# Ugness/MeBT

Hardware: AMD Instinct MI355X
Metric: masked video tokens/sec/GPU (train step, 24L d=1024, 1024+256 tok) (higher is better)
Workload: dtype bf16; 1 GPU; Sky-Timelapse 16f MeBT train step: 24L/1024d/16h, 1024 VQ tokens + 256 latents, batch 6/GPU, t=0.5 (NC=NT=512), fwd + masked CE + bwd + AdamW; global_batch=6, parallelism=dp1, optimizer=in-backward (fused into the weight-gradient launches)

## Files before the change

include/mebt_hip.h:

```cpp
#ifndef MEBT_HIP_H
#define MEBT_HIP_H

#include <stdint.h>

#ifdef __cplusplus
extern "C" {
#endif

#define MEBT_ABI_VERSION 2
#define MEBT_MAX_LAYERS 128

typedef void* mebt_stream_t;
typedef struct mebt_model mebt_model;

enum mebt_status { MEBT_STATUS_OK = 0, MEBT_STATUS_EINVAL = 1, MEBT_STATUS_ESHAPE = 2, MEBT_STATUS_EHIP = 3,
                   MEBT_STATUS_EWORKSPACE = 4, MEBT_STATUS_EDTYPE = 5 };
enum mebt_dtype { MEBT_DTYPE_F32 = 0, MEBT_DTYPE_BF16 = 1, MEBT_DTYPE_F16 = 2  };
enum mebt_mode { MEBT_MODE_LATENT_ENC = 0, MEBT_MODE_LATENT_SELF = 1, MEBT_MODE_LATENT_DEC = 2, MEBT_MODE_LT2L = 3,
                 MEBT_MODE_MASKGIT = 4  };

typedef struct mebt_model_desc {
    int32_t n_layer, n_head, n_embd, vocab, n_latent , block_size;
    int32_t dtype;
    int32_t modes[MEBT_MAX_LAYERS];
    float label_smoothing;
    float embd_pdrop, resid_pdrop, attn_pdrop;
} mebt_model_desc;

const char* mebt_last_error(void);
int mebt_abi_version(void);

int mebt_model_create(const mebt_model_desc* desc, mebt_model** out);
void mebt_model_destroy(mebt_model* m);
int mebt_model_param_counts(const mebt_model* m, int64_t* n_w, int64_t* n_p);
int mebt_model_bind(mebt_model* m, float* W, void* W_lp, float* gW, float* P, float* gP);
int mebt_model_sync_lowp(mebt_model* m, mebt_stream_t stream);
int64_t mebt_workspace_bytes(const mebt_model* m, int32_t B, int32_t NC, int32_t NT, int32_t training);

int mebt_forward(mebt_model* m, void* ws, int64_t ws_bytes, int32_t B, int32_t N, int32_t NC, int32_t NT,
                 const int64_t* x_ids, const int64_t* ci, const int64_t* ti, float* logits,
                 int32_t training, uint64_t dropout_seed, mebt_stream_t stream);
int64_t mebt_kvcache_bytes(const mebt_model* m, int32_t B, int32_t N);
int mebt_forward_kvcache(mebt_model* m, void* ws, int64_t ws_bytes, int32_t B, int32_t N, int32_t NC, int32_t NT,
                         const int64_t* x_ids, const int64_t* ci, const int64_t* ti, void* logits, int32_t flags,
                         void* kv_cache, const int64_t* dirty, int32_t ND, mebt_stream_t stream);
int mebt_gpt_forward(mebt_model* m, void* ws, int64_t ws_bytes, int32_t B, int32_t NC, int32_t NT, const float* sos,
                     const float* contexts, const float* targets, float* logits, mebt_stream_t stream);
int mebt_gpt_forward_train(mebt_model* m, void* ws, int64_t ws_bytes, int32_t B, int32_t NC, int32_t NT, const float* sos,
                           const float* contexts, const float* targets, float* logits, int32_t dropout, uint64_t dropout_seed,
                           mebt_stream_t stream);
int mebt_gpt_backward(mebt_model* m, void* ws, const float* dlogits, float* d_sos, float* d_contexts, float* d_targets,
                      mebt_stream_t stream);
int mebt_loss(mebt_model* m, void* ws, const float* logits, double* out4, mebt_stream_t stream);
int mebt_loss_with_grad(mebt_model* m, void* ws, const float* logits, double* out4, float loss_scale, mebt_stream_t stream);
int mebt_backward_head(mebt_model* m, void* ws, const float* logits, const float* upstream, float loss_scale, mebt_stream_t stream);
int mebt_backward_head_dlogits(mebt_model* m, void* ws, const float* dlogits, mebt_stream_t stream);
int mebt_backward_layers(mebt_model* m, void* ws, int32_t layer_hi, int32_t layer_lo, mebt_stream_t stream);
int mebt_backward_embed(mebt_model* m, void* ws, mebt_stream_t stream);
int mebt_adamw_step(mebt_model* m, float* mW, float* vW, float* mP, float* vP, float lr, float beta1, float beta2,
                    float eps, float weight_decay, int32_t step, float grad_scale, mebt_stream_t stream);

int mebt_adamw_range(mebt_model* m, float* mW, float* vW, float* mP, float* vP, float lr, float beta1, float beta2,
                     float eps, float weight_decay, int32_t step, float grad_scale, int32_t kind, int32_t layer_hi,
                     int32_t layer_lo, mebt_stream_t stream);

int mebt_adamw_slice(mebt_model* m, int32_t which, int64_t off, int64_t n, const void* grad, int32_t grad_bf16, float* mW,
                     float* vW, float* mP, float* vP, float lr, float beta1, float beta2, float eps, float weight_decay,
                     int32_t step, float grad_scale, mebt_stream_t stream);

int mebt_adamw_slice_pieces(mebt_model* m, int32_t which, int64_t off, int64_t n, const void* grad_pieces, int32_t pieces, float* mW,
                            float* vW, float* mP, float* vP, float lr, float beta1, float beta2, float eps, float weight_decay,
                            int32_t step, float grad_scale, mebt_stream_t stream);

int mebt_model_set_fused_adamw(mebt_model* m, float* mW, float* vW, float lr, float beta1, float beta2, float eps,
                               float weight_decay, int32_t step, float grad_scale);

int mebt_model_bind_wire_grads(mebt_model* m, void* gWb);

int mebt_model_set_forward_waits(mebt_model* m, int32_t n, const int32_t* layer, void* const* events);
int mebt_model_set_grad_accumulate(mebt_model* m, int32_t on);

int mebt_op_gemm(int32_t dtype, const void* A, const void* B, void* C, void* C2, const float* bias, const void* aux,
                 int32_t M, int32_t N, int32_t K, int32_t lda, int32_t ldb, int32_t ldc, int32_t ld_aux,
                 int32_t a_kc, int32_t b_kc, int32_t epilogue, int32_t c_f32, int32_t beta, int32_t split_k,
                 mebt_stream_t stream);
int mebt_op_layernorm_fwd(int32_t dtype, const void* x, void* y, const float* gamma, const float* beta, float* mean,
                          float* rstd, int32_t rows, int32_t d, mebt_stream_t stream);
int mebt_op_layernorm_bwd(int32_t dtype, const void* x, const void* dy, const float* gamma, const float* mean,
                          const float* rstd, void* dx, float* dgamma, float* dbeta, int32_t rows, int32_t d,
                          mebt_stream_t stream);
int mebt_op_attention_fwd(int32_t dtype, const void* q, const void* k, const void* v, void* o, float* lse, int32_t B,
                          int32_t H, int32_t NQ, int32_t NK, int32_t HD, int32_t ldq, int32_t ldk, int32_t ldv,
                          int32_t ldo, int32_t force_generic, mebt_stream_t stream);
int mebt_op_attention_bwd(int32_t dtype, const void* q, const void* k, const void* v, const void* o, const float* lse,
                          const void* d_o, void* dq, void* dk, void* dv, float* delta, int32_t B, int32_t H,
                          int32_t NQ, int32_t NK, int32_t HD, int32_t ldq, int32_t ldk, int32_t ldv, int32_t ldo,
                          int32_t force_generic, mebt_stream_t stream);
int mebt_op_embed_fwd(int32_t dtype, const int64_t* x_ids, const int64_t* ci, const int64_t* ti, const float* tok_emb,
                      const float* pos_emb, const float* mask_emb, const float* sos_emb, void* sos, void* ctx, void* tgt,
                      int32_t B, int32_t N, int32_t NC, int32_t NT, int32_t NS, int32_t d, int32_t vocab,
                      int32_t block_size, mebt_stream_t stream);
int mebt_op_sample(const float* logits, const float* noise, float temperature, int32_t top_k, float top_p, int64_t* ids,
                   float* score, float* probs, int32_t rows, int32_t V, mebt_stream_t stream);
int mebt_op_sample_seeded(const float* logits, uint64_t seed, float temperature, int32_t top_k, float top_p, int64_t* ids,
                          float* score, float* probs, int32_t rows, int32_t V, mebt_stream_t stream);
int mebt_op_wgrad_grouped(int32_t n, const void* const* dY, const void* const* X, const int32_t* n_out, const int32_t* k_in,
                          const int32_t* tokens, const int64_t* w_off, float* const* bias, float* W, float* gW, float* mW, float* vW,
                          void* Wlp, int32_t fused, float lr, float beta1, float beta2, float eps, float weight_decay, int32_t step,
                          float grad_scale, mebt_stream_t stream);
int mebt_op_gemm_pair(const void* const* A, const void* const* B, void* const* C, const float* const* bias, const void* const* aux,
                      const int32_t* M, const int32_t* N, const int32_t* K, const int32_t* lda, const int32_t* ldb, const int32_t* ldc,
                      const int32_t* ld_aux, const int32_t* epilogue, const int32_t* c_f32, int32_t b_kc, mebt_stream_t stream);
int mebt_op_topk_threshold(const float* logits, int32_t top_k, float* kth, int64_t* ids_scratch, int32_t rows, int32_t V,
                           mebt_stream_t stream);
int mebt_op_sample_scatter(const float* logits, const float* noise, uint64_t seed, float temperature, int32_t top_k, int64_t* ids,
                           float* score, float* probs_map, const int64_t* ti, int32_t B, int32_t N, int32_t NT, int32_t V,
                           mebt_stream_t stream);
int mebt_op_sample_lp(const void* logits, int32_t logits_bf16, const float* noise, uint64_t seed, float temperature, int32_t top_k,
                      int64_t* ids, float* score, float* probs_map, const int64_t* ti, int32_t B, int32_t N, int32_t NT, int32_t V,
                      int32_t draw, mebt_stream_t stream);
int mebt_op_scatter_ids(int64_t* x, const int64_t* ti, const int64_t* ids, int32_t B, int32_t N, int32_t NT,
                        mebt_stream_t stream);
int mebt_op_next_mask(const int64_t* ci, const int64_t* ti, const float* score, const float* noise, float ctemp,
                      int32_t n_new, int32_t B, int32_t NC, int32_t NT, int64_t* new_ci, int64_t* new_ti,
                      mebt_stream_t stream);
int mebt_op_cast_bf16(const float* src, void* dst, int64_t n, mebt_stream_t stream);

void mebt_gemm_autotune(int32_t mode);
int32_t mebt_gemm_autotune_enabled(void);
int64_t mebt_gemm_tune_export(char* buf, int64_t cap);
int32_t mebt_gemm_tune_import(const char* text, int32_t overwrite);
int64_t mebt_gemm_tune_alternatives(char* buf, int64_t cap);

#define MEBT_CONV_MAX_TAPS 64
typedef struct mebt_conv3d_desc {
    const void* in; void* out; const void* w; const float* bias; const void* resid;
    int32_t B, Ti, Hi, Wi, Cin, To, Ho, Wo, Cout;
    int32_t cT, cH, cW;
    int32_t os[3], pi[3], sm[3];
    int32_t ntaps;
    int8_t tap[MEBT_CONV_MAX_TAPS][4];
    int32_t in_mode;
    int32_t out_mode;
} mebt_conv3d_desc;
int mebt_op_conv3d(int32_t dtype, const mebt_conv3d_desc* d, int32_t allow_mfma, mebt_stream_t stream);
int mebt_op_groupnorm_silu(int32_t dtype, const void* x, void* y, const float* gamma, const float* beta, float* stats, int32_t B,
                           int64_t vox_per_sample, int32_t C, mebt_stream_t stream);
int mebt_op_codebook_argmin(const float* z, const float* embeddings, float* score, float* esq, int64_t* ids, int32_t M,
                            int32_t n_codes, int32_t d, mebt_stream_t stream);
int mebt_op_codebook_argmin_filtered(const float* z, const float* embeddings, void* score, float* esq, void* lowp, int64_t* ids,
                                     int32_t M, int32_t n_codes, int32_t d, mebt_stream_t stream);
int mebt_op_embedding_rows(int32_t dtype, const int64_t* ids, const float* embeddings, void* out, int64_t rows, int32_t d,
                           int32_t n_codes, mebt_stream_t stream);
int mebt_op_cast_f16(const float* src, void* dst, int64_t n, mebt_stream_t stream);

int mebt_op_frames_to_video(const uint8_t* frames, float* out, int32_t N, int32_t T, int32_t Hs, int32_t Ws, int32_t y0, int32_t x0,
                            int32_t S, int32_t R, const int32_t* tab, int32_t K, int32_t rows, int32_t span, const float* lut,
                            const int32_t* slots, int32_t Bout, mebt_stream_t stream);
int mebt_op_frames_to_clip_u8(const uint8_t* frames, uint8_t* out, int32_t N, int32_t T, int32_t Hs, int32_t Ws, int32_t y0, int32_t x0,
                              int32_t S, int32_t R, const int32_t* tab, int32_t K, int32_t rows, int32_t span, const uint8_t* lut,
                              const int32_t* slots, int32_t Bout, mebt_stream_t stream);
int mebt_op_pack_to_video(const uint8_t* pack, int64_t F, const int64_t* ids, float* out, int32_t B, int32_t T, int32_t R,
                          const float* lut, mebt_stream_t stream);
int mebt_op_pack_to_clip_u8(const uint8_t* pack, int64_t F, const int64_t* ids, uint8_t* out, int32_t B, int32_t T, int32_t R,
                            const uint8_t* lut, mebt_stream_t stream);
int mebt_op_video_to_clip_u8(const float* in, uint8_t* out, int32_t B, int32_t Td, int32_t T, int32_t H, int32_t W,
                             mebt_stream_t stream);
int mebt_op_i3d_preprocess(int32_t dtype, const uint8_t* in, void* out, int32_t N, int32_t H, int32_t W, int32_t Ho, int32_t Wo,
                           mebt_stream_t stream);
#define MEBT_I3D_MAX_SEGS 3
typedef struct mebt_i3d_seg {
    void* out;
    int32_t n0, n1, cstride, coff;
} mebt_i3d_seg;
typedef struct mebt_i3d_conv_desc {
    const void* in; const void* w; const float* bias;
    int32_t B, Ti, Hi, Wi, Cin, To, Ho, Wo, Cout;
    int32_t k[3], s[3], pad_front[3], pad_back[3];
    int32_t relu;
    int32_t nseg;
    mebt_i3d_seg seg[MEBT_I3D_MAX_SEGS];
} mebt_i3d_conv_desc;
int mebt_op_i3d_conv(int32_t dtype, const mebt_i3d_conv_desc* d, mebt_stream_t stream);
int mebt_op_i3d_maxpool(int32_t dtype, const void* in, void* out, int32_t B, int32_t Ti, int32_t Hi, int32_t Wi, int32_t C, int32_t kt,
                        int32_t kh, int32_t kw, int32_t st, int32_t sh, int32_t sw, mebt_stream_t stream);
int mebt_op_i3d_head(int32_t dtype, const void* x, const float* w, const float* bias, float* pooled, float* logits, int32_t B, int32_t T,
                     int32_t H, int32_t W, int32_t C, int32_t ncls, mebt_stream_t stream);

int mebt_profile_enable(int32_t on);
int mebt_profile_read(int32_t family, double* launches, double* total_ms, double* total_flops);
int64_t mebt_profile_dump(char* buf, int64_t cap);
int32_t mebt_profile_read_waits(int32_t cap, int32_t* layer, double* ms);
int mebt_debug_dropout_mask(uint64_t seed, uint32_t site, float p, int64_t n, float* out, mebt_stream_t stream);
int mebt_debug_clock_probe(unsigned long long* out4, uint64_t ref_ticks_100mhz, mebt_stream_t stream);
void mebt_debug_side_stream(mebt_model* m, int32_t on);
void mebt_debug_set_side_stream(mebt_model* m, mebt_stream_t stream);
void mebt_debug_gemm_tile(int32_t bm, int32_t bn);
void mebt_debug_gemm_variant(int32_t dma);
void mebt_debug_gemm_scratch(void* buf, int64_t bytes);
void mebt_debug_gemm_stamps(unsigned long long* buf);
void mebt_debug_attn_dropout(uint64_t seed, float p, void* dmask);
void mebt_debug_attn_legacy(int32_t bits);
int mebt_debug_attn_block_order(int32_t T, int32_t X, int32_t H, int32_t xcd, int32_t* pos_to_id, mebt_stream_t stream);
void mebt_debug_grouped_config(int32_t tbm, int32_t tbn, int32_t ring);
void mebt_debug_pair_config(int32_t tbm, int32_t tbn, int32_t ring);
int32_t mebt_debug_gemm_last_launch(int32_t out[8]);
void mebt_debug_grouped_stages(int32_t n);

#ifdef __cplusplus
}
#endif
#endif
```

mebt_amd/_lib.py:

```python
import ctypes as C
import os

_HERE = os.path.dirname(os.path.abspath(__file__))
LIB_PATH = os.environ.get("MEBT_HIP_LIB") or os.path.join(_HERE, "lib", "libmebt_hip.so")

SHIPPED_TUNE = os.path.join(_HERE, "tune", "gfx950.txt")

MEBT_MAX_LAYERS = 128
F32, BF16, F16 = 0, 1, 2
EPI_NONE, EPI_GELU, EPI_RESID, EPI_GELU_BWD = 0, 1, 2, 3
MODE_IDS = {"latent_enc": 0, "latent_self": 1, "latent_dec": 2, "lt2l": 3, "maskgit": 4}

c_i32, c_i64, c_f32, c_vp = C.c_int32, C.c_int64, C.c_float, C.c_void_p


class ModelDesc(C.Structure):
    _fields_ = [("n_layer", c_i32), ("n_head", c_i32), ("n_embd", c_i32), ("vocab", c_i32),
                ("n_latent", c_i32), ("block_size", c_i32), ("dtype", c_i32),
                ("modes", c_i32 * MEBT_MAX_LAYERS), ("label_smoothing", c_f32),
                ("embd_pdrop", c_f32), ("resid_pdrop", c_f32), ("attn_pdrop", c_f32)]


PROTOTYPES = {
    "mebt_last_error": (C.c_char_p, []),
    "mebt_abi_version": (c_i32, []),
    "mebt_model_create": (c_i32, [C.POINTER(ModelDesc), C.POINTER(c_vp)]),
    "mebt_model_destroy": (None, [c_vp]),
    "mebt_model_param_counts": (c_i32, [c_vp, C.POINTER(c_i64), C.POINTER(c_i64)]),
    "mebt_model_bind": (c_i32, [c_vp, c_vp, c_vp, c_vp, c_vp, c_vp]),
    "mebt_model_sync_lowp": (c_i32, [c_vp, c_vp]),
    "mebt_workspace_bytes": (c_i64, [c_vp, c_i32, c_i32, c_i32, c_i32]),
    "mebt_forward": (c_i32, [c_vp, c_vp, c_i64, c_i32, c_i32, c_i32, c_i32, c_vp, c_vp, c_vp, c_vp, c_i32, C.c_uint64, c_vp]),
    "mebt_kvcache_bytes": (c_i64, [c_vp, c_i32, c_i32]),
    "mebt_forward_kvcache": (c_i32, [c_vp, c_vp, c_i64, c_i32, c_i32, c_i32, c_i32, c_vp, c_vp, c_vp, c_vp, c_i32, c_vp, c_vp, c_i32, c_vp]),
    "mebt_gpt_forward": (c_i32, [c_vp, c_vp, c_i64, c_i32, c_i32, c_i32, c_vp, c_vp, c_vp, c_vp, c_vp]),
    "mebt_gpt_forward_train": (c_i32, [c_vp, c_vp, c_i64, c_i32, c_i32, c_i32, c_vp, c_vp, c_vp, c_vp, c_i32, C.c_uint64, c_vp]),
    "mebt_gpt_backward": (c_i32, [c_vp, c_vp, c_vp, c_vp, c_vp, c_vp, c_vp]),
    "mebt_loss": (c_i32, [c_vp, c_vp, c_vp, c_vp, c_vp]),
    "mebt_loss_with_grad": (c_i32, [c_vp, c_vp, c_vp, c_vp, C.c_float, c_vp]),
    "mebt_backward_head": (c_i32, [c_vp, c_vp, c_vp, c_vp, c_f32, c_vp]),
    "mebt_backward_head_dlogits": (c_i32, [c_vp, c_vp, c_vp, c_vp]),
    "mebt_backward_layers": (c_i32, [c_vp, c_vp, c_i32, c_i32, c_vp]),
    "mebt_backward_embed": (c_i32, [c_vp, c_vp, c_vp]),
    "mebt_adamw_step": (c_i32, [c_vp, c_vp, c_vp, c_vp, c_vp, c_f32, c_f32, c_f32, c_f32, c_f32, c_i32, c_f32, c_vp]),
    "mebt_adamw_range": (c_i32, [c_vp, c_vp, c_vp, c_vp, c_vp, c_f32, c_f32, c_f32, c_f32, c_f32, c_i32, c_f32, c_i32, c_i32, c_i32, c_vp]),
    "mebt_adamw_slice": (c_i32, [c_vp, c_i32, c_i64, c_i64, c_vp, c_i32, c_vp, c_vp, c_vp, c_vp, c_f32, c_f32, c_f32, c_f32, c_f32, c_i32, c_f32, c_vp]),
    "mebt_adamw_slice_pieces": (c_i32, [c_vp, c_i32, c_i64, c_i64, c_vp, c_i32, c_vp, c_vp, c_vp, c_vp, c_f32, c_f32, c_f32, c_f32, c_f32, c_i32, c_f32, c_vp]),
    "mebt_model_set_fused_adamw": (c_i32, [c_vp, c_vp, c_vp, c_f32, c_f32, c_f32, c_f32, c_f32, c_i32, c_f32]),
    "mebt_model_set_grad_accumulate": (c_i32, [c_vp, c_i32]),
    "mebt_model_bind_wire_grads": (c_i32, [c_vp, c_vp]),
    "mebt_model_set_forward_waits": (c_i32, [c_vp, c_i32, C.POINTER(C.c_int32), C.POINTER(C.c_void_p)]),
    "mebt_op_gemm": (c_i32, [c_i32, c_vp, c_vp, c_vp, c_vp, c_vp, c_vp] + [c_i32] * 13 + [c_vp]),
    "mebt_op_layernorm_fwd": (c_i32, [c_i32, c_vp, c_vp, c_vp, c_vp, c_vp, c_vp, c_i32, c_i32, c_vp]),
    "mebt_op_layernorm_bwd": (c_i32, [c_i32, c_vp, c_vp, c_vp, c_vp, c_vp, c_vp, c_vp, c_vp, c_i32, c_i32, c_vp]),
    "mebt_op_attention_fwd": (c_i32, [c_i32, c_vp, c_vp, c_vp, c_vp, c_vp] + [c_i32] * 10 + [c_vp]),
    "mebt_op_attention_bwd": (c_i32, [c_i32] + [c_vp] * 10 + [c_i32] * 10 + [c_vp]),
    "mebt_op_embed_fwd": (c_i32, [c_i32] + [c_vp] * 10 + [c_i32] * 8 + [c_vp]),
    "mebt_op_sample": (c_i32, [c_vp, c_vp, c_f32, c_i32, c_f32, c_vp, c_vp, c_vp, c_i32, c_i32, c_vp]),
    "mebt_op_sample_seeded": (c_i32, [c_vp, C.c_uint64, c_f32, c_i32, c_f32, c_vp, c_vp, c_vp, c_i32, c_i32, c_vp]),
    "mebt_op_sample_scatter": (c_i32, [c_vp, c_vp, C.c_uint64, c_f32, c_i32, c_vp, c_vp, c_vp, c_vp, c_i32, c_i32, c_i32, c_i32, c_vp]),
    "mebt_op_sample_lp": (c_i32, [c_vp, c_i32, c_vp, C.c_uint64, c_f32, c_i32, c_vp, c_vp, c_vp, c_vp, c_i32, c_i32, c_i32, c_i32, c_i32, c_vp]),
    "mebt_op_wgrad_grouped": (c_i32, [c_i32, c_vp, c_vp, c_vp, c_vp, c_vp, c_vp, c_vp, c_vp, c_vp, c_vp, c_vp, c_vp, c_i32, c_f32, c_f32, c_f32,
                                      c_f32, c_f32, c_i32, c_f32, c_vp]),
    "mebt_op_gemm_pair": (c_i32, [c_vp] * 14 + [c_i32, c_vp]),
    "mebt_op_topk_threshold": (c_i32, [c_vp, c_i32, c_vp, c_vp, c_i32, c_i32, c_vp]),
    "mebt_op_scatter_ids": (c_i32, [c_vp, c_vp, c_vp, c_i32, c_i32, c_i32, c_vp]),
    "mebt_op_next_mask": (c_i32, [c_vp, c_vp, c_vp, c_vp, c_f32, c_i32, c_i32, c_i32, c_i32, c_vp, c_vp, c_vp]),
    "mebt_op_cast_bf16": (c_i32, [c_vp, c_vp, c_i64, c_vp]),
    "mebt_op_conv3d": (c_i32, [c_i32, c_vp, c_i32, c_vp]),
    "mebt_op_groupnorm_silu": (c_i32, [c_i32, c_vp, c_vp, c_vp, c_vp, c_vp, c_i32, c_i64, c_i32, c_vp]),
    "mebt_op_codebook_argmin": (c_i32, [c_vp, c_vp, c_vp, c_vp, c_vp, c_i32, c_i32, c_i32, c_vp]),
    "mebt_op_codebook_argmin_filtered": (c_i32, [c_vp, c_vp, c_vp, c_vp, c_vp, c_vp, c_i32, c_i32, c_i32, c_vp]),
    "mebt_op_embedding_rows": (c_i32, [c_i32, c_vp, c_vp, c_vp, c_i64, c_i32, c_i32, c_vp]),
    "mebt_op_cast_f16": (c_i32, [c_vp, c_vp, c_i64, c_vp]),
    "mebt_op_i3d_preprocess": (c_i32, [c_i32, c_vp, c_vp, c_i32, c_i32, c_i32, c_i32, c_i32, c_vp]),
    "mebt_op_i3d_conv": (c_i32, [c_i32, c_vp, c_vp]),
    "mebt_op_i3d_maxpool": (c_i32, [c_i32, c_vp, c_vp] + [c_i32] * 11 + [c_vp]),
    "mebt_op_i3d_head": (c_i32, [c_i32, c_vp, c_vp, c_vp, c_vp, c_vp] + [c_i32] * 6 + [c_vp]),
    "mebt_op_frames_to_video": (c_i32, [c_vp, c_vp] + [c_i32] * 8 + [c_vp, c_i32, c_i32, c_i32, c_vp, c_vp, c_i32, c_vp]),
    "mebt_op_frames_to_clip_u8": (c_i32, [c_vp, c_vp] + [c_i32] * 8 + [c_vp, c_i32, c_i32, c_i32, c_vp, c_vp, c_i32, c_vp]),
    "mebt_op_pack_to_video": (c_i32, [c_vp, c_i64, c_vp, c_vp, c_i32, c_i32, c_i32, c_vp, c_vp]),
    "mebt_op_pack_to_clip_u8": (c_i32, [c_vp, c_i64, c_vp, c_vp, c_i32, c_i32, c_i32, c_vp, c_vp]),
    "mebt_op_video_to_clip_u8": (c_i32, [c_vp, c_vp, c_i32, c_i32, c_i32, c_i32, c_i32, c_vp]),
    "mebt_debug_dropout_mask": (c_i32, [C.c_uint64, C.c_uint32, c_f32, c_i64, c_vp, c_vp]),
    "mebt_debug_clock_probe": (c_i32, [c_vp, C.c_uint64, c_vp]),
    "mebt_debug_side_stream": (None, [c_vp, c_i32]),
    "mebt_debug_set_side_stream": (None, [c_vp, c_vp]),
    "mebt_debug_gemm_tile": (None, [c_i32, c_i32]),
    "mebt_debug_gemm_variant": (None, [c_i32]),
    "mebt_debug_grouped_stages": (None, [c_i32]),
    "mebt_debug_gemm_scratch": (None, [c_vp, c_i64]),
    "mebt_debug_gemm_stamps": (None, [c_vp]),
    "mebt_debug_grouped_config": (None, [c_i32, c_i32, c_i32]),
    "mebt_debug_pair_config": (None, [c_i32, c_i32, c_i32]),
    "mebt_debug_gemm_last_launch": (c_i32, [C.POINTER(c_i32)]),
    "mebt_debug_attn_dropout": (None, [C.c_uint64, c_f32, c_vp]),
    "mebt_debug_attn_legacy": (None, [c_i32]),
    "mebt_debug_attn_block_order": (c_i32, [c_i32, c_i32, c_i32, c_i32, c_vp, c_vp]),
    "mebt_gemm_autotune": (None, [c_i32]),
    "mebt_gemm_autotune_enabled": (c_i32, []),
    "mebt_gemm_tune_export": (c_i64, [C.c_char_p, c_i64]),
    "mebt_gemm_tune_import": (c_i32, [C.c_char_p, c_i32]),
    "mebt_gemm_tune_alternatives": (c_i64, [C.c_char_p, c_i64]),
    "mebt_profile_enable": (c_i32, [c_i32]),
    "mebt_profile_read": (c_i32, [c_i32, C.POINTER(C.c_double), C.POINTER(C.c_double), C.POINTER(C.c_double)]),
    "mebt_profile_dump": (c_i64, [C.c_char_p, c_i64]),
    "mebt_profile_read_waits": (c_i32, [c_i32, C.POINTER(C.c_int32), C.POINTER(C.c_double)]),
}

_lib = None


def load():
    global _lib
    if _lib is not None:
        return _lib
    if not os.path.exists(LIB_PATH):
        raise RuntimeError(
            f"{LIB_PATH} not found: build it with `python -c 'import __graft_entry__ as g; g.build()'` "
            "(or `make -C mebt_amd/csrc`). mebt_amd has no fallback path without its HIP library.")
    try:
        import torch
    except ImportError:
        pass
    lib = C.CDLL(LIB_PATH)
    for name, (res, args) in PROTOTYPES.items():
        fn = getattr(lib, name)
        fn.restype = res
        fn.argtypes = args
    _lib = lib
    if os.environ.get("MEBT_GEMM_TUNE_SHIPPED", "1") != "0" and os.path.exists(SHIPPED_TUNE):
        with open(SHIPPED_TUNE, "rb") as f:
            lib.mebt_gemm_tune_import(f.read(), 0)
    return lib


def tune_table_text():
    lib = load()
    n = lib.mebt_gemm_tune_export(None, 0)
    buf = C.create_string_buffer(int(n))
    lib.mebt_gemm_tune_export(buf, n)
    return buf.value.decode()


def tune_table_merge(text, overwrite=True, replace=False):
    return int(load().mebt_gemm_tune_import(text.encode() if isinstance(text, str) else text, 2 if replace else (1 if overwrite else 0)))


class MebtError(RuntimeError):
    pass


def check(status):
    if status != 0:
        msg = load().mebt_last_error()
        raise MebtError(f"libmebt_hip status {status}: {msg.decode() if msg else '?'}")


def ptr(t):
    return None if t is None else t.data_ptr()


def cur_stream():
    import torch
    return torch.cuda.current_stream().cuda_stream
```

mebt_amd/csrc/capi.cpp:

```cpp
#include "common.h"
#include "kernels.h"
#include <cmath>
#include "../../include/mebt_hip.h"
#include <string.h>

static hipStream_t S(mebt_stream_t s) { return reinterpret_cast<hipStream_t>(s); }
static int check_dtype(int dtype) {
    if (dtype == MEBT_F32 || dtype == MEBT_BF16) return MEBT_OK;
    mebt_set_error("unsupported dtype (0 = f32, 1 = bf16)");
    return MEBT_EDTYPE;
}

extern "C" int mebt_op_gemm(int32_t dtype, const void* A, const void* B, void* C, void* C2, const float* bias, const void* aux,
                            int32_t M, int32_t N, int32_t K, int32_t lda, int32_t ldb, int32_t ldc, int32_t ld_aux,
                            int32_t a_kc, int32_t b_kc, int32_t epilogue, int32_t c_f32, int32_t beta, int32_t split_k,
                            mebt_stream_t stream) {
    if (int rc = check_dtype(dtype)) return rc;
    if (!A || !B || (!C && epilogue != EPI_GELU)) { mebt_set_error("gemm: null operand"); return MEBT_EINVAL; }
    if (epilogue < EPI_NONE || epilogue > EPI_GELU_BWD) { mebt_set_error("gemm: bad epilogue"); return MEBT_EINVAL; }
    if ((epilogue == EPI_RESID || epilogue == EPI_GELU_BWD) && !aux) { mebt_set_error("gemm: epilogue needs aux"); return MEBT_EINVAL; }
    if (epilogue == EPI_GELU && !C2) { mebt_set_error("gemm: GELU epilogue needs C2"); return MEBT_EINVAL; }
    if (M < 0 || N < 0 || K <= 0) { mebt_set_error("gemm: bad extents"); return MEBT_ESHAPE; }
    static bool inited = false;
    if (!inited) { if (int rc = gemm_init_attributes()) return rc; inited = true; }
// ... 52 lines not shown
}

extern "C" int mebt_op_layernorm_fwd(int32_t dtype, const void* x, void* y, const float* gamma, const float* beta, float* mean,
                                     float* rstd, int32_t rows, int32_t d, mebt_stream_t stream) {
    if (int rc = check_dtype(dtype)) return rc;
    if (!x || !y || !gamma || !beta) { mebt_set_error("layernorm: null pointer"); return MEBT_EINVAL; }
    LnFwdParams p;
    p.x = x; p.y = y; p.gamma = gamma; p.beta = beta; p.mean = mean; p.rstd = rstd; p.rows = rows; p.d = d;
    p.seg = 0; p.seg_stride = 0; p.seg_off = 0;
    return launch_ln_fwd(p, dtype, S(stream));
}

extern "C" int mebt_op_layernorm_bwd(int32_t dtype, const void* x, const void* dy, const float* gamma, const float* mean,
                                     const float* rstd, void* dx, float* dgamma, float* dbeta, int32_t rows, int32_t d,
                                     mebt_stream_t stream) {
    if (int rc = check_dtype(dtype)) return rc;
    if (!x || !dy || !gamma || !mean || !rstd || !dx || !dgamma || !dbeta) { mebt_set_error("layernorm_bwd: null pointer"); return MEBT_EINVAL; }
    LnBwdParams p;
    p.x = x; p.dy = dy; p.dy2 = nullptr; p.dx_add = nullptr; p.gamma = gamma; p.mean = mean; p.rstd = rstd; p.dx = dx; p.dx_f32 = dtype == MEBT_F32;
    p.dx_accumulate = 0; p.dgamma = dgamma; p.dbeta = dbeta; p.rows = rows; p.d = d; p.seg = 0; p.seg_stride = 0; p.seg_off = 0;
    return launch_ln_bwd(p, dtype, S(stream));
}

static DropCfg g_op_attn_drop = make_drop(0, 0, 0.f);
static uint16_t* g_op_attn_dmask = nullptr;
extern "C" void mebt_debug_attn_dropout(uint64_t seed, float p, void* dmask) {
    g_op_attn_drop = make_drop(seed, SITE_ATTN, p);
    g_op_attn_dmask = p > 0.f ? (uint16_t*)dmask : nullptr;
}
extern "C" void mebt_debug_attn_legacy(int32_t bits) { mebt_attn_set_legacy(bits); }
extern "C" int mebt_debug_attn_block_order(int32_t T, int32_t X, int32_t H, int32_t xcd, int32_t* pos_to_id, mebt_stream_t stream) {
    if (!pos_to_id) { mebt_set_error("attention block order: null pointer"); return MEBT_EINVAL; }
    return launch_attn_block_order_probe(T, X, H, xcd, pos_to_id, S(stream));
}

extern "C" int mebt_op_attention_fwd(int32_t dtype, const void* q, const void* k, const void* v, void* o, float* lse, int32_t B,
                                     int32_t H, int32_t NQ, int32_t NK, int32_t HD, int32_t ldq, int32_t ldk, int32_t ldv,
                                     int32_t ldo, int32_t force_generic, mebt_stream_t stream) {
    if (int rc = check_dtype(dtype)) return rc;
    if (!q || !o || (NK > 0 && (!k || !v))) { mebt_set_error("attention: null pointer"); return MEBT_EINVAL; }
    AttnParams p;
    memset(&p, 0, sizeof(p));
    p.q = q; p.k = k; p.v = v; p.o = o; p.lse = lse; p.B = B; p.H = H; p.NQ = NQ; p.NK = NK; p.HD = HD;
    p.ldq = ldq; p.ldk = ldk; p.ldv = ldv; p.ldo = ldo;
    p.drop = g_op_attn_drop; p.dmask = g_op_attn_dmask;
    mebt_attn_force_generic(force_generic);
    const int rc = launch_attn_fwd(p, dtype, S(stream));
    mebt_attn_force_generic(0);
    return rc;
}

extern "C" int mebt_op_attention_bwd(int32_t dtype, const void* q, const void* k, const void* v, const void* o, const float* lse,
                                     const void* d_o, void* dq, void* dk, void* dv, float* delta, int32_t B, int32_t H,
                                     int32_t NQ, int32_t NK, int32_t HD, int32_t ldq, int32_t ldk, int32_t ldv, int32_t ldo,
                                     int32_t force_generic, mebt_stream_t stream) {
    if (int rc = check_dtype(dtype)) return rc;
    if (!q || !o || !lse || !d_o || !dq || !delta || (NK > 0 && (!k || !v || !dk || !dv))) { mebt_set_error("attention_bwd: null pointer"); return MEBT_EINVAL; }
    AttnParams p;
    memset(&p, 0, sizeof(p));
    p.q = q; p.k = k; p.v = v; p.o = const_cast<void*>(o); p.lse = const_cast<float*>(lse); p.B = B; p.H = H; p.NQ = NQ; p.NK = NK; p.HD = HD;
    p.ldq = ldq; p.ldk = ldk; p.ldv = ldv; p.ldo = ldo;
    p.d_o = d_o; p.dq = dq; p.dk = dk; p.dv = dv; p.delta = delta; p.lddo = ldo; p.lddq = ldq; p.lddk = ldk; p.lddv = ldv;
    p.drop = g_op_attn_drop; p.dmask = g_op_attn_dmask;
    mebt_attn_force_generic(force_generic);
    const int rc = launch_attn_bwd(p, dtype, S(stream));
    mebt_attn_force_generic(0);
    return rc;
}

extern "C" int mebt_op_embed_fwd(int32_t dtype, const int64_t* x_ids, const int64_t* ci, const int64_t* ti, const float* tok_emb,
                                 const float* pos_emb, const float* mask_emb, const float* sos_emb, void* sos, void* ctx, void* tgt,
                                 int32_t B, int32_t N, int32_t NC, int32_t NT, int32_t NS, int32_t d, int32_t vocab,
                                 int32_t block_size, mebt_stream_t stream) {
    if (int rc = check_dtype(dtype)) return rc;
    if (!x_ids || !tok_emb || !pos_emb || !mask_emb) { mebt_set_error("embed: null pointer"); return MEBT_EINVAL; }
    if (N > block_size) { mebt_set_error("embed: N exceeds block_size"); return MEBT_ESHAPE; }
    EmbedParams p;
    p.x_ids = x_ids; p.ci = ci; p.ti = ti; p.tok_emb = tok_emb; p.pos_emb = pos_emb; p.mask_emb = mask_emb; p.sos_emb = sos_emb;
    p.sos = sos; p.ctx = ctx; p.tgt = tgt; p.B = B; p.N = N; p.NC = NC; p.NT = NT; p.NS = NS; p.d = d; p.vocab = vocab; p.block_size = block_size;
    p.drop = make_drop(0, 0, 0.f);
    return launch_embed_fwd(p, dtype, S(stream));
}

extern "C" int mebt_op_sample(const float* logits, const float* noise, float temperature, int32_t top_k, float top_p, int64_t* ids,
                              float* score, float* probs, int32_t rows, int32_t V, mebt_stream_t stream) {
    if (!logits || !noise || !ids) { mebt_set_error("sample: null pointer"); return MEBT_EINVAL; }
    SampleParams p;
    p.logits = logits; p.noise = noise; p.temperature = temperature; p.top_k = top_k; p.top_p = top_p; p.ids = ids; p.score = score;
    p.probs = probs; p.rows = rows; p.V = V;
    return launch_sample(p, S(stream));
}

extern "C" int mebt_op_sample_seeded(const float* logits, uint64_t seed, float temperature, int32_t top_k, float top_p, int64_t* ids,
                                     float* score, float* probs, int32_t rows, int32_t V, mebt_stream_t stream) {
    if (!logits || !ids) { mebt_set_error("sample: null pointer"); return MEBT_EINVAL; }
    SampleParams p;
    p.logits = logits; p.noise = nullptr; p.noise_seed = seed; p.temperature = temperature; p.top_k = top_k; p.top_p = top_p; p.ids = ids;
    p.score = score; p.probs = probs; p.rows = rows; p.V = V;
    return launch_sample(p, S(stream));
}

extern "C" int mebt_op_sample_scatter(const float* logits, const float* noise, uint64_t seed, float temperature, int32_t top_k, int64_t* ids,
                                      float* score, float* probs_map, const int64_t* ti, int32_t B, int32_t N, int32_t NT, int32_t V,
                                      mebt_stream_t stream) {
    if (!logits || !ids || !probs_map || !ti) { mebt_set_error("sample_scatter: null pointer"); return MEBT_EINVAL; }
    if (B <= 0 || NT <= 0 || N < NT) { mebt_set_error("sample_scatter: need B > 0 and 0 < NT <= N"); return MEBT_ESHAPE; }
    SampleParams p;
    p.logits = logits; p.noise = noise; p.noise_seed = seed; p.temperature = temperature; p.top_k = top_k; p.top_p = 0.f; p.ids = ids;
    p.score = score; p.probs = probs_map; p.rows = B * NT; p.V = V; p.probs_ti = ti; p.probs_N = N; p.probs_NT = NT;
    return launch_sample(p, S(stream));
}

extern "C" int mebt_op_sample_lp(const void* logits, int32_t logits_bf16, const float* noise, uint64_t seed, float temperature, int32_t top_k,
                                 int64_t* ids, float* score, float* probs_map, const int64_t* ti, int32_t B, int32_t N, int32_t NT, int32_t V,
                                 int32_t draw, mebt_stream_t stream) {
    if (!logits || !ids) { mebt_set_error("sample_lp: null pointer"); return MEBT_EINVAL; }
    if ((probs_map != nullptr) != (ti != nullptr)) { mebt_set_error("sample_lp: probs_map and ti go together"); return MEBT_EINVAL; }
    if (B <= 0 || NT <= 0 || (probs_map && N < NT)) { mebt_set_error("sample_lp: need B > 0 and 0 < NT <= N"); return MEBT_ESHAPE; }
    SampleParams p;
    p.logits = reinterpret_cast<const float*>(logits); p.logits_bf16 = logits_bf16 ? 1 : 0; p.noise = noise; p.noise_seed = seed;
    p.temperature = temperature; p.top_k = top_k; p.top_p = 0.f; p.ids = ids; p.score = score; p.probs = probs_map; p.rows = B * NT; p.V = V;
    p.probs_ti = ti; p.probs_N = probs_map ? N : 0; p.probs_NT = probs_map ? NT : 0;
    if (draw != 0 && draw != 1) { mebt_set_error("sample_lp: draw must be 0 (arg-max p / q) or 1 (inverse CDF)"); return MEBT_EINVAL; }
    if (draw == 1 && noise) { mebt_set_error("sample_lp: the inverse-CDF draw takes no noise tensor"); return MEBT_EINVAL; }
    p.icdf = draw;
    return launch_sample(p, S(stream));
}

extern "C" int mebt_op_topk_threshold(const float* logits, int32_t top_k, float* kth, int64_t* ids_scratch, int32_t rows, int32_t V, mebt_stream_t stream) {
    if (!logits || !kth || !ids_scratch) { mebt_set_error("topk_threshold: null pointer"); return MEBT_EINVAL; }
    if (top_k <= 0 || top_k >= V) { mebt_set_error("topk_threshold: k must be in [1, V)"); return MEBT_ESHAPE; }
    SampleParams p;
    p.logits = logits; p.noise = nullptr; p.noise_seed = 0; p.temperature = 1.0f; p.top_k = top_k; p.top_p = 0.f; p.ids = ids_scratch;
    p.score = nullptr; p.probs = nullptr; p.rows = rows; p.V = V; p.kth = kth;
    return launch_sample(p, S(stream));
}

extern "C" int mebt_op_scatter_ids(int64_t* x, const int64_t* ti, const int64_t* ids, int32_t B, int32_t N, int32_t NT, mebt_stream_t stream) {
    if (!x || !ti || !ids) { mebt_set_error("scatter_ids: null pointer"); return MEBT_EINVAL; }
    return launch_scatter_ids(x, ti, ids, B, N, NT, S(stream));
}

extern "C" int mebt_op_next_mask(const int64_t* ci, const int64_t* ti, const float* score, const float* noise, float ctemp,
                                 int32_t n_new, int32_t B, int32_t NC, int32_t NT, int64_t* new_ci, int64_t* new_ti, mebt_stream_t stream) {
    if (!ti || !score || !noise || !new_ci || (NT - n_new > 0 && !new_ti) || (NC > 0 && !ci)) { mebt_set_error("next_mask: null pointer"); return MEBT_EINVAL; }
    NextMaskParams p;
    p.ci = ci; p.ti = ti; p.score = score; p.noise = noise; p.ctemp = ctemp; p.n_new = n_new; p.B = B; p.NC = NC; p.NT = NT;
    p.new_ci = new_ci; p.new_ti = new_ti;
    return launch_next_mask(p, S(stream));
}

extern "C" int mebt_op_cast_bf16(const float* src, void* dst, int64_t n, mebt_stream_t stream) {
    if (!src || !dst) { mebt_set_error("cast: null pointer"); return MEBT_EINVAL; }
    return launch_cast_f32_to_bf16(src, dst, (size_t)n, S(stream));
}
```

mebt_amd/csrc/common.h:

```cpp
#pragma once
#include <hip/hip_runtime.h>
#include <stdint.h>

typedef __bf16 bf16_t;
typedef __bf16 bf16x4 __attribute__((ext_vector_type(4)));
typedef __bf16 bf16x8 __attribute__((ext_vector_type(8)));
typedef short s16x4 __attribute__((ext_vector_type(4)));
typedef float f32x4 __attribute__((ext_vector_type(4)));
typedef float f32x16 __attribute__((ext_vector_type(16)));
typedef uint32_t u32x4 __attribute__((ext_vector_type(4)));
typedef uint32_t u32x2 __attribute__((ext_vector_type(2)));

#define MEBT_WAVE 64

enum { MEBT_OK = 0, MEBT_EINVAL = 1, MEBT_ESHAPE = 2, MEBT_EHIP = 3, MEBT_EWORKSPACE = 4, MEBT_EDTYPE = 5 };

#define MEBT_HIP_CHECK(expr)                                   \
    do {                                                       \
        hipError_t _e = (expr);                                \
        if (_e != hipSuccess) { mebt_set_hip_error(_e, #expr); (void)hipGetLastError(); return MEBT_EHIP; } \
    } while (0)
void mebt_set_hip_error(hipError_t e, const char* what);
void mebt_set_error(const char* msg);

// ... 9 lines not shown

typedef __attribute__((address_space(3))) void* lds_void_ptr;
typedef __attribute__((address_space(3))) char* lds_char_ptr;
__device__ __forceinline__ void dma16(__amdgpu_buffer_rsrc_t rsrc, unsigned lds_addr, unsigned voff) {
    unsigned keep;
    asm volatile("s_mov_b32 %0, m0\n\ts_mov_b32 m0, %2\n\ts_nop 0\n\tbuffer_load_dwordx4 %1, %3, 0 offen lds\n\ts_mov_b32 m0, %0"
                 : "=&s"(keep)
                 : "v"(voff), "s"(lds_addr), "s"(rsrc)
                 : "memory");
}

__device__ __forceinline__ unsigned lds_addr_of(const void* p) { return (unsigned)(size_t)(lds_char_ptr)(char*)p; }

template <typename T> __device__ __forceinline__ float to_f32(T v);
template <> __device__ __forceinline__ float to_f32<float>(float v) { return v; }
template <> __device__ __forceinline__ float to_f32<bf16_t>(bf16_t v) { return (float)v; }
template <typename T> __device__ __forceinline__ T from_f32(float v);
template <> __device__ __forceinline__ float from_f32<float>(float v) { return v; }
template <> __device__ __forceinline__ bf16_t from_f32<bf16_t>(float v) { return (bf16_t)v; }

template <typename T> __device__ __forceinline__ f32x4 load4(const T* p);
template <> __device__ __forceinline__ f32x4 load4<float>(const float* p) { return *reinterpret_cast<const f32x4*>(p); }
template <> __device__ __forceinline__ f32x4 load4<bf16_t>(const bf16_t* p) {
    bf16x4 v = *reinterpret_cast<const bf16x4*>(p);
    return f32x4{(float)v[0], (float)v[1], (float)v[2], (float)v[3]};
}
template <typename T> __device__ __forceinline__ void store4(T* p, f32x4 v);
template <> __device__ __forceinline__ void store4<float>(float* p, f32x4 v) { *reinterpret_cast<f32x4*>(p) = v; }
template <> __device__ __forceinline__ void store4<bf16_t>(bf16_t* p, f32x4 v) {
    bf16x4 o = {(bf16_t)v[0], (bf16_t)v[1], (bf16_t)v[2], (bf16_t)v[3]};
    *reinterpret_cast<bf16x4*>(p) = o;
}

__device__ __forceinline__ float wave_sum(float v) {
#pragma unroll
    for (int o = 32; o > 0; o >>= 1) v += __shfl_xor(v, o, 64);
    return v;
}
__device__ __forceinline__ float wave_max(float v) {
#pragma unroll
    for (int o = 32; o > 0; o >>= 1) v = fmaxf(v, __shfl_xor(v, o, 64));
    return v;
}
__device__ __forceinline__ int wave_sum_i(int v) {
#pragma unroll
    for (int o = 32; o > 0; o >>= 1) v += __shfl_xor(v, o, 64);
    return v;
}

__device__ __forceinline__ float gelu_f(float x) { return 0.5f * x * (1.0f + erff(x * 0.70710678118654752f)); }
__device__ __forceinline__ float gelu_grad_f(float x) {
    const float cdf = 0.5f * (1.0f + erff(x * 0.70710678118654752f));
    const float pdf = 0.3989422804014327f * __expf(-0.5f * x * x);
    return cdf + x * pdf;
}

__device__ __forceinline__ float erf_fast(float x) {
    const float ax = fabsf(x);
    float d = 1.0f + ax * (0.278393f + ax * (0.230389f + ax * (0.000972f + ax * 0.078108f)));
    d *= d; d *= d;
    return copysignf(1.0f - __frcp_rn(d), x);
}
__device__ __forceinline__ float gelu_fast(float x) { return 0.5f * x * (1.0f + erf_fast(x * 0.70710678118654752f)); }
__device__ __forceinline__ float gelu_grad_fast(float x) {
    const float cdf = 0.5f * (1.0f + erf_fast(x * 0.70710678118654752f));
    return cdf + x * 0.3989422804014327f * __builtin_amdgcn_exp2f(-0.7213475204444817f * x * x);
}

struct AdamWHyper { float lr, beta1, beta2, eps, weight_decay, bc1, bc2, grad_scale; };
__device__ __forceinline__ void adamw_update4(f32x4& p, const f32x4& g, f32x4& m, f32x4& v, const AdamWHyper& a) {
    const float step_size = a.lr / a.bc1;
    const float inv_sqrt_bc2 = rsqrtf(a.bc2);
#pragma unroll
    for (int j = 0; j < 4; ++j) {
        const float gj = g[j] * a.grad_scale;
        p[j] *= 1.0f - a.lr * a.weight_decay;
        m[j] = a.beta1 * m[j] + (1.0f - a.beta1) * gj;
        v[j] = a.beta2 * v[j] + (1.0f - a.beta2) * gj * gj;
        const float denom = sqrtf(v[j]) * inv_sqrt_bc2 + a.eps;
        p[j] -= step_size * (m[j] / denom);
    }
}

__device__ __forceinline__ uint32_t pair_hash(uint64_t seed, uint32_t site, uint64_t pair) {
    uint32_t h = ((uint32_t)pair ^ (uint32_t)seed) + ((uint32_t)(pair >> 32) + site) * 0x632BE5ABu + (uint32_t)(seed >> 32);
    h *= 0x9E3779B1u;
    h ^= h >> 15;
    h *= 0x85EBCA77u;
    h ^= h >> 13;
    return h;
}
__device__ __forceinline__ uint32_t mix_hash(uint64_t seed, uint32_t site, uint64_t idx) {
    const uint32_t h = pair_hash(seed, site, idx >> 1);
    return (idx & 1) ? (h >> 16) : (h & 0xFFFFu);
}
struct DropCfg {
    uint64_t seed;
    uint32_t site;
    uint32_t thresh;
    float inv_keep;
    uint32_t small;
    uint32_t base32;
};
__device__ __forceinline__ uint32_t pair_hash_cfg(const DropCfg& d, uint64_t pair) {
    if (!d.small) return pair_hash(d.seed, d.site, pair);
    uint32_t h = ((uint32_t)pair ^ (uint32_t)d.seed) + d.base32;
    h *= 0x9E3779B1u;
    h ^= h >> 15;
    h *= 0x85EBCA77u;
    h ^= h >> 13;
    return h;
}
__device__ __forceinline__ float drop_keep(const DropCfg& d, uint64_t idx) {
    const uint32_t h = pair_hash_cfg(d, idx >> 1);
    return ((idx & 1) ? (h >> 16) : (h & 0xFFFFu)) >= d.thresh ? d.inv_keep : 0.0f;
}
__device__ __forceinline__ f32x4 drop_keep4(const DropCfg& d, uint64_t idx0) {
    f32x4 k;
    if ((idx0 & 1) == 0) {
        const uint32_t h0 = pair_hash_cfg(d, idx0 >> 1), h1 = pair_hash_cfg(d, (idx0 >> 1) + 1);
        k[0] = (h0 & 0xFFFFu) >= d.thresh ? d.inv_keep : 0.0f;
        k[1] = (h0 >> 16) >= d.thresh ? d.inv_keep : 0.0f;
        k[2] = (h1 & 0xFFFFu) >= d.thresh ? d.inv_keep : 0.0f;
        k[3] = (h1 >> 16) >= d.thresh ? d.inv_keep : 0.0f;
    } else {
#pragma unroll
        for (int j = 0; j < 4; ++j) k[j] = drop_keep(d, idx0 + j);
    }
    return k;
}
```

mebt_amd/csrc/elementwise.hip:

```cpp
#include "common.h"
#include <cstdlib>
#include "kernels.h"

namespace {

template <typename T>
__global__ __launch_bounds__(256) void embed_fwd_kernel(const EmbedParams p) {
    const int lane = threadIdx.x & 63;
    const long row = (long)blockIdx.x * 4 + (threadIdx.x >> 6);
    const long per_b = (long)p.NS + p.NC + p.NT;
    if (row >= per_b * p.B) return;
    const int b = (int)(row / per_b);
    const int r = (int)(row % per_b);
    const float* src0;
    const float* src1 = nullptr;
    T* dst;
    DropCfg dc = p.drop;
    uint64_t ebase;
    if (r < p.NS) {
        src0 = p.sos_emb + (size_t)r * p.d;
        dst = reinterpret_cast<T*>(p.sos) + ((size_t)b * p.NS + r) * p.d;
        dc.site = SITE_EMB_SOS; ebase = ((uint64_t)b * p.NS + r) * p.d;
    } else if (r < p.NS + p.NC) {
        const int i = r - p.NS;
        long pos = p.ci[(size_t)b * p.NC + i];
        pos = pos < 0 ? 0 : (pos >= p.N ? p.N - 1 : pos);
        long tok = p.x_ids[(size_t)b * p.N + pos];
        tok = tok < 0 ? 0 : (tok >= p.vocab ? p.vocab - 1 : tok);
        src0 = p.tok_emb + (size_t)tok * p.d;
        src1 = p.pos_emb + (size_t)pos * p.d;
        dst = reinterpret_cast<T*>(p.ctx) + ((size_t)b * p.NC + i) * p.d;
        dc.site = SITE_EMB_CTX; ebase = ((uint64_t)b * p.NC + i) * p.d;
    } else {
        const int j = r - p.NS - p.NC;
        long pos = p.ti[(size_t)b * p.NT + j];
        pos = pos < 0 ? 0 : (pos >= p.N ? p.N - 1 : pos);
        src0 = p.mask_emb;
        src1 = p.pos_emb + (size_t)pos * p.d;
        dst = reinterpret_cast<T*>(p.tgt) + ((size_t)b * p.NT + j) * p.d;
        dc.site = SITE_EMB_TGT; ebase = ((uint64_t)b * p.NT + j) * p.d;
    }
    for (int e = lane * 4; e < p.d; e += 256) {
        f32x4 v = *reinterpret_cast<const f32x4*>(src0 + e);
        if (src1) v += *reinterpret_cast<const f32x4*>(src1 + e);
        if (dc.thresh) {
            v *= drop_keep4(dc, ebase + e);
        }
        store4<T>(dst + e, v);
    }
}

template <typename T>
__global__ __launch_bounds__(256) void embed_bwd_kernel(const EmbedBwdParams p) {
    const int lane = threadIdx.x & 63;
    const long row = (long)blockIdx.x * 4 + (threadIdx.x >> 6);
    const long per_b = (long)p.NC + p.NT;
    if (row >= per_b * p.B) return;
    const int b = (int)(row / per_b);
    const int r = (int)(row % per_b);
    if (r < p.NC) {
        const long pos = p.ci[(size_t)b * p.NC + r];
        const long tok = p.x_ids[(size_t)b * p.N + pos];
        const float* g = p.g_ctx + ((size_t)b * p.NC + r) * p.d;
        float* gt = p.g_tok_emb + (size_t)tok * p.d;
        float* gp = p.g_pos_emb + (size_t)pos * p.d;
        for (int e = lane; e < p.d; e += 64) {
            const float v = g[e];
            atomicAdd(gt + e, v);
            atomicAdd(gp + e, v);
        }
    } else {
        const int j0 = r - p.NC;
        const long pos = p.ti[(size_t)b * p.NT + j0];
        const T* g = reinterpret_cast<const T*>(p.g_tgt) + ((size_t)b * p.NT + j0) * p.d;
        float* gp = p.g_pos_emb + (size_t)pos * p.d;
        for (int e = lane; e < p.d; e += 64) atomicAdd(gp + e, to_f32<T>(g[e]));
    }
}

constexpr int LN_MAXC = 8;

__device__ __forceinline__ long map_row(long r, int seg, int seg_stride, int seg_off) {
    return seg > 0 ? (r / seg) * (long)seg_stride + seg_off + (r % seg) : r;
}

struct LnFwdMulti { LnFwdParams j[MEBT_LN_MAXJ]; int blk_start[MEBT_LN_MAXJ + 1]; int n; };
struct LnBwdMulti { LnBwdParams j[MEBT_LN_MAXJ]; int blk_start[MEBT_LN_MAXJ + 1]; int rpw[MEBT_LN_MAXJ]; int n; };

template <typename T>
__global__ __launch_bounds__(256) void ln_fwd_kernel(const LnFwdMulti mj) {
    int job = 0;
#pragma unroll
    for (int i = 1; i < MEBT_LN_MAXJ; ++i)
        if (i < mj.n && (int)blockIdx.x >= mj.blk_start[i]) job = i;
    const LnFwdParams& p = mj.j[job];
    const int lane = threadIdx.x & 63;
    const long row = (long)(blockIdx.x - mj.blk_start[job]) * 4 + (threadIdx.x >> 6);
    if (row >= p.rows) return;
    const T* x = reinterpret_cast<const T*>(p.x) + (size_t)row * p.d;
    f32x4 v[LN_MAXC];
    float s = 0.f;
#pragma unroll
    for (int c = 0; c < LN_MAXC; ++c) {
        const int e = lane * 4 + 256 * c;
        if (e < p.d) {
            v[c] = load4<T>(x + e);
            s += v[c][0] + v[c][1] + v[c][2] + v[c][3];
        }
    }
    const float mean = wave_sum(s) / p.d;
    float q = 0.f;
#pragma unroll
    for (int c = 0; c < LN_MAXC; ++c) {
        const int e = lane * 4 + 256 * c;
        if (e < p.d) {
#pragma unroll
            for (int j = 0; j < 4; ++j) { const float t = v[c][j] - mean; q += t * t; }
        }
    }
    const float rstd = rsqrtf(wave_sum(q) / p.d + 1e-5f);
    const long orow = map_row(row, p.seg, p.seg_stride, p.seg_off);
    T* y = reinterpret_cast<T*>(p.y) + (size_t)orow * p.d;
#pragma unroll
    for (int c = 0; c < LN_MAXC; ++c) {
        const int e = lane * 4 + 256 * c;
        if (e < p.d) {
            const f32x4 g = *reinterpret_cast<const f32x4*>(p.gamma + e);
            const f32x4 b = *reinterpret_cast<const f32x4*>(p.beta + e);
            f32x4 o;
#pragma unroll
            for (int j = 0; j < 4; ++j) o[j] = (v[c][j] - mean) * rstd * g[j] + b[j];
            store4<T>(y + e, o);
        }
    }
    if (p.mean && lane == 0) { p.mean[orow] = mean; p.rstd[orow] = rstd; }
}

template <typename T>
__device__ __forceinline__ void ln_bwd_dx_body(const LnBwdMulti& mj, int bid) {
    int job = 0;
#pragma unroll
    for (int i = 1; i < MEBT_LN_MAXJ; ++i)
        if (i < mj.n && bid >= mj.blk_start[i]) job = i;
    const LnBwdParams& p = mj.j[job];
    const int lane = threadIdx.x & 63;
    const int d = p.d;
    const long row = (long)(bid - mj.blk_start[job]) * 4 + (threadIdx.x >> 6);
    if (row >= p.rows) return;
    const long mrow = map_row(row, p.seg, p.seg_stride, p.seg_off);
    const T* x = reinterpret_cast<const T*>(p.x) + (size_t)row * d;
    const T* dy = reinterpret_cast<const T*>(p.dy) + (size_t)mrow * d;
    const T* dy2 = p.dy2 ? reinterpret_cast<const T*>(p.dy2) + (size_t)row * d : nullptr;
    const float mean = p.mean[mrow], rstd = p.rstd[mrow];
    f32x4 xh[LN_MAXC], gy[LN_MAXC];
    float s1 = 0.f, s2 = 0.f;
#pragma unroll
    for (int c = 0; c < LN_MAXC; ++c) {
        const int e = lane * 4 + 256 * c;
        if (e < d) {
// ... 338 lines not shown
    const float lt = l[tgt];
    float mx = -INFINITY, sum = 0.f;
    int rank = 0;
    for (int e = threadIdx.x * 4; e < p.V; e += 1024) {
        const f32x4 v = *reinterpret_cast<const f32x4*>(l + e);
#pragma unroll
        for (int q = 0; q < 4; ++q) {
            mx = fmaxf(mx, v[q]);
            sum += v[q];
            rank += (v[q] > lt) || (v[q] == lt && (e + q) < tgt);
        }
    }
    mx = block_max(mx, sh);
    float se = 0.f;
    for (int e = threadIdx.x * 4; e < p.V; e += 1024) {
        const f32x4 v = *reinterpret_cast<const f32x4*>(l + e);
#pragma unroll
        for (int q = 0; q < 4; ++q) se += __expf(v[q] - mx);
    }
    se = block_sum(se, sh);
    sum = block_sum(sum, sh);
    const float rk = block_sum((float)rank, sh);
    if (threadIdx.x == 0) {
        const float lse = mx + logf(se);
        const float eps = p.label_smoothing;
        p.row_lse[row] = lse;
        p.row_loss[row] = (1.f - eps) * (lse - lt) + eps * (lse - sum / p.V);
        p.row_rank[row] = (int)(rk + 0.5f);
    }
}

template <typename T, int NCH>
__global__ __launch_bounds__(256) void ce_fused_kernel(const CeParams p) {
    __shared__ float sh[4];
    const int row = blockIdx.x;
    const int b = row / p.NT, j = row % p.NT;
    const long pos = p.ti[(size_t)b * p.NT + j];
    const long tgt = p.x_ids[(size_t)b * p.N + pos];
    const float* l = p.logits + (size_t)row * p.V;
    f32x4 v[NCH];
#pragma unroll
    for (int c = 0; c < NCH; ++c) v[c] = *reinterpret_cast<const f32x4*>(l + threadIdx.x * 4 + 1024 * c);
    const float lt = l[tgt];
    float mx = -INFINITY, sum = 0.f;
    int rank = 0;
#pragma unroll
    for (int c = 0; c < NCH; ++c) {
        const int e = threadIdx.x * 4 + 1024 * c;
#pragma unroll
        for (int q = 0; q < 4; ++q) {
            mx = fmaxf(mx, v[c][q]);
            sum += v[c][q];
            rank += (v[c][q] > lt) || (v[c][q] == lt && (e + q) < tgt);
        }
    }
    mx = block_max(mx, sh);
    float se = 0.f;
#pragma unroll
    for (int c = 0; c < NCH; ++c)
#pragma unroll
        for (int q = 0; q < 4; ++q) se += __expf(v[c][q] - mx);
    se = block_sum(se, sh);
    sum = block_sum(sum, sh);
    const float rk = block_sum((float)rank, sh);
    const float lse = mx + logf(se);
    const float eps = p.label_smoothing;
    if (threadIdx.x == 0) {
        p.row_lse[row] = lse;
        p.row_loss[row] = (1.f - eps) * (lse - lt) + eps * (lse - sum / p.V);
        p.row_rank[row] = (int)(rk + 0.5f);
    }
    T* d = reinterpret_cast<T*>(p.dlogits) + (size_t)row * p.V;
    const float sc = p.grad_scale, u = eps / p.V;
#pragma unroll
    for (int c = 0; c < NCH; ++c) {
        const int e = threadIdx.x * 4 + 1024 * c;
        f32x4 o;
#pragma unroll
        for (int q = 0; q < 4; ++q) o[q] = (__expf(v[c][q] - lse) - ((e + q) == tgt ? 1.f - eps : 0.f) - u) * sc;
        store4<T>(d + e, o);
    }
}

__global__ __launch_bounds__(256) void ce_reduce_kernel(const float* row_loss, const int* row_rank, int rows, double* out) {
    __shared__ double sd[3][256];
    double s = 0, t1 = 0, t5 = 0;
    for (int r = threadIdx.x; r < rows; r += 256) {
        s += row_loss[r];
        t1 += row_rank[r] < 1;
        t5 += row_rank[r] < 5;
    }
    sd[0][threadIdx.x] = s; sd[1][threadIdx.x] = t1; sd[2][threadIdx.x] = t5;
    __syncthreads();
    for (int o = 128; o > 0; o >>= 1) {
        if (threadIdx.x < o) {
            sd[0][threadIdx.x] += sd[0][threadIdx.x + o];
            sd[1][threadIdx.x] += sd[1][threadIdx.x + o];
            sd[2][threadIdx.x] += sd[2][threadIdx.x + o];
        }
        __syncthreads();
    }
    if (threadIdx.x == 0) { out[0] = sd[0][0]; out[1] = sd[1][0]; out[2] = sd[2][0]; out[3] = rows; }
}

template <typename T>
__global__ __launch_bounds__(256) void ce_bwd_kernel(const CeBwdParams p) {
    const int row = blockIdx.x;
    const int b = row / p.NT, j = row % p.NT;
    const long pos = p.ti[(size_t)b * p.NT + j];
    const long tgt = p.x_ids[(size_t)b * p.N + pos];
    const float* l = p.logits + (size_t)row * p.V;
    T* d = reinterpret_cast<T*>(p.dlogits) + (size_t)row * p.V;
    const float lse = p.row_lse[row];
    const float sc = p.scale * (p.upstream ? *p.upstream : 1.0f);
    const float eps = p.label_smoothing, u = eps / p.V;
    for (int e = threadIdx.x * 4; e < p.V; e += 1024) {
        const f32x4 v = *reinterpret_cast<const f32x4*>(l + e);
        f32x4 o;
#pragma unroll
        for (int q = 0; q < 4; ++q) o[q] = (__expf(v[q] - lse) - ((e + q) == tgt ? 1.f - eps : 0.f) - u) * sc;
        store4<T>(d + e, o);
    }
}

template <typename TG>
__global__ __launch_bounds__(256) void adamw_kernel(const AdamWParams a) {
    const AdamWHyper h = {a.lr, a.beta1, a.beta2, a.eps, a.weight_decay, a.bc1, a.bc2, a.grad_scale};
    for (size_t i = ((size_t)blockIdx.x * 256 + threadIdx.x) * 4; i < a.n; i += (size_t)gridDim.x * 1024) {
        f32x4 p = *reinterpret_cast<const f32x4*>(a.p + i);
        f32x4 g = load4<TG>(reinterpret_cast<const TG*>(a.g) + i);
        if constexpr (sizeof(TG) == 2)
            for (int j = 1; j < a.g_pieces; ++j) g += load4<TG>(reinterpret_cast<const TG*>(a.g) + (size_t)j * a.g_stride + i);
        f32x4 m = *reinterpret_cast<const f32x4*>(a.m + i);
        f32x4 v = *reinterpret_cast<const f32x4*>(a.v + i);
        adamw_update4(p, g, m, v, h);
        *reinterpret_cast<f32x4*>(a.p + i) = p;
        *reinterpret_cast<f32x4*>(a.m + i) = m;
        *reinterpret_cast<f32x4*>(a.v + i) = v;
        if (a.p_bf16) store4<bf16_t>(reinterpret_cast<bf16_t*>(a.p_bf16) + i, p);
    }
}

template <typename TS, typename TD>
__global__ __launch_bounds__(256) void apply_dropout_kernel(const TS* src, TD* dst, size_t n, DropCfg d) {
    for (size_t i = ((size_t)blockIdx.x * 256 + threadIdx.x) * 4; i < n; i += (size_t)gridDim.x * 1024) {
        f32x4 v = load4<TS>(src + i);
        v *= drop_keep4(d, i);
        store4<TD>(dst + i, v);
    }
}

template <typename TS, typename TD>
__global__ __launch_bounds__(256) void copy_rows_kernel(const TS* src, TD* dst, long rows, int d, int s_seg, int s_stride, int s_off,
                                                        int d_seg, int d_stride, int d_off) {
    const int d4 = d / 4;
    const long total = rows * d4;
    for (long i = (long)blockIdx.x * 256 + threadIdx.x; i < total; i += (long)gridDim.x * 256) {
        const long r = i / d4;
        const int e = (int)(i % d4) * 4;
        store4<TD>(dst + (size_t)map_row(r, d_seg, d_stride, d_off) * d + e, load4<TS>(src + (size_t)map_row(r, s_seg, s_stride, s_off) * d + e));
    }
}

__global__ __launch_bounds__(256) void cast_bf16_kernel(const float* src, bf16_t* dst, size_t n) {
    for (size_t i = ((size_t)blockIdx.x * 256 + threadIdx.x) * 4; i < n; i += (size_t)gridDim.x * 1024)
        store4<bf16_t>(dst + i, *reinterpret_cast<const f32x4*>(src + i));
}

}

#define CHECK_LAUNCH() MEBT_HIP_CHECK(hipGetLastError())

int launch_embed_fwd(const EmbedParams& p, int dtype, hipStream_t stream) {
    if (p.d % 4) { mebt_set_error("embed: d must be a multiple of 4"); return MEBT_ESHAPE; }
    const long rows = (long)p.B * (p.NS + p.NC + p.NT);
    if (rows == 0) return MEBT_OK;
    const dim3 grid((unsigned)((rows + 3) / 4));
    if (dtype == MEBT_BF16) hipLaunchKernelGGL(embed_fwd_kernel<bf16_t>, grid, dim3(256), 0, stream, p);
    else hipLaunchKernelGGL(embed_fwd_kernel<float>, grid, dim3(256), 0, stream, p);
    CHECK_LAUNCH();
    return MEBT_OK;
}

int launch_embed_bwd(const EmbedBwdParams& p, int dtype, hipStream_t stream) {
    const long rows = (long)p.B * (p.NC + p.NT);
    if (rows > 0) {
        const dim3 grid((unsigned)((rows + 3) / 4));
        if (dtype == MEBT_BF16) hipLaunchKernelGGL(embed_bwd_kernel<bf16_t>, grid, dim3(256), 0, stream, p);
        else hipLaunchKernelGGL(embed_bwd_kernel<float>, grid, dim3(256), 0, stream, p);
        CHECK_LAUNCH();
    }
    int rc = launch_colsum(p.g_tgt, p.B * p.NT, p.d, p.d, p.g_mask_emb, dtype, stream);
    if (rc) return rc;
    if (p.NS > 0) rc = launch_colsum(p.g_sos, p.B, p.NS * p.d, p.NS * p.d, p.g_sos_emb, dtype, stream);
    return rc;
}

int launch_ln_fwd_multi(const LnFwdParams* jobs, int n, int dtype, hipStream_t stream) {
    LnFwdMulti mj;
    int k = 0, blocks = 0;
    for (int i = 0; i < n; ++i) {
        const LnFwdParams& p = jobs[i];
        if (p.rows <= 0) continue;
        if (p.d % 4 || p.d > 256 * LN_MAXC) { mebt_set_error("layernorm: d must be a multiple of 4 and <= 2048"); return MEBT_ESHAPE; }
        if (k == MEBT_LN_MAXJ) { mebt_set_error("layernorm: too many jobs in one launch"); return MEBT_EINVAL; }
        mj.j[k] = p;
        mj.blk_start[k] = blocks;
        blocks += (p.rows + 3) / 4;
        ++k;
    }
    if (!k) return MEBT_OK;
    mj.n = k;
    for (int i = k; i <= MEBT_LN_MAXJ; ++i) mj.blk_start[i] = blocks;
    bool same_d = true;
    for (int i = 1; i < k; ++i) same_d = same_d && mj.j[i].d == mj.j[0].d;
    const int d0 = mj.j[0].d;
    if (dtype == MEBT_BF16) {
        if (same_d && d0 == 1024) hipLaunchKernelGGL((ln_fwd_fast_kernel<bf16_t, 2>), dim3(blocks), dim3(256), 0, stream, mj);
        else if (same_d && d0 == 512) hipLaunchKernelGGL((ln_fwd_fast_kernel<bf16_t, 1>), dim3(blocks), dim3(256), 0, stream, mj);
        else if (same_d && d0 == 2048) hipLaunchKernelGGL((ln_fwd_fast_kernel<bf16_t, 4>), dim3(blocks), dim3(256), 0, stream, mj);
        else hipLaunchKernelGGL(ln_fwd_kernel<bf16_t>, dim3(blocks), dim3(256), 0, stream, mj);
    } else {
        if (same_d && d0 == 1024) hipLaunchKernelGGL((ln_fwd_fast_kernel<float, 4>), dim3(blocks), dim3(256), 0, stream, mj);
        else if (same_d && d0 == 256) hipLaunchKernelGGL((ln_fwd_fast_kernel<float, 1>), dim3(blocks), dim3(256), 0, stream, mj);
        else hipLaunchKernelGGL(ln_fwd_kernel<float>, dim3(blocks), dim3(256), 0, stream, mj);
    }
    CHECK_LAUNCH();
    return MEBT_OK;
}

int launch_ln_fwd(const LnFwdParams& p, int dtype, hipStream_t stream) { return launch_ln_fwd_multi(&p, 1, dtype, stream); }

static int prepare_colsum(const GroupedColsum& c, GroupedColsum& k, int& blocks_out);
int launch_ln_bwd_multi(const LnBwdParams* jobs, int n, int dtype, hipStream_t stream, hipStream_t param_stream, const GroupedColsum* colsums) {
    LnBwdMulti mj, mp;
    int k = 0, blocks = 0, pblocks = 0;
    for (int i = 0; i < n; ++i) {
        const LnBwdParams& p = jobs[i];
        if (p.rows <= 0) continue;
        if (p.d % 4 || p.d > 256 * LN_MAXC) { mebt_set_error("layernorm: d must be a multiple of 4 and <= 2048"); return MEBT_ESHAPE; }
        if (k == MEBT_LN_MAXJ) { mebt_set_error("layernorm: too many jobs in one launch"); return MEBT_EINVAL; }
        mj.j[k] = p; mp.j[k] = p;
        mj.rpw[k] = 1;
        mj.blk_start[k] = blocks;
        blocks += (p.rows + 3) / 4;
        const int gx = (p.d + 63) / 64;
        int rpb = 256;
        while ((p.rows + rpb - 1) / rpb > 32) rpb *= 2;
        while (rpb > 64 && (long)gx * ((p.rows + rpb - 1) / rpb) < 256) rpb /= 2;
        mp.rpw[k] = rpb;
        mp.blk_start[k] = pblocks;
        pblocks += gx * ((p.rows + rpb - 1) / rpb);
        ++k;
    }
    if (!k) return MEBT_OK;
    mj.n = mp.n = k;
    for (int i = k; i <= MEBT_LN_MAXJ; ++i) { mj.blk_start[i] = blocks; mp.blk_start[i] = pblocks; }
    (void)param_stream;
    bool same_d = true;
    for (int i = 1; i < k; ++i) same_d = same_d && mj.j[i].d == mj.j[0].d;
    const int d0 = mj.j[0].d;
    GroupedColsum cs;
    int cblocks = 0;
    if (colsums) { if (int rc = prepare_colsum(*colsums, cs, cblocks)) return rc; }
    if (cblocks) {
        const dim3 grid(blocks + pblocks + cblocks);
        const int cs_start = blocks + pblocks;
        if (dtype == MEBT_BF16) {
            if (same_d && d0 == 1024) hipLaunchKernelGGL((ln_bwd_colsum_kernel<bf16_t, 2>), grid, dim3(256), 0, stream, mj, mp, cs, blocks, cs_start);
            else if (same_d && d0 == 512) hipLaunchKernelGGL((ln_bwd_colsum_kernel<bf16_t, 1>), grid, dim3(256), 0, stream, mj, mp, cs, blocks, cs_start);
            else if (same_d && d0 == 2048) hipLaunchKernelGGL((ln_bwd_colsum_kernel<bf16_t, 4>), grid, dim3(256), 0, stream, mj, mp, cs, blocks, cs_start);
            else hipLaunchKernelGGL((ln_bwd_colsum_kernel<bf16_t, 0>), grid, dim3(256), 0, stream, mj, mp, cs, blocks, cs_start);
        } else {
            if (same_d && d0 == 1024) hipLaunchKernelGGL((ln_bwd_colsum_kernel<float, 4>), grid, dim3(256), 0, stream, mj, mp, cs, blocks, cs_start);
            else if (same_d && d0 == 256) hipLaunchKernelGGL((ln_bwd_colsum_kernel<float, 1>), grid, dim3(256), 0, stream, mj, mp, cs, blocks, cs_start);
            else hipLaunchKernelGGL((ln_bwd_colsum_kernel<float, 0>), grid, dim3(256), 0, stream, mj, mp, cs, blocks, cs_start);
        }
        CHECK_LAUNCH();
        return MEBT_OK;
    }
    const dim3 grid(blocks + pblocks);
    if (dtype == MEBT_BF16) {
        if (same_d && d0 == 1024) hipLaunchKernelGGL((ln_bwd_kernel<bf16_t, 2>), grid, dim3(256), 0, stream, mj, mp, blocks);
        else if (same_d && d0 == 512) hipLaunchKernelGGL((ln_bwd_kernel<bf16_t, 1>), grid, dim3(256), 0, stream, mj, mp, blocks);
        else if (same_d && d0 == 2048) hipLaunchKernelGGL((ln_bwd_kernel<bf16_t, 4>), grid, dim3(256), 0, stream, mj, mp, blocks);
        else hipLaunchKernelGGL((ln_bwd_kernel<bf16_t, 0>), grid, dim3(256), 0, stream, mj, mp, blocks);
    } else {
        if (same_d && d0 == 1024) hipLaunchKernelGGL((ln_bwd_kernel<float, 4>), grid, dim3(256), 0, stream, mj, mp, blocks);
        else if (same_d && d0 == 256) hipLaunchKernelGGL((ln_bwd_kernel<float, 1>), grid, dim3(256), 0, stream, mj, mp, blocks);
        else hipLaunchKernelGGL((ln_bwd_kernel<float, 0>), grid, dim3(256), 0, stream, mj, mp, blocks);
    }
    CHECK_LAUNCH();
    return MEBT_OK;
}

int launch_ln_bwd(const LnBwdParams& p, int dtype, hipStream_t stream, hipStream_t param_stream) { return launch_ln_bwd_multi(&p, 1, dtype, stream, param_stream, nullptr); }

int launch_colsum(const void* X, int M, int N, int ldx, float* out, int dtype, hipStream_t stream) {
    if (M <= 0 || N <= 0) return MEBT_OK;
    if (N % 4) { mebt_set_error("colsum: N must be a multiple of 4"); return MEBT_ESHAPE; }
    const int gx = (N + 63) / 64;
    int rpb = 256;
    while ((M + rpb - 1) / rpb > 32) rpb *= 2;
    while (rpb > 64 && (long)gx * ((M + rpb - 1) / rpb) < 256) rpb /= 2;
    const dim3 grid(gx, (M + rpb - 1) / rpb);
    if (dtype == MEBT_BF16) hipLaunchKernelGGL(colsum_kernel<bf16_t>, grid, dim3(256), 0, stream, reinterpret_cast<const bf16_t*>(X), M, N, ldx, out, rpb);
    else hipLaunchKernelGGL(colsum_kernel<float>, grid, dim3(256), 0, stream, reinterpret_cast<const float*>(X), M, N, ldx, out, rpb);
    CHECK_LAUNCH();
    return MEBT_OK;
}

static int prepare_colsum(const GroupedColsum& c, GroupedColsum& k, int& blocks_out) {
    int n = 0, blocks = 0;
    for (int i = 0; i < c.n; ++i) {
        if (c.g[i].M <= 0 || c.g[i].N <= 0) continue;
        if (c.g[i].N % 4) { mebt_set_error("colsum: N must be a multiple of 4"); return MEBT_ESHAPE; }
        k.g[n] = c.g[i];
        k.g[n].gx = (c.g[i].N + 63) / 64;
        int rpb = 256;
        while ((c.g[i].M + rpb - 1) / rpb > 32) rpb *= 2;
        while (rpb > 64 && (long)k.g[n].gx * ((c.g[i].M + rpb - 1) / rpb) < 128) rpb /= 2;
        k.g[n].rpb = rpb;
        k.blk_start[n] = blocks;
        blocks += k.g[n].gx * ((c.g[i].M + rpb - 1) / rpb);
        ++n;
    }
    k.n = n;
    for (int i = n; i <= MEBT_MAX_GROUP; ++i) k.blk_start[i] = blocks;
    blocks_out = blocks;
    return MEBT_OK;
}

int launch_colsum_grouped(GroupedColsum& c, int dtype, hipStream_t stream) {
    GroupedColsum k;
    int blocks = 0;
    if (int rc = prepare_colsum(c, k, blocks)) return rc;
    if (!blocks) return MEBT_OK;
    if (dtype == MEBT_BF16) hipLaunchKernelGGL(colsum_grouped_kernel<bf16_t>, dim3(blocks), dim3(256), 0, stream, k);
    else hipLaunchKernelGGL(colsum_grouped_kernel<float>, dim3(blocks), dim3(256), 0, stream, k);
    CHECK_LAUNCH();
    return MEBT_OK;
}

int launch_ce_fwd(const CeParams& p, hipStream_t stream) {
    if (p.V % 4) { mebt_set_error("cross-entropy: V must be a multiple of 4"); return MEBT_ESHAPE; }
    if (p.rows > 0) {
        if (p.dlogits && ce_fwd_can_fuse_grad(p.V)) {
            if (p.dl_bf16) hipLaunchKernelGGL((ce_fused_kernel<bf16_t, 16>), dim3(p.rows), dim3(256), 0, stream, p);
            else hipLaunchKernelGGL((ce_fused_kernel<float, 16>), dim3(p.rows), dim3(256), 0, stream, p);
        } else {
            hipLaunchKernelGGL(ce_fwd_kernel, dim3(p.rows), dim3(256), 0, stream, p);
        }
        CHECK_LAUNCH();
    }
    hipLaunchKernelGGL(ce_reduce_kernel, dim3(1), dim3(256), 0, stream, p.row_loss, p.row_rank, p.rows, p.out);
    CHECK_LAUNCH();
    return MEBT_OK;
}

int launch_ce_bwd(const CeBwdParams& p, int dtype, hipStream_t stream) {
    if (p.rows <= 0) return MEBT_OK;
    if (dtype == MEBT_BF16) hipLaunchKernelGGL(ce_bwd_kernel<bf16_t>, dim3(p.rows), dim3(256), 0, stream, p);
    else hipLaunchKernelGGL(ce_bwd_kernel<float>, dim3(p.rows), dim3(256), 0, stream, p);
    CHECK_LAUNCH();
    return MEBT_OK;
}

int launch_adamw(const AdamWParams& p, hipStream_t stream) {
    if (p.n == 0) return MEBT_OK;
    if (p.n % 4) { mebt_set_error("adamw: flat buffer length must be a multiple of 4"); return MEBT_ESHAPE; }
    const size_t blocks = (p.n / 4 + 255) / 256;
    if (p.g_bf16) hipLaunchKernelGGL(adamw_kernel<bf16_t>, dim3((unsigned)(blocks < 4096 ? blocks : 4096)), dim3(256), 0, stream, p);
    else hipLaunchKernelGGL(adamw_kernel<float>, dim3((unsigned)(blocks < 4096 ? blocks : 4096)), dim3(256), 0, stream, p);
    CHECK_LAUNCH();
    return MEBT_OK;
}

int launch_apply_dropout(const void* src, void* dst, size_t n, int src_f32, int dst_f32, const DropCfg& d, hipStream_t stream) {
    if (n == 0) return MEBT_OK;
    if (n % 4) { mebt_set_error("dropout: length must be a multiple of 4"); return MEBT_ESHAPE; }
    const size_t blocks = (n / 4 + 255) / 256;
    const dim3 grid((unsigned)(blocks < 4096 ? blocks : 4096));
    if (src_f32 && dst_f32) hipLaunchKernelGGL((apply_dropout_kernel<float, float>), grid, dim3(256), 0, stream, (const float*)src, (float*)dst, n, d);
    else if (!src_f32 && !dst_f32) hipLaunchKernelGGL((apply_dropout_kernel<bf16_t, bf16_t>), grid, dim3(256), 0, stream, (const bf16_t*)src, (bf16_t*)dst, n, d);
    else { mebt_set_error("dropout: mixed element types are not supported"); return MEBT_EDTYPE; }
    CHECK_LAUNCH();
    return MEBT_OK;
}

int launch_copy_rows(const void* src, void* dst, long rows, int d, int src_f32, int dst_f32, int s_seg, int s_stride, int s_off,
                     int d_seg, int d_stride, int d_off, hipStream_t stream) {
    if (rows <= 0 || d <= 0) return MEBT_OK;
    if (d % 4) { mebt_set_error("copy_rows: d must be a multiple of 4"); return MEBT_ESHAPE; }
    const long blocks = (rows * (d / 4) + 255) / 256;
    const dim3 grid((unsigned)(blocks < 8192 ? blocks : 8192));
#define COPY_ROWS(TS, TD) hipLaunchKernelGGL((copy_rows_kernel<TS, TD>), grid, dim3(256), 0, stream, (const TS*)src, (TD*)dst, rows, d, s_seg, s_stride, s_off, d_seg, d_stride, d_off)
    if (src_f32 && dst_f32) COPY_ROWS(float, float);
    else if (src_f32) COPY_ROWS(float, bf16_t);
    else if (dst_f32) COPY_ROWS(bf16_t, float);
    else COPY_ROWS(bf16_t, bf16_t);
#undef COPY_ROWS
    CHECK_LAUNCH();
    return MEBT_OK;
}

namespace {
__global__ __launch_bounds__(256) void index_rows_kernel(const char* src, char* dst, const int64_t* idx, long rows, int n, int npos, int row_bytes, int scatter) {
    const int lane = threadIdx.x & 63;
    const long r = (long)blockIdx.x * 4 + (threadIdx.x >> 6);
    if (r >= rows) return;
    const long b = r / n;
    const long pos = idx[r];
    if (pos < 0 || pos >= npos) return;
    const char* s = src + (size_t)(scatter ? r : b * npos + pos) * row_bytes;
    char* d = dst + (size_t)(scatter ? b * npos + pos : r) * row_bytes;
    for (int o = lane * 16; o < row_bytes; o += 1024) *reinterpret_cast<u32x4*>(d + o) = *reinterpret_cast<const u32x4*>(s + o);
}
}
namespace {
__global__ __launch_bounds__(256) void cast_i64_i32_kernel(const int64_t* src, int32_t* dst, size_t n) {
    const size_t i = (size_t)blockIdx.x * 256 + threadIdx.x;
    if (i < n) dst[i] = (int32_t)src[i];
}
}
int launch_cast_i64_i32(const int64_t* src, int32_t* dst, size_t n, hipStream_t stream) {
    if (!n) return MEBT_OK;
    hipLaunchKernelGGL(cast_i64_i32_kernel, dim3((unsigned)((n + 255) / 256)), dim3(256), 0, stream, src, dst, n);
    CHECK_LAUNCH();
    return MEBT_OK;
}
int launch_index_rows(const void* src, void* dst, const int64_t* idx, int B, int n, int npos, int row_bytes, int scatter, hipStream_t stream) {
    const long rows = (long)B * n;
    if (rows <= 0) return MEBT_OK;
    if (row_bytes % 16) { mebt_set_error("index_rows: rows must be a multiple of 16 bytes"); return MEBT_ESHAPE; }
    hipLaunchKernelGGL(index_rows_kernel, dim3((unsigned)((rows + 3) / 4)), dim3(256), 0, stream, (const char*)src, (char*)dst, idx, rows, n, npos, row_bytes, scatter);
    CHECK_LAUNCH();
    return MEBT_OK;
}

int launch_cast_f32_to_bf16(const float* src, void* dst, size_t n, hipStream_t stream) {
    if (n == 0) return MEBT_OK;
    if (n % 4) { mebt_set_error("cast: length must be a multiple of 4"); return MEBT_ESHAPE; }
    const size_t blocks = (n / 4 + 255) / 256;
    hipLaunchKernelGGL(cast_bf16_kernel, dim3((unsigned)(blocks < 4096 ? blocks : 4096)), dim3(256), 0, stream, src, reinterpret_cast<bf16_t*>(dst), n);
    CHECK_LAUNCH();
    return MEBT_OK;
}

namespace {
__global__ __launch_bounds__(64) void clock_probe_kernel(unsigned long long* out, unsigned long long ref_ticks) {
    if (threadIdx.x != 0) return;
    const unsigned long long t0 = __builtin_amdgcn_s_memtime(), r0 = __builtin_amdgcn_s_memrealtime();
    while (__builtin_amdgcn_s_memrealtime() - r0 < ref_ticks) __builtin_amdgcn_s_sleep(127);
    out[0] = t0; out[1] = r0; out[2] = __builtin_amdgcn_s_memtime(); out[3] = __builtin_amdgcn_s_memrealtime();
}
}
// ... 7 lines not shown
```

mebt_amd/csrc/engine.cpp:

```cpp
#include "common.h"
#include "kernels.h"
#include "../../include/mebt_hip.h"
#include <string.h>
#include <math.h>
#include <vector>
#include <string>
#include <cstdlib>

namespace {

struct LayerOffsets {
    int64_t wq, wk, wv, wp, w1, w2;
    int64_t ln1w, ln1b, ln2w, ln2b, bq, bk, bv, bp, b1, b2;
};

struct Carve {
    char* base;
    int64_t off;
    void* take(int64_t bytes) {
        const int64_t o = off;
        off += (bytes + 255) & ~(int64_t)255;
        return base ? base + o : nullptr;
    }
};

struct LayerAct {
    void *qn, *kn, *q, *k, *v, *att, *x, *hn, *pre, *u, *out;
    float *mean1q, *rstd1q, *mean1k, *rstd1k, *mean2, *rstd2, *lse;
    uint16_t* dmask = nullptr;
    const void* q_in;
    const void* k_in;
    void *c_out, *t_out;
    int NQ, NK, ldqkv_q, ldqkv_k;
};

struct FwdCtx {
    bool valid = false;
    void* ws = nullptr;
    int B = 0, N = 0, NC = 0, NT = 0;
    const int64_t *x_ids = nullptr, *ci = nullptr, *ti = nullptr;
    int32_t* ci32 = nullptr;
    void *sos0 = nullptr, *ctx = nullptr, *tgt0 = nullptr;
    std::vector<LayerAct> L;
    const void *S_final = nullptr, *T_final = nullptr;
    void* hf = nullptr; float *meanf = nullptr, *rstdf = nullptr;
    float* logits_ws = nullptr;
    float *row_lse = nullptr, *row_loss = nullptr; int* row_rank = nullptr; double* loss_out = nullptr;
    bool loss_done = false;
    bool dlogits_ready = false;
    float dlogits_scale = 0.f;
    void *g_S = nullptr, *g_T = nullptr; float* g_C = nullptr;
    void* g_cat = nullptr;
    void *dlogits = nullptr, *dhf = nullptr, *datt = nullptr;
    struct Scratch { void *d4, *dh, *dx, *dqkv_q, *dqkv_k, *dqn, *dkn, *dout_m, *dx_m; } sc[2];
    float* delta = nullptr;
    bool gS_defined = false, gT_defined = false, gC_defined = false;
    int doutm_ready = -1;
    int last_bwd_lo = -1;
    bool drop_on = false; uint64_t drop_seed = 0;
    GemmScratch tune = {nullptr, 0, nullptr, 0};
};

}

struct mebt_model {
    mebt_model_desc d;
    std::vector<LayerOffsets> lo;
    int64_t n_w = 0, n_p = 0;
    int64_t head_w = 0, lnf_w = 0, lnf_b = 0, mask_emb = 0, sos_emb = 0, pos_emb = 0, tok_emb = 0;
    float *W = nullptr, *gW = nullptr, *P = nullptr, *gP = nullptr;
    void* Wlp = nullptr;
    bool attn_bits = true;
    bool tune_flush = true;
    void* gWb = nullptr;

    std::vector<char> live;
    bool tok_live = false;
    bool has_maskgit = false;
    FwdCtx ctx;
    hipStream_t side = nullptr;
    hipEvent_t ev_fork = nullptr, ev_e1 = nullptr, ev_layer[2] = {nullptr, nullptr}, ev_join = nullptr;
    bool use_side = true;
    hipStream_t side_own = nullptr;
    bool fused_on = false;
    bool grad_acc = false;
    GroupedWgrad pend_w;
    bool pend = false;
    float *fused_mW = nullptr, *fused_vW = nullptr;
    AdamWHyper fused_h = {0, 0, 0, 0, 0, 1, 1, 1};
    bool wire() const { return gWb && d.dtype == MEBT_BF16 && !grad_acc && !fused_on; }
    std::vector<std::pair<int, hipEvent_t>> fw_waits;
    int esz() const { return d.dtype == MEBT_BF16 ? 2 : 4; }
    const void* Wop(int64_t off) const {
        return d.dtype == MEBT_BF16 ? (const void*)((const char*)Wlp + off * 2) : (const void*)(W + off);
    }
};

static hipStream_t S(mebt_stream_t s) { return reinterpret_cast<hipStream_t>(s); }
static int fork_side(mebt_model* m, hipStream_t st);
static int join_side(mebt_model* m, hipStream_t st);

namespace {
struct ProfRec {
    hipEvent_t a, b; double flops, bytes; int kind = 0;
    int tag = 0;
    int dims[8] = {0, 0, 0, 0, 0, 0, 0, 0};
};
bool g_prof_on = false;
std::vector<ProfRec> g_prof;
std::vector<hipEvent_t> g_ev_pool;
hipEvent_t get_event() {
    if (!g_ev_pool.empty()) { hipEvent_t e = g_ev_pool.back(); g_ev_pool.pop_back(); return e; }
    hipEvent_t e;
    (void)hipEventCreate(&e);
    return e;
}
}

static int gemm(const mebt_model* m, GemmParams p, hipStream_t st) {
    if (p.K <= 0) {
        if (p.c_f32 && !p.beta && p.M > 0 && p.N > 0 && p.epilogue == EPI_NONE && !p.bias)
            MEBT_HIP_CHECK(hipMemset2DAsync(p.C, (size_t)p.ldc * 4, 0, (size_t)p.N * 4, p.M, st));
        else if (p.M > 0 && p.N > 0) { mebt_set_error("gemm: K = 0 with a fused epilogue is not supported"); return MEBT_ESHAPE; }
        return MEBT_OK;
    }
    p.scratch = m->ctx.tune.flush ? &m->ctx.tune : nullptr;
    ProfRec r;
    const bool prof = g_prof_on && p.M > 0 && p.N > 0;
    if (prof) {
        r.a = get_event(); r.b = get_event(); r.flops = 2.0 * p.M * p.N * p.K;
        r.tag = 'g'; r.dims[0] = p.M; r.dims[1] = p.N; r.dims[2] = p.K; r.dims[3] = p.a_kc; r.dims[4] = p.b_kc; r.dims[5] = p.epilogue; r.dims[6] = p.c_f32;
        const double esz = m->d.dtype == MEBT_BF16 ? 2.0 : 4.0, csz = (p.c_f32 || m->d.dtype == MEBT_F32) ? 4.0 : 2.0;
        r.bytes = ((double)p.M * p.K + (double)p.N * p.K) * esz + (double)p.M * p.N * (csz * (p.C ? 1 : 0) + (p.C2 ? esz : 0) + (p.aux ? esz : 0));
        (void)hipEventRecord(r.a, st);
    }
    const int rc = launch_gemm(p, m->d.dtype, st);
    if (prof) { (void)hipEventRecord(r.b, st); g_prof.push_back(r); }
    return rc;
}

static int gemm_pair(const mebt_model* m, const GemmParams& p0_in, const GemmParams& p1_in, hipStream_t st) {
    GemmParams p0 = p0_in, p1 = p1_in;
    if (m->d.dtype != MEBT_BF16 || p0.K <= 0 || p1.K <= 0 || p0.M <= 0 || p1.M <= 0) {
        if (int rc = gemm(m, p0, st)) return rc;
        return gemm(m, p1, st);
    }
    p0.scratch = p1.scratch = m->ctx.tune.flush ? &m->ctx.tune : nullptr;
    ProfRec r;
    if (g_prof_on) {
        r.a = get_event(); r.b = get_event(); r.flops = 2.0 * p0.M * p0.N * p0.K + 2.0 * p1.M * p1.N * p1.K;
        r.tag = 'p'; r.dims[0] = p0.M; r.dims[1] = p0.N; r.dims[2] = p0.K; r.dims[3] = p1.M; r.dims[4] = p1.N; r.dims[5] = p1.K; r.dims[6] = p0.b_kc;
        r.bytes = 0;
        for (const GemmParams* q : {&p0, &p1})
            r.bytes += ((double)q->M * q->K + (double)q->N * q->K) * 2.0 + (double)q->M * q->N * (2.0 * (q->C ? 1 : 0) + (q->aux ? 2.0 : 0));
        (void)hipEventRecord(r.a, st);
    }
    const int rc = launch_gemm_pair(p0, p1, m->d.dtype, st);
    if (g_prof_on) { (void)hipEventRecord(r.b, st); g_prof.push_back(r); }
    return rc;
}

extern "C" int mebt_profile_enable(int32_t on) {
    g_prof_on = on != 0;
    for (auto& r : g_prof) { g_ev_pool.push_back(r.a); g_ev_pool.push_back(r.b); }
    g_prof.clear();
    return MEBT_OK;
}
extern "C" int mebt_profile_read(int32_t family, double* launches, double* total_ms, double* total_flops) {
    double ms = 0, fl = 0, n = 0;
    const int kind = family >= 2 ? family : 0;
    for (auto& r : g_prof) {
        if (r.kind != kind) continue;
        MEBT_HIP_CHECK(hipEventSynchronize(r.b));
        float t = 0;
        MEBT_HIP_CHECK(hipEventElapsedTime(&t, r.a, r.b));
        ms += t; fl += family >= 1 ? r.bytes : r.flops;
        n += 1;
    }
    *launches = n; *total_ms = ms; *total_flops = fl;
// ... 144 lines not shown
}

static void mode_shape(const mebt_model* m, int mode, int NC, int NT, int& NQ, int& NK) {
    const int NS = m->d.n_latent;
    switch (mode) {
        case MEBT_MODE_LATENT_ENC: NQ = NS; NK = NC; break;
        case MEBT_MODE_LATENT_SELF: NQ = NS; NK = NS; break;
        case MEBT_MODE_LATENT_DEC: NQ = NT; NK = NS; break;
        case MEBT_MODE_MASKGIT: NQ = NC + NT; NK = NC + NT; break;
        default: NQ = NS; NK = NS + NT; break;
    }
}

static void carve(const mebt_model* m, Carve& c, FwdCtx& x, int B, int NC, int NT, int training) {
    const int64_t d = m->d.n_embd, e = m->esz(), NS = m->d.n_latent, H = m->d.n_head, V = m->d.vocab;
    if (m->d.dtype == MEBT_BF16) {
        const int64_t fb = m->tune_flush ? (int64_t)MEBT_TUNE_FLUSH_BYTES : 16;
        x.tune.flush = c.take(fb); x.tune.flush_bytes = (size_t)fb;
        x.tune.splitk = (float*)c.take((int64_t)MEBT_TUNE_SPLITK_BYTES); x.tune.splitk_bytes = MEBT_TUNE_SPLITK_BYTES;
    } else {
        x.tune = {nullptr, 0, nullptr, 0};
    }
    x.sos0 = c.take(B * NS * d * e);
    x.ctx = c.take((int64_t)B * NC * d * e);
    x.tgt0 = c.take((int64_t)B * NT * d * e);
    x.ci32 = training ? nullptr : (int32_t*)c.take((int64_t)B * NC * 4);
    x.L.assign(m->d.n_layer, LayerAct());
    const int64_t layer_base = c.off;
    int64_t layer_max = c.off;
    void* pingS[2] = {nullptr, nullptr};
    void* pingT[2] = {nullptr, nullptr};
    if (!training) {
        pingS[0] = c.take(B * NS * d * e); pingS[1] = c.take(B * NS * d * e);
        pingT[0] = c.take((int64_t)B * NT * d * e); pingT[1] = c.take((int64_t)B * NT * d * e);
    }
    for (int i = 0; i < m->d.n_layer; ++i)
        if (m->d.modes[i] == MEBT_MODE_MASKGIT) {
            x.L[i].c_out = c.take((int64_t)B * NC * d * e);
            x.L[i].t_out = c.take((int64_t)B * NT * d * e);
        }
    const int64_t after_ping = c.off;
    int nS = 0, nT = 0;
    for (int i = 0; i < m->d.n_layer; ++i) {
        LayerAct& a = x.L[i];
        const int mode = m->d.modes[i];
        mode_shape(m, mode, NC, NT, a.NQ, a.NK);
        const int64_t Mq = (int64_t)B * a.NQ, Mk = (int64_t)B * a.NK;
        if (!training) c.off = after_ping;
        a.qn = c.take(Mq * d * e);
        a.mean1q = (float*)c.take(Mq * 4); a.rstd1q = (float*)c.take(Mq * 4);
        if (mode == MEBT_MODE_LATENT_SELF || mode == MEBT_MODE_MASKGIT) {
            a.kn = a.qn; a.mean1k = a.mean1q; a.rstd1k = a.rstd1q;
            a.q = c.take(Mq * 3 * d * e);
            a.k = (char*)a.q + d * e; a.v = (char*)a.q + 2 * d * e;
            a.ldqkv_q = 3 * d; a.ldqkv_k = 3 * d;
        } else {
            a.kn = c.take(Mk * d * e);
            a.mean1k = (float*)c.take(Mk * 4); a.rstd1k = (float*)c.take(Mk * 4);
            a.q = c.take(Mq * d * e);
            a.k = c.take(Mk * 2 * d * e); a.v = (char*)a.k + d * e;
            a.ldqkv_q = d; a.ldqkv_k = 2 * d;
        }
        a.att = c.take(Mq * d * e);
        a.lse = (float*)c.take((int64_t)B * H * a.NQ * 4);
        a.dmask = (training && m->d.attn_pdrop > 0.f && m->d.dtype == MEBT_BF16 && d / H == 64 && m->attn_bits)
                      ? (uint16_t*)c.take((int64_t)mebt_attn_dmask_bytes(B, (int)H, a.NQ, a.NK)) : nullptr;
        a.x = c.take(Mq * d * e);
        a.mean2 = (float*)c.take(Mq * 4); a.rstd2 = (float*)c.take(Mq * 4);
        a.hn = c.take(Mq * d * e);
        a.pre = training ? c.take(Mq * 4 * d * e) : nullptr;
        a.u = c.take(Mq * 4 * d * e);
        if (training || mode == MEBT_MODE_MASKGIT) a.out = c.take(Mq * d * e);
        else a.out = (mode == MEBT_MODE_LATENT_DEC) ? pingT[(nT++) & 1] : pingS[(nS++) & 1];
        if (c.off > layer_max) layer_max = c.off;
    }
    (void)layer_base;
    c.off = layer_max;
    const int64_t R = (int64_t)B * NT;
    x.hf = c.take(R * d * e);
    x.meanf = (float*)c.take(R * 4); x.rstdf = (float*)c.take(R * 4);
    x.logits_ws = nullptr;
    if (training) {
        x.row_lse = (float*)c.take(R * 4); x.row_loss = (float*)c.take(R * 4); x.row_rank = (int*)c.take(R * 4);
        x.loss_out = (double*)c.take(32);
        int64_t Mmax = (int64_t)B * (NS + NT);
        if ((int64_t)B * NC > Mmax) Mmax = (int64_t)B * NC;
        if (m->has_maskgit && (int64_t)B * (NC + NT) > Mmax) Mmax = (int64_t)B * (NC + NT);
        x.g_cat = m->has_maskgit ? c.take((int64_t)B * (NC + NT) * d * e) : nullptr;
        x.g_S = c.take(B * NS * d * e);
        x.g_T = c.take(R * d * e);
        x.g_C = (float*)c.take((int64_t)B * NC * d * 4);
        x.dlogits = c.take(R * V * e);
        x.dhf = c.take(R * d * e);
        x.datt = c.take(Mmax * d * e);
        for (int k = 0; k < 2; ++k) {
            FwdCtx::Scratch& s = x.sc[k];
            s.d4 = c.take(Mmax * 4 * d * e);
            s.dh = c.take(Mmax * d * e);
            s.dx = c.take(Mmax * d * e);
            s.dqkv_q = c.take(Mmax * 3 * d * e);
            s.dqkv_k = c.take(Mmax * 2 * d * e);
            s.dqn = c.take(Mmax * d * e);
            s.dkn = c.take(Mmax * d * e);
            s.dout_m = c.take(Mmax * d * e);
            s.dx_m = m->d.resid_pdrop > 0.f ? c.take(Mmax * d * e) : nullptr;
        }
        x.delta = (float*)c.take((int64_t)B * H * (m->has_maskgit && NC > NS ? NC + NT : NS + NT) * 4);
    }
}

extern "C" int64_t mebt_workspace_bytes(const mebt_model* m, int32_t B, int32_t NC, int32_t NT, int32_t training) {
    if (!m || B < 0 || NC < 0 || NT < 0) return -1;
    Carve c{reinterpret_cast<char*>((uintptr_t)1 << 30), 0};
    FwdCtx x;
    carve(m, c, x, B, NC, NT, training);
    return c.off + 256;
}

static GemmParams gp(const void* A, const void* Bm, void* C, int M, int N, int K, int lda, int ldb, int ldc, int a_kc, int b_kc) {
    GemmParams p;
    memset(&p, 0, sizeof(p));
    p.A = A; p.B = Bm; p.C = C; p.M = M; p.N = N; p.K = K; p.lda = lda; p.ldb = ldb; p.ldc = ldc; p.a_kc = a_kc; p.b_kc = b_kc;
    p.split_k = 1;
    return p;
}

static int ln_fwd(const mebt_model* m, const void* x, void* y, int64_t gw, int64_t gb, float* mean, float* rstd, int rows,
                  int seg, int seg_stride, int seg_off, hipStream_t st) {
    LnFwdParams p;
    p.x = x; p.y = y; p.gamma = m->P + gw; p.beta = m->P + gb; p.mean = mean; p.rstd = rstd;
    p.rows = rows; p.d = m->d.n_embd; p.seg = seg; p.seg_stride = seg_stride; p.seg_off = seg_off;
    return launch_ln_fwd(p, m->d.dtype, st);
}

#define RC(expr) do { int _rc = (expr); if (_rc) return _rc; } while (0)

static int pf_level() {
    static const int lv = [] { const char* e = getenv("MEBT_GEMM_PREFETCH"); return e ? atoi(e) : 1; }();
    return lv;
}
static void set_pf(const mebt_model* m, GemmParams& p, int64_t w_off, int64_t n_elems) {
    if (pf_level() < 1 || m->d.dtype != MEBT_BF16 || w_off < 0 || n_elems <= 0) return;
    p.pf = m->Wop(w_off);
    p.pf_bytes = (unsigned)(n_elems * 2 > 0x7FFFFFFF ? 0x7FFFFFFF : n_elems * 2);
}
static void set_pf2(const mebt_model* m, GemmParams& p, const void* lo, const void* hi) {
    if (pf_level() < 2 || m->d.dtype != MEBT_BF16 || !lo || !hi || hi <= lo) return;
    const size_t n = (const char*)hi - (const char*)lo;
    p.pf2 = lo;
    p.pf2_bytes = (unsigned)(n > 0x7FFFFFFFull ? 0x7FFFFFFFull : n);
}
static void pf2_tail(const mebt_model* m, GemmParams& p, const LayerAct& a) { set_pf2(m, p, a.x, (const char*)a.out); }
static void pf2_head(const mebt_model* m, GemmParams& p, const LayerAct& a) { set_pf2(m, p, a.qn, (const char*)a.x); }

static int fw_wait(const mebt_model* m, int layer, hipStream_t st) {
    for (const auto& w : m->fw_waits)
        if (w.first == layer) {
            ProfRec r;
            if (g_prof_on) { r.a = get_event(); r.b = get_event(); r.flops = layer; r.bytes = 0; r.kind = 4; (void)hipEventRecord(r.a, st); }
            MEBT_HIP_CHECK(hipStreamWaitEvent(st, w.second, 0));
            if (g_prof_on) { (void)hipEventRecord(r.b, st); g_prof.push_back(r); }
        }
    return MEBT_OK;
}
static bool fw_pending(const mebt_model* m, int layer) {
    for (const auto& w : m->fw_waits)
        if (w.first == layer) return true;
// ... 149 lines not shown
        ap.drop = make_drop(dropout_seed, 16 * i + SITE_ATTN, p_att);
        ap.dmask = (p_att > 0.f && training) ? a.dmask : nullptr;
        RC(launch_attn_fwd(ap, dt, st));
        {
            GemmParams p = gp(a.att, m->Wop(o.wp), a.x, Mq, d, d, d, d, d, 1, 1);
            p.bias = m->P + o.bp; p.epilogue = EPI_RESID; p.aux = a.qn; p.ld_aux = d;
            p.drop = make_drop(dropout_seed, 16 * i + SITE_PROJ, p_res);
            set_pf(m, p, o.w1, (int64_t)4 * d * d);
            RC(gemm(m, p, st));
        }
        RC(ln_fwd(m, a.x, a.hn, o.ln2w, o.ln2b, a.mean2, a.rstd2, Mq, 0, 0, 0, st));
        {
            GemmParams p = gp(a.hn, m->Wop(o.w1), a.pre, Mq, 4 * d, d, d, d, 4 * d, 1, 1);
            p.bias = m->P + o.b1; p.epilogue = EPI_GELU; p.C2 = a.u;
            set_pf(m, p, o.w2, (int64_t)4 * d * d);
            RC(gemm(m, p, st));
        }
        {
            GemmParams p = gp(a.u, m->Wop(o.w2), a.out, Mq, d, 4 * d, 4 * d, 4 * d, d, 1, 1);
            p.bias = m->P + o.b2; p.epilogue = EPI_RESID; p.aux = a.x; p.ld_aux = d;
            p.drop = make_drop(dropout_seed, 16 * i + SITE_MLP, p_res);
            if (fw_pending(m, i + 1)) {}
            else if (i + 1 < m->d.n_layer) set_pf(m, p, m->lo[i + 1].wq, (int64_t)3 * d * d);
            else set_pf(m, p, m->head_w, (int64_t)V * d);
            RC(gemm(m, p, st));
        }
        if (mode == MEBT_MODE_LATENT_DEC) Tv = a.out;
        else if (mode == MEBT_MODE_MASKGIT) {
            const int f32 = dt == MEBT_F32;
            RC(launch_copy_rows(a.out, a.c_out, (long)B * NC, d, f32, f32, NC, NC + NT, 0, 0, 0, 0, st));
            RC(launch_copy_rows(a.out, a.t_out, (long)B * NT, d, f32, f32, NT, NC + NT, NC, 0, 0, 0, st));
            Cv = a.c_out; Tv = a.t_out;
        } else Sv = a.out;
    }
    x.S_final = Sv; x.T_final = Tv;
    RC(ln_fwd(m, Tv, x.hf, m->lnf_w, m->lnf_b, x.meanf, x.rstdf, B * NT, 0, 0, 0, st));
    RC(fw_wait(m, m->d.n_layer, st));
    {
        GemmParams p = gp(x.hf, m->Wop(m->head_w), logits, B * NT, V, d, d, d, V, 1, 1);
        p.c_f32 = logits_lp ? 0 : 1;
        RC(gemm(m, p, st));
    }
    m->fw_waits.clear();
    x.valid = training != 0;
    x.loss_done = false;
    x.dlogits_ready = false;
    return MEBT_OK;
}

extern "C" int mebt_forward(mebt_model* m, void* ws, int64_t ws_bytes, int32_t B, int32_t N, int32_t NC, int32_t NT,
                            const int64_t* x_ids, const int64_t* ci, const int64_t* ti, float* logits,
                            int32_t training, uint64_t dropout_seed, mebt_stream_t stream) {
    return forward_impl(m, ws, ws_bytes, B, N, NC, NT, x_ids, ci, ti, nullptr, logits, training, dropout_seed, stream);
}

extern "C" int64_t mebt_kvcache_bytes(const mebt_model* m, int32_t B, int32_t N) {
    if (!m || B <= 0 || N <= 0) return -1;
    int n_enc = 0;
    for (int i = 0; i < m->d.n_layer; ++i) n_enc += m->d.modes[i] == MEBT_MODE_LATENT_ENC;
    return (int64_t)n_enc * B * N * 2 * m->d.n_embd * 2;
}
extern "C" int mebt_forward_kvcache(mebt_model* m, void* ws, int64_t ws_bytes, int32_t B, int32_t N, int32_t NC, int32_t NT,
                                    const int64_t* x_ids, const int64_t* ci, const int64_t* ti, void* logits, int32_t flags,
                                    void* kv_cache, const int64_t* dirty, int32_t ND, mebt_stream_t stream) {
    if (!kv_cache) { mebt_set_error("forward_kvcache: null cache"); return MEBT_EINVAL; }
    if (flags & ~4) { mebt_set_error("forward_kvcache: inference only (flags: 0 or 4)"); return MEBT_EINVAL; }
    const KvCacheArgs kv{kv_cache, dirty, ND};
    return forward_impl(m, ws, ws_bytes, B, N, NC, NT, x_ids, ci, ti, nullptr, reinterpret_cast<float*>(logits), flags, 0, stream, &kv);
}

extern "C" int mebt_gpt_forward(mebt_model* m, void* ws, int64_t ws_bytes, int32_t B, int32_t NC, int32_t NT,
                                const float* sos, const float* contexts, const float* targets, float* logits, mebt_stream_t stream) {
    const float* e[3] = {sos, contexts, targets};
    return forward_impl(m, ws, ws_bytes, B, 1, NC, NT, nullptr, nullptr, nullptr, e, logits, 0, 0, stream);
}

extern "C" int mebt_gpt_forward_train(mebt_model* m, void* ws, int64_t ws_bytes, int32_t B, int32_t NC, int32_t NT, const float* sos,
                                      const float* contexts, const float* targets, float* logits, int32_t dropout, uint64_t dropout_seed,
                                      mebt_stream_t stream) {
    const float* e[3] = {sos, contexts, targets};
    return forward_impl(m, ws, ws_bytes, B, 1, NC, NT, nullptr, nullptr, nullptr, e, logits, 1 | (dropout ? 2 : 0), dropout_seed, stream);
}

static int loss_impl(mebt_model* m, void* ws, const float* logits, double* out4, bool with_grad, float loss_scale, mebt_stream_t stream) {
    if (!m || !m->ctx.valid || m->ctx.ws != ws) { mebt_set_error("loss: no training-mode forward on this workspace"); return MEBT_EINVAL; }
    FwdCtx& x = m->ctx;
    if (!x.x_ids) { mebt_set_error("loss: the last forward ran on caller-embedded inputs (no token ids to score against)"); return MEBT_EINVAL; }
    if (!out4) out4 = x.loss_out;
    x.loss_done = true;
    CeParams p;
    p.logits = logits; p.x_ids = x.x_ids; p.ti = x.ti; p.rows = x.B * x.NT; p.V = m->d.vocab; p.B = x.B; p.N = x.N; p.NT = x.NT;
    p.label_smoothing = m->d.label_smoothing; p.row_lse = x.row_lse; p.row_loss = x.row_loss; p.row_rank = x.row_rank; p.out = out4;
    x.dlogits_ready = false;
    if (with_grad && x.dlogits && ce_fwd_can_fuse_grad(p.V)) {
        p.dlogits = x.dlogits; p.grad_scale = loss_scale; p.dl_bf16 = m->d.dtype == MEBT_BF16;
        x.dlogits_ready = true; x.dlogits_scale = loss_scale;
    }
    return launch_ce_fwd(p, S(stream));
}
extern "C" int mebt_loss(mebt_model* m, void* ws, const float* logits, double* out4, mebt_stream_t stream) {
    return loss_impl(m, ws, logits, out4, false, 0.f, stream);
}
extern "C" int mebt_loss_with_grad(mebt_model* m, void* ws, const float* logits, double* out4, float loss_scale, mebt_stream_t stream) {
    return loss_impl(m, ws, logits, out4, true, loss_scale, stream);
}

static int ln_bwd(const mebt_model* m, const void* x, const void* dy, const void* dy2, int64_t gw, int64_t gb, const float* mean,
                  const float* rstd, void* dx, int dx_f32, int acc, int rows, int seg, int seg_stride, int seg_off, hipStream_t st,
                  const void* dx_add = nullptr) {
    LnBwdParams p;
    p.x = x; p.dy = dy; p.dy2 = dy2; p.dx_add = dx_add; p.gamma = m->P + gw; p.mean = mean; p.rstd = rstd; p.dx = dx; p.dx_f32 = dx_f32;
    p.dx_accumulate = acc; p.dgamma = m->gP + gw; p.dbeta = m->gP + gb; p.rows = rows; p.d = m->d.n_embd;
    p.seg = seg; p.seg_stride = seg_stride; p.seg_off = seg_off;
    return launch_ln_bwd(p, m->d.dtype, st);
}

static int wgrad(const mebt_model* m, const void* dY, int ld_dy, const void* X, int ld_x, int64_t w_off, int n_out, int k_in, int tokens, hipStream_t st) {
    GemmParams p = gp(dY, X, m->gW + w_off, n_out, k_in, tokens, ld_dy, ld_x, k_in, 0, 0);
    p.c_f32 = 1; p.split_k = 0; p.beta = m->grad_acc ? 1 : 0;
    if (m->wire()) { p.C = (char*)m->gWb + (size_t)w_off * 2; p.c_f32 = 0; p.split_k = 1; }
    return gemm(m, p, st);
}
static int dgrad(const mebt_model* m, const void* dY, int ld_dy, int64_t w_off, void* dX, int tokens, int n_out, int k_in, int epilogue, const void* aux, int ld_aux, hipStream_t st,
                 int64_t pf_off = -1, int64_t pf_elems = 0, const LayerAct* pf2_layer = nullptr, int pf2_part = 0) {
    GemmParams p = gp(dY, m->Wop(w_off), dX, tokens, k_in, n_out, ld_dy, k_in, k_in, 1, 0);
    p.epilogue = epilogue; p.aux = aux; p.ld_aux = ld_aux;
    set_pf(m, p, pf_off, pf_elems);
    if (pf2_layer) { if (pf2_part) pf2_tail(m, p, *pf2_layer); else pf2_head(m, p, *pf2_layer); }
    return gemm(m, p, st);
}

static int head_backward_common(mebt_model* m, hipStream_t st) {
    FwdCtx& x = m->ctx;
    const int d = m->d.n_embd, V = m->d.vocab, R = x.B * x.NT;
    hipStream_t sd = st;
    if (m->use_side) {
        RC(fork_side(m, st));
        sd = m->side;
        MEBT_HIP_CHECK(hipEventRecord(m->ev_layer[0], sd));
        MEBT_HIP_CHECK(hipEventRecord(m->ev_layer[1], sd));
    }
    RC(wgrad(m, x.dlogits, V, x.hf, d, m->head_w, V, d, R, sd));
    RC(dgrad(m, x.dlogits, V, m->head_w, x.dhf, R, V, d, EPI_NONE, nullptr, 0, st, m->lo[m->d.n_layer - 1].w2, (int64_t)4 * d * d,
             &x.L[m->d.n_layer - 1], 1));
    RC(ln_bwd(m, x.T_final, x.dhf, nullptr, m->lnf_w, m->lnf_b, x.meanf, x.rstdf, x.g_T, 0, 0, R, 0, 0, 0, st));
    x.gT_defined = true; x.gS_defined = false; x.gC_defined = false; x.doutm_ready = -1; x.last_bwd_lo = m->d.n_layer;
    return join_side(m, st);
}

static int backward_prologue(mebt_model* m, void* ws, hipStream_t st) {
    if (!m || !m->ctx.valid || m->ctx.ws != ws) { mebt_set_error("backward: no training-mode forward on this workspace"); return MEBT_EINVAL; }
    if (!m->gW || !m->gP) { mebt_set_error("backward: gradient buffers not bound"); return MEBT_EINVAL; }
    const int d = m->d.n_embd;
    if (m->grad_acc) {
        if (m->fused_on) { mebt_set_error("backward: gradient accumulation and the optimizer-in-backward exclude each other"); return MEBT_EINVAL; }
        return MEBT_OK;
    }
    MEBT_HIP_CHECK(hipMemsetAsync(m->gP, 0, (size_t)m->n_p * 4, st));
    for (int i = 0; i < m->d.n_layer; ++i)
        if (!m->live[i]) {
            MEBT_HIP_CHECK(hipMemsetAsync(m->gW + m->lo[i].wq, 0, (size_t)12 * d * d * 4, st));
            if (m->wire()) MEBT_HIP_CHECK(hipMemsetAsync((char*)m->gWb + (size_t)m->lo[i].wq * 2, 0, (size_t)12 * d * d * 2, st));
        }
    return MEBT_OK;
}

extern "C" int mebt_backward_head(mebt_model* m, void* ws, const float* logits, const float* upstream, float loss_scale, mebt_stream_t stream) {
    hipStream_t st = S(stream);
    RC(backward_prologue(m, ws, st));
    FwdCtx& x = m->ctx;
    const int V = m->d.vocab, dt = m->d.dtype, R = x.B * x.NT;
    if (x.dlogits_ready && !upstream && x.dlogits_scale == loss_scale) {
        x.dlogits_ready = false;
        return head_backward_common(m, st);
    }
    if (!x.loss_done) RC(mebt_loss(m, ws, logits, nullptr, stream));
    CeBwdParams cp;
    cp.logits = logits; cp.x_ids = x.x_ids; cp.ti = x.ti; cp.row_lse = x.row_lse; cp.dlogits = x.dlogits; cp.upstream = upstream;
    cp.scale = loss_scale; cp.label_smoothing = m->d.label_smoothing; cp.rows = R; cp.V = V; cp.B = x.B; cp.N = x.N; cp.NT = x.NT;
    RC(launch_ce_bwd(cp, dt, st));
    return head_backward_common(m, st);
}

extern "C" int mebt_backward_head_dlogits(mebt_model* m, void* ws, const float* dlogits, mebt_stream_t stream) {
    hipStream_t st = S(stream);
    RC(backward_prologue(m, ws, st));
    FwdCtx& x = m->ctx;
    if (!dlogits) { mebt_set_error("backward: null dlogits"); return MEBT_EINVAL; }
    x.dlogits_ready = false;
    const size_t n = (size_t)x.B * x.NT * m->d.vocab;
    if (m->d.dtype == MEBT_BF16) RC(launch_cast_f32_to_bf16(dlogits, x.dlogits, n, st));
    else MEBT_HIP_CHECK(hipMemcpyAsync(x.dlogits, dlogits, n * 4, hipMemcpyDeviceToDevice, st));
    return head_backward_common(m, st);
}

static int fork_side(mebt_model* m, hipStream_t st) {
    MEBT_HIP_CHECK(hipEventRecord(m->ev_fork, st));
    MEBT_HIP_CHECK(hipStreamWaitEvent(m->side, m->ev_fork, 0));
    return MEBT_OK;
}
static int join_side(mebt_model* m, hipStream_t st) {
    if (!m->use_side) return MEBT_OK;
    MEBT_HIP_CHECK(hipEventRecord(m->ev_join, m->side));
    MEBT_HIP_CHECK(hipStreamWaitEvent(st, m->ev_join, 0));
    return MEBT_OK;
}

struct Leaves {
    GroupedWgrad w;
    GroupedColsum c;
    Leaves() { w.n = 0; c.n = 0; }
    void wgrad(const void* dY, int ld_dy, const void* X, int ld_x, float* C, int n_out, int k_in, int tokens, float* bias = nullptr, bool in_gemm = false) {
        GroupedWgrad::Item& it = w.g[w.n++];
        it.A = dY; it.B = X; it.C = C; it.M = n_out; it.N = k_in; it.K = tokens; it.lda = ld_dy; it.ldb = ld_x; it.ldc = k_in; it.ntx = 0;
        it.bias = in_gemm ? bias : nullptr;
        if (bias && !in_gemm) colsum(dY, tokens, n_out, ld_dy, bias);
    }
    void colsum(const void* X, int M, int N, int ldx, float* out) {
        GroupedColsum::Item& it = c.g[c.n++];
        it.X = X; it.out = out; it.M = M; it.N = N; it.ldx = ldx; it.gx = 0; it.rpb = 0;
    }
};

static int fused_adamw_slice(mebt_model* m, const float* g, int64_t n, hipStream_t st) {
    const int64_t off = g - m->gW;
    AdamWParams a;
    a.p = m->W + off; a.g = g; a.m = m->fused_mW + off; a.v = m->fused_vW + off; a.n = (size_t)n;
    a.p_bf16 = m->Wlp ? (void*)((char*)m->Wlp + off * 2) : nullptr;
    a.lr = m->fused_h.lr; a.beta1 = m->fused_h.beta1; a.beta2 = m->fused_h.beta2; a.eps = m->fused_h.eps;
    a.weight_decay = m->fused_h.weight_decay; a.bc1 = m->fused_h.bc1; a.bc2 = m->fused_h.bc2; a.grad_scale = m->fused_h.grad_scale;
    return launch_adamw(a, st);
}

static int flush_leaves(mebt_model* m, Leaves& lv, hipStream_t sd, bool with_colsum = false) {
    const int dt = m->d.dtype;
    if (with_colsum) RC(launch_colsum_grouped(lv.c, dt, sd));
    for (int i = 0; i < lv.w.n; ++i) {
        const GroupedWgrad::Item& it = lv.w.g[i];
        if (it.K <= 0 && it.M > 0 && it.N > 0 && !m->grad_acc) {
            MEBT_HIP_CHECK(hipMemset2DAsync(it.C, (size_t)it.ldc * 4, 0, (size_t)it.N * 4, it.M, sd));
            if (m->wire()) MEBT_HIP_CHECK(hipMemset2DAsync((char*)m->gWb + (size_t)(it.C - m->gW) * 2, (size_t)it.ldc * 2, 0, (size_t)it.N * 2, it.M, sd));
        }
    }
    if (dt == MEBT_BF16) {
        ProfRec r;
        const bool prof = g_prof_on;
        if (prof) {
            r.a = get_event(); r.b = get_event(); r.flops = 0; r.bytes = 0;
            r.tag = 'w'; r.dims[0] = lv.w.n;
            for (int i = 0; i < lv.w.n; ++i) {
                const GroupedWgrad::Item& it = lv.w.g[i];
                if (it.K <= 0) continue;
                r.dims[1] += it.M * it.N / 1024; if (it.K > r.dims[2]) r.dims[2] = it.K;
                r.flops += 2.0 * it.M * it.N * it.K;
                r.bytes += ((double)it.M * it.K + (double)it.N * it.K) * 2.0 + (double)it.M * it.N * (m->fused_on ? 26.0 : 4.0);
            }
            (void)hipEventRecord(r.a, sd);
        }
        lv.w.scratch = m->ctx.tune.flush ? &m->ctx.tune : nullptr;
        lv.w.beta = m->grad_acc ? 1 : 0;
        lv.w.gW = m->gW;
        lv.w.Cb = m->wire() ? m->gWb : nullptr;
        if (m->fused_on) {
            lv.w.fused = 1; lv.w.W = m->W; lv.w.gW = m->gW; lv.w.mW = m->fused_mW; lv.w.vW = m->fused_vW; lv.w.Wlp = m->Wlp;
            lv.w.opt = m->fused_h;
            for (int i = 0; i < lv.w.n; ++i) {
                const GroupedWgrad::Item& it = lv.w.g[i];
                if (it.K <= 0 && it.M > 0 && it.N > 0) RC(fused_adamw_slice(m, it.C, (int64_t)it.M * it.N, sd));
            }
        }
        const int rc = launch_wgrad_grouped(lv.w, dt, sd);
        if (prof) { (void)hipEventRecord(r.b, sd); g_prof.push_back(r); }
        return rc;
    }
    for (int i = 0; i < lv.w.n; ++i) {
        const GroupedWgrad::Item& it = lv.w.g[i];
        if (it.K > 0) {
            GemmParams p = gp(it.A, it.B, it.C, it.M, it.N, it.K, it.lda, it.ldb, it.ldc, 0, 0);
            p.c_f32 = 1; p.beta = m->grad_acc ? 1 : 0;
            RC(gemm(m, p, sd));
        }
        if (m->fused_on && it.M > 0 && it.N > 0) RC(fused_adamw_slice(m, it.C, (int64_t)it.M * it.N, sd));
    }
    return MEBT_OK;
}

static int flush_or_park(mebt_model* m, Leaves& lv, hipStream_t sd, bool side) {
    static const bool pair_on = [] { const char* e = getenv("MEBT_WGRAD_PAIR"); return !(e && e[0] == '0'); }();
    if (!pair_on || side || m->d.dtype != MEBT_BF16 || lv.w.n > MEBT_MAX_GROUP / 2) return flush_leaves(m, lv, sd);
    if (!m->pend) {
        m->pend_w = lv.w;
        m->pend = true;
        return MEBT_OK;
    }
    for (int k = 0; k < m->pend_w.n && lv.w.n < MEBT_MAX_GROUP; ++k) lv.w.g[lv.w.n++] = m->pend_w.g[k];
    m->pend = false;
    return flush_leaves(m, lv, sd);
}
static int flush_parked(mebt_model* m, hipStream_t sd) {
    if (!m->pend) return MEBT_OK;
    Leaves lv;
    lv.w = m->pend_w;
    m->pend = false;
    return flush_leaves(m, lv, sd);
}

static int backward_layer(mebt_model* m, int i, hipStream_t st) {
    FwdCtx& x = m->ctx;
    LayerAct& a = x.L[i];
    const LayerOffsets& o = m->lo[i];
    const int mode = m->d.modes[i], d = m->d.n_embd, dt = m->d.dtype, B = x.B, NS = m->d.n_latent, NT = x.NT, H = m->d.n_head;
    const int Mq = B * a.NQ, Mk = B * a.NK;
    const bool isdec = mode == MEBT_MODE_LATENT_DEC, ismg = mode == MEBT_MODE_MASKGIT;
    if (ismg ? !(x.gT_defined || x.gC_defined) : isdec ? !x.gT_defined : !x.gS_defined) return MEBT_OK;
    const bool side = m->use_side;
    hipStream_t sd = side ? m->side : st;
    FwdCtx::Scratch& sc = x.sc[i & 1];
    if (side) MEBT_HIP_CHECK(hipStreamWaitEvent(st, m->ev_layer[i & 1], 0));
    const void* dout = isdec ? x.g_T : x.g_S;
    const int f32 = dt == MEBT_F32;
    const size_t esz = m->esz();
    if (ismg) {
        const int NC = x.NC;
        if (x.gC_defined) RC(launch_copy_rows(x.g_C, x.g_cat, (long)B * NC, d, 1, f32, 0, 0, 0, NC, NC + NT, 0, st));
        else if (NC > 0) MEBT_HIP_CHECK(hipMemset2DAsync(x.g_cat, (size_t)(NC + NT) * d * esz, 0, (size_t)NC * d * esz, B, st));
        if (x.gT_defined) RC(launch_copy_rows(x.g_T, x.g_cat, (long)B * NT, d, f32, f32, 0, 0, 0, NT, NC + NT, NC, st));
        else MEBT_HIP_CHECK(hipMemset2DAsync((char*)x.g_cat + (size_t)NC * d * esz, (size_t)(NC + NT) * d * esz, 0, (size_t)NT * d * esz, B, st));
        dout = x.g_cat;
    }
    const float p_res = x.drop_on ? m->d.resid_pdrop : 0.f, p_att = x.drop_on ? m->d.attn_pdrop : 0.f;
    Leaves lv;
    if (x.doutm_ready == i) x.doutm_ready = -1;
    else if (p_res > 0.f) RC(launch_apply_dropout(dout, sc.dout_m, (size_t)Mq * d, f32, f32, make_drop(x.drop_seed, 16 * i + SITE_MLP, p_res), st));
    else MEBT_HIP_CHECK(hipMemcpyAsync(sc.dout_m, dout, (size_t)Mq * d * esz, hipMemcpyDeviceToDevice, st));
    const void* dmlp = sc.dout_m;
    static const bool bias_in_wgrad = [] { const char* e = getenv("MEBT_BIAS_IN_WGRAD"); return !(e && e[0] == '0'); }();
    const bool bg = dt == MEBT_BF16 && bias_in_wgrad;
    const int64_t dd = (int64_t)d * d;
    lv.wgrad(dmlp, d, a.u, 4 * d, m->gW + o.w2, d, 4 * d, Mq, m->gP + o.b2, bg);
    RC(dgrad(m, dmlp, d, o.w2, sc.d4, Mq, d, 4 * d, EPI_GELU_BWD, a.pre, 4 * d, st, o.w1, 4 * dd));
    lv.wgrad(sc.d4, 4 * d, a.hn, d, m->gW + o.w1, 4 * d, d, Mq, m->gP + o.b1, bg);
    RC(dgrad(m, sc.d4, 4 * d, o.w1, sc.dh, Mq, 4 * d, d, EPI_NONE, nullptr, 0, st, o.wp, dd, &a, 0));
    const void* dproj = sc.dx;
    {
        LnBwdParams p;
        p.x = a.x; p.dy = sc.dh; p.dy2 = nullptr; p.dx_add = dout; p.gamma = m->P + o.ln2w; p.mean = a.mean2; p.rstd = a.rstd2;
        p.dx = sc.dx; p.dx_f32 = f32; p.dx_accumulate = 0; p.dgamma = m->gP + o.ln2w; p.dbeta = m->gP + o.ln2b;
        p.rows = Mq; p.d = d; p.seg = 0; p.seg_stride = 0; p.seg_off = 0;
        if (p_res > 0.f) {
            p.dx2 = sc.dx_m; p.drop2 = make_drop(x.drop_seed, 16 * i + SITE_PROJ, p_res);
            dproj = sc.dx_m;
        }
        if (side) RC(fork_side(m, st));
        RC(launch_ln_bwd(p, dt, st, sd));
    }
    lv.wgrad(dproj, d, a.att, d, m->gW + o.wp, d, d, Mq, m->gP + o.bp, bg);
    RC(dgrad(m, dproj, d, o.wp, x.datt, Mq, d, d, EPI_NONE, nullptr, 0, st, o.wq, 3 * dd));
    AttnParams ap;
    memset(&ap, 0, sizeof(ap));
    ap.q = a.q; ap.k = a.k; ap.v = a.v; ap.o = a.att; ap.lse = a.lse; ap.B = B; ap.H = H; ap.NQ = a.NQ; ap.NK = a.NK; ap.HD = d / H;
    ap.ldq = a.ldqkv_q; ap.ldk = a.ldqkv_k; ap.ldv = a.ldqkv_k; ap.ldo = d;
    ap.d_o = x.datt; ap.lddo = d; ap.delta = x.delta;
    ap.drop = make_drop(x.drop_seed, 16 * i + SITE_ATTN, p_att);
    ap.dmask = p_att > 0.f ? a.dmask : nullptr;
    if (mode == MEBT_MODE_LATENT_SELF || ismg) {
        ap.dq = sc.dqkv_q; ap.dk = (char*)sc.dqkv_q + (size_t)d * esz; ap.dv = (char*)sc.dqkv_q + (size_t)2 * d * esz;
        ap.lddq = ap.lddk = ap.lddv = 3 * d;
// ... 43 lines not shown
        RC(flush_or_park(m, lv, sd, side));
        if (mode == MEBT_MODE_LATENT_ENC) {
            ln1(a.q_in, sc.dqn, nullptr, a.mean1q, a.rstd1q, x.g_S, 0, 0, Mq, 0, 0, 0);
            if (Mk > 0) {
                ln1(a.k_in, sc.dkn, nullptr, a.mean1k, a.rstd1k, x.g_C, 1, x.gC_defined ? 1 : 0, Mk, 0, 0, 0);
                x.gC_defined = true;
            }
        } else if (mode == MEBT_MODE_LATENT_DEC) {
            ln1(a.q_in, sc.dqn, nullptr, a.mean1q, a.rstd1q, x.g_T, 0, 0, Mq, 0, 0, 0);
            ln1(a.k_in, sc.dkn, nullptr, a.mean1k, a.rstd1k, x.g_S, 0, x.gS_defined ? 1 : 0, Mk, 0, 0, 0);
            x.gS_defined = true;
        } else {
            ln1(a.q_in, sc.dkn, sc.dqn, a.mean1k, a.rstd1k, x.g_S, 0, 0, B * NS, NS, NS + NT, 0);
            ln1(a.k_in, sc.dkn, nullptr, a.mean1k, a.rstd1k, x.g_T, 0, x.gT_defined ? 1 : 0, B * NT, NT, NS + NT, NS);
            x.gT_defined = true;
        }
    }
    static const int fuse_doutm = [] { const char* e = getenv("MEBT_FUSE_DOUTM"); return e ? atoi(e) : 1; }();
    if (i > 0 && !side && p_res > 0.f && fuse_doutm && m->d.modes[i - 1] != MEBT_MODE_MASKGIT) {
        const bool below_dec = m->d.modes[i - 1] == MEBT_MODE_LATENT_DEC;
        const void* want = below_dec ? x.g_T : x.g_S;
        int k = -1;
        for (int j = 0; j < nj; ++j) if (lj[j].dx == want) k = j;
        if (k >= 0 && !lj[k].dx_f32) {
            lj[k].dx2 = x.sc[(i - 1) & 1].dout_m;
            lj[k].drop2 = make_drop(x.drop_seed, 16 * (i - 1) + SITE_MLP, p_res);
            x.doutm_ready = i - 1;
        }
    }
    RC(launch_ln_bwd_multi(lj, nj, dt, st, sd, &lv.c));
    if (side) MEBT_HIP_CHECK(hipEventRecord(m->ev_layer[i & 1], sd));
    return MEBT_OK;
}

extern "C" int mebt_backward_layers(mebt_model* m, void* ws, int32_t layer_hi, int32_t layer_lo, mebt_stream_t stream) {
    if (!m || !m->ctx.valid || m->ctx.ws != ws) { mebt_set_error("backward: no training-mode forward on this workspace"); return MEBT_EINVAL; }
    if (layer_hi >= m->d.n_layer || layer_lo < 0 || layer_lo > layer_hi) { mebt_set_error("backward_layers: bad layer range"); return MEBT_EINVAL; }
    if (m->ctx.last_bwd_lo != layer_hi + 1) m->ctx.doutm_ready = -1;
    m->pend = false;
    for (int i = layer_hi; i >= layer_lo; --i) RC(backward_layer(m, i, S(stream)));
    RC(flush_parked(m, S(stream)));
    m->ctx.last_bwd_lo = layer_lo;
    return join_side(m, S(stream));
}

static int input_grad_dropout(mebt_model* m, hipStream_t st);

extern "C" int mebt_gpt_backward(mebt_model* m, void* ws, const float* dlogits, float* d_sos, float* d_contexts, float* d_targets,
                                 mebt_stream_t stream) {
    RC(mebt_backward_head_dlogits(m, ws, dlogits, stream));
    RC(mebt_backward_layers(m, ws, m->d.n_layer - 1, 0, stream));
    FwdCtx& x = m->ctx;
    hipStream_t st = S(stream);
    RC(input_grad_dropout(m, st));
    const int d = m->d.n_embd, f32 = m->d.dtype == MEBT_F32;
    struct { float* dst; const void* src; bool defined; long rows; int src_f32; } o[3] = {
        {d_sos, x.g_S, x.gS_defined, (long)x.B * m->d.n_latent, f32}, {d_contexts, x.g_C, x.gC_defined, (long)x.B * x.NC, 1},
        {d_targets, x.g_T, x.gT_defined, (long)x.B * x.NT, f32}};
    for (auto& t : o) {
        if (!t.dst || t.rows <= 0) continue;
        if (t.defined) RC(launch_copy_rows(t.src, t.dst, t.rows, d, t.src_f32, 1, 0, 0, 0, 0, 0, 0, st));
        else MEBT_HIP_CHECK(hipMemsetAsync(t.dst, 0, (size_t)t.rows * d * 4, st));
    }
    return MEBT_OK;
}

static int input_grad_dropout(mebt_model* m, hipStream_t st) {
    FwdCtx& x = m->ctx;
    if (x.drop_on && m->d.embd_pdrop > 0.f) {
        const int f32 = m->d.dtype == MEBT_F32;
        const size_t dd = m->d.n_embd;
        const float pe = m->d.embd_pdrop;
        if (x.gS_defined) RC(launch_apply_dropout(x.g_S, x.g_S, (size_t)x.B * m->d.n_latent * dd, f32, f32, make_drop(x.drop_seed, SITE_EMB_SOS, pe), st));
        if (x.gT_defined) RC(launch_apply_dropout(x.g_T, x.g_T, (size_t)x.B * x.NT * dd, f32, f32, make_drop(x.drop_seed, SITE_EMB_TGT, pe), st));
        if (x.gC_defined) RC(launch_apply_dropout(x.g_C, x.g_C, (size_t)x.B * x.NC * dd, 1, 1, make_drop(x.drop_seed, SITE_EMB_CTX, pe), st));
    }
    return MEBT_OK;
}

extern "C" int mebt_backward_embed(mebt_model* m, void* ws, mebt_stream_t stream) {
    if (!m || !m->ctx.valid || m->ctx.ws != ws) { mebt_set_error("backward: no training-mode forward on this workspace"); return MEBT_EINVAL; }
    FwdCtx& x = m->ctx;
    if (!x.x_ids) { mebt_set_error("backward_embed: the last forward ran on caller-embedded inputs: use mebt_gpt_backward"); return MEBT_EINVAL; }
    RC(input_grad_dropout(m, S(stream)));
    EmbedBwdParams p;
    p.x_ids = x.x_ids; p.ci = x.ci; p.ti = x.ti;
    p.g_ctx = x.g_C; p.g_tgt = x.g_T; p.g_sos = x.g_S;
    p.g_tok_emb = m->gP + m->tok_emb; p.g_pos_emb = m->gP + m->pos_emb; p.g_mask_emb = m->gP + m->mask_emb; p.g_sos_emb = m->gP + m->sos_emb;
    p.B = x.B; p.N = x.N; p.NC = x.gC_defined ? x.NC : 0; p.NT = x.gT_defined ? x.NT : 0; p.NS = x.gS_defined ? m->d.n_latent : 0; p.d = m->d.n_embd;
    if (p.NC != x.NC && x.NC > 0) {
        mebt_set_error("backward_embed: contexts without a live latent_enc block are not supported");
        return MEBT_EINVAL;
    }
    ProfRec r;
    if (g_prof_on) {
        r.a = get_event(); r.b = get_event(); r.kind = 3; r.flops = 0;
        const double dd = p.d;
        r.bytes = (double)p.B * ((double)p.NC * dd * 4 + ((double)p.NT + p.NS) * dd * m->esz() + ((double)2 * p.NC + p.NT) * dd * 4);
        (void)hipEventRecord(r.a, S(stream));
    }
    const int rc = launch_embed_bwd(p, m->d.dtype, S(stream));
    if (g_prof_on) { (void)hipEventRecord(r.b, S(stream)); g_prof.push_back(r); }
    return rc;
}

extern "C" int mebt_adamw_range(mebt_model* m, float* mW, float* vW, float* mP, float* vP, float lr, float beta1, float beta2,
                                float eps, float weight_decay, int32_t step, float grad_scale, int32_t kind, int32_t layer_hi,
                                int32_t layer_lo, mebt_stream_t stream) {
    if (!m || !m->W || !m->gW || !m->gP) { mebt_set_error("adamw: model / gradients not bound"); return MEBT_EINVAL; }
    if (step < 1) { mebt_set_error("adamw: step must be >= 1"); return MEBT_EINVAL; }
    if (kind == 1 && (layer_hi >= m->d.n_layer || layer_lo < 0 || layer_lo > layer_hi)) { mebt_set_error("adamw: bad layer range"); return MEBT_EINVAL; }
    hipStream_t st = S(stream);
    AdamWParams a;
    a.lr = lr; a.beta1 = beta1; a.beta2 = beta2; a.eps = eps; a.grad_scale = grad_scale;
    a.bc1 = (float)(1.0 - pow((double)beta1, step)); a.bc2 = (float)(1.0 - pow((double)beta2, step));
    const int d = m->d.n_embd;
    auto run = [&](float* p, const float* g, float* mm, float* vv, void* lp, int64_t off, int64_t n, float wd) -> int {
        a.p = p + off; a.g = g + off; a.m = mm + off; a.v = vv + off; a.n = (size_t)n; a.weight_decay = wd;
        a.p_bf16 = lp ? (void*)((char*)lp + off * 2) : nullptr;
        return launch_adamw(a, st);
    };
    if (kind == 1 || kind == 3 || kind == 4) {
        const int lo = kind != 1 ? 0 : layer_lo, hi = kind != 1 ? m->d.n_layer - 1 : layer_hi;
        int i = lo;
        while (i <= hi) {
            if (!m->live[i]) { ++i; continue; }
            int j = i;
            while (j + 1 <= hi && m->live[j + 1]) ++j;
            if (kind != 4) RC(run(m->W, m->gW, mW, vW, m->Wlp, m->lo[i].wq, (int64_t)(j - i + 1) * 12 * d * d, weight_decay));
            RC(run(m->P, m->gP, mP, vP, nullptr, m->lo[i].ln1w, (int64_t)(j - i + 1) * 13 * d, 0.f));
            i = j + 1;
        }
    }
    if (kind == 0 || kind == 3 || kind == 4) RC(run(m->W, m->gW, mW, vW, m->Wlp, m->head_w, (int64_t)m->d.vocab * d, weight_decay));
    if (kind == 2 || kind == 3 || kind == 4) {
        const int64_t tail_n = (m->tok_live ? m->n_p : m->tok_emb) - m->lnf_w;
        RC(run(m->P, m->gP, mP, vP, nullptr, m->lnf_w, tail_n, 0.f));
    }
    return MEBT_OK;
}

static int adamw_slice_impl(mebt_model* m, int32_t which, int64_t off, int64_t n, const void* grad, int32_t grad_bf16, int32_t pieces, float* mW,
                            float* vW, float* mP, float* vP, float lr, float beta1, float beta2, float eps, float weight_decay,
                            int32_t step, float grad_scale, mebt_stream_t stream) {
    if (!m || !m->W || !grad) { mebt_set_error("adamw_slice: model not bound / null gradient"); return MEBT_EINVAL; }
    if (pieces < 1 || (pieces > 1 && !grad_bf16)) { mebt_set_error("adamw_slice: pieces >= 1, several pieces only of bf16 gradients"); return MEBT_EINVAL; }
    if (step < 1) { mebt_set_error("adamw: step must be >= 1"); return MEBT_EINVAL; }
    const int64_t total = which == 0 ? m->n_w : m->n_p;
    if (off < 0 || n < 0 || off + n > total || (off % 4) || (n % 4)) { mebt_set_error("adamw_slice: bad range (multiples of 4 inside the buffer)"); return MEBT_EINVAL; }
    hipStream_t st = S(stream);
    AdamWParams a;
    a.lr = lr; a.beta1 = beta1; a.beta2 = beta2; a.eps = eps; a.grad_scale = grad_scale; a.g_bf16 = grad_bf16 ? 1 : 0;
    a.g_pieces = pieces; a.g_stride = (size_t)n;
    a.bc1 = (float)(1.0 - pow((double)beta1, step)); a.bc2 = (float)(1.0 - pow((double)beta2, step));
    a.weight_decay = which == 0 ? weight_decay : 0.f;
    const int d = m->d.n_embd;
    const int64_t gsz = grad_bf16 ? 2 : 4;
    auto run = [&](int64_t lo, int64_t hi) -> int {
        const int64_t a0 = lo > off ? lo : off, a1 = hi < off + n ? hi : off + n;
        if (a1 <= a0) return MEBT_OK;
        float* pb = which == 0 ? m->W : m->P;
        a.p = pb + a0; a.m = (which == 0 ? mW : mP) + a0; a.v = (which == 0 ? vW : vP) + a0; a.n = (size_t)(a1 - a0);
        a.g = reinterpret_cast<const float*>(reinterpret_cast<const char*>(grad) + (a0 - off) * gsz);
        a.p_bf16 = (which == 0 && m->Wlp) ? (void*)((char*)m->Wlp + a0 * 2) : nullptr;
        return launch_adamw(a, st);
    };
    for (int i = 0; i < m->d.n_layer; ++i) {
        if (!m->live[i]) continue;
        if (which == 0) RC(run(m->lo[i].wq, m->lo[i].wq + (int64_t)12 * d * d));
        else RC(run(m->lo[i].ln1w, m->lo[i].ln1w + (int64_t)13 * d));
    }
    if (which == 0) RC(run(m->head_w, m->n_w));
    else RC(run(m->lnf_w, m->tok_live ? m->n_p : m->tok_emb));
    return MEBT_OK;
}
extern "C" int mebt_adamw_slice(mebt_model* m, int32_t which, int64_t off, int64_t n, const void* grad, int32_t grad_bf16, float* mW,
                                float* vW, float* mP, float* vP, float lr, float beta1, float beta2, float eps, float weight_decay,
                                int32_t step, float grad_scale, mebt_stream_t stream) {
    return adamw_slice_impl(m, which, off, n, grad, grad_bf16, 1, mW, vW, mP, vP, lr, beta1, beta2, eps, weight_decay, step, grad_scale, stream);
}
extern "C" int mebt_adamw_slice_pieces(mebt_model* m, int32_t which, int64_t off, int64_t n, const void* grad_pieces, int32_t pieces, float* mW,
                                       float* vW, float* mP, float* vP, float lr, float beta1, float beta2, float eps, float weight_decay,
                                       int32_t step, float grad_scale, mebt_stream_t stream) {
    return adamw_slice_impl(m, which, off, n, grad_pieces, 1, pieces, mW, vW, mP, vP, lr, beta1, beta2, eps, weight_decay, step, grad_scale, stream);
}

extern "C" int mebt_model_bind_wire_grads(mebt_model* m, void* gWb) {
    if (!m) { mebt_set_error("bind_wire_grads: null model"); return MEBT_EINVAL; }
    m->gWb = gWb;
    return MEBT_OK;
}

extern "C" int mebt_model_set_grad_accumulate(mebt_model* m, int32_t on) {
    if (!m) { mebt_set_error("set_grad_accumulate: null model"); return MEBT_EINVAL; }
    m->grad_acc = on != 0;
    return MEBT_OK;
}

extern "C" int mebt_model_set_fused_adamw(mebt_model* m, float* mW, float* vW, float lr, float beta1, float beta2, float eps,
                                          float weight_decay, int32_t step, float grad_scale) {
    if (!m) { mebt_set_error("set_fused_adamw: null model"); return MEBT_EINVAL; }
    if (step <= 0) { m->fused_on = false; return MEBT_OK; }
    if (!mW || !vW || !m->W || !m->gW) { mebt_set_error("set_fused_adamw: optimizer state / model not bound"); return MEBT_EINVAL; }
    m->fused_on = true; m->fused_mW = mW; m->fused_vW = vW;
    m->fused_h = {lr, beta1, beta2, eps, weight_decay, (float)(1.0 - pow((double)beta1, step)), (float)(1.0 - pow((double)beta2, step)), grad_scale};
    return MEBT_OK;
}

extern "C" int mebt_adamw_step(mebt_model* m, float* mW, float* vW, float* mP, float* vP, float lr, float beta1, float beta2,
                               float eps, float weight_decay, int32_t step, float grad_scale, mebt_stream_t stream) {
    return mebt_adamw_range(m, mW, vW, mP, vP, lr, beta1, beta2, eps, weight_decay, step, grad_scale, 3, 0, 0, stream);
}

extern "C" int mebt_debug_dropout_mask(uint64_t seed, uint32_t site, float p, int64_t n, float* out, mebt_stream_t stream) {
    if (!out || n < 0 || (n % 4)) { mebt_set_error("dropout_mask: bad arguments (n must be a multiple of 4)"); return MEBT_EINVAL; }
    return launch_apply_dropout(out, out, (size_t)n, 1, 1, make_drop(seed, site, p), S(stream));
}
```

mebt_amd/csrc/kernels.h:

```cpp
#pragma once
#include <hip/hip_runtime.h>
#include <stdint.h>
#include <cstdlib>
#include "common.h"

enum { MEBT_F32 = 0, MEBT_BF16 = 1 };
enum { SITE_ATTN = 0, SITE_PROJ = 1, SITE_MLP = 2, SITE_EMB_SOS = 0xFFFF0, SITE_EMB_CTX = 0xFFFF1, SITE_EMB_TGT = 0xFFFF2 };
static inline DropCfg make_drop(uint64_t seed, uint32_t site, float p) {
    DropCfg d;
    d.seed = seed; d.site = site;
    d.thresh = p > 0.f ? (uint32_t)((double)p * 65536.0 + 0.5) : 0u;
    d.inv_keep = d.thresh ? (float)(65536.0 / (65536.0 - d.thresh)) : 1.0f;
    d.small = 0;
    d.base32 = site * 0x632BE5ABu + (uint32_t)(seed >> 32);
    return d;
}
static inline void drop_mark_small(DropCfg& d, uint64_t n_elems) {
    static const bool on = [] { const char* e = getenv("MEBT_DROP_SMALL"); return !(e && e[0] == '0'); }();
    d.small = (on && n_elems < (1ull << 33)) ? 1u : 0u;
}
enum { EPI_NONE = 0, EPI_GELU = 1, EPI_RESID = 2, EPI_GELU_BWD = 3, EPI_ADAMW = 4  };

struct GemmScratch { void* flush; size_t flush_bytes; float* splitk; size_t splitk_bytes; };
#define MEBT_TUNE_FLUSH_BYTES (384ull << 20)
#define MEBT_TUNE_SPLITK_BYTES (112ull << 20)

struct GemmParams {
    const void* A;
    const void* B;
    void* C;
    void* C2;
    const float* bias;
    const void* aux;
    int M, N, K;
    int lda, ldb, ldc, ld_aux;
    int a_kc, b_kc;
    int epilogue;
    int c_f32;
    int beta;
    int split_k;
    long slab = 0;
    DropCfg drop;
    float* opt_p = nullptr; float* opt_m = nullptr; float* opt_v = nullptr; void* opt_lp = nullptr;
    AdamWHyper opt = {0, 0, 0, 0, 0, 1, 1, 1};
    const GemmScratch* scratch = nullptr;
    const void* pf = nullptr;
    unsigned pf_bytes = 0;
    const void* pf2 = nullptr;
    unsigned pf2_bytes = 0;
    unsigned* pf_sink = nullptr;
    int coarse_m = 0;
    int narrow_store = 0;
    float* rowsum_a = nullptr;
    unsigned long long* stamps = nullptr;
};
int launch_gemm(const GemmParams& p, int dtype, hipStream_t stream);
int launch_gemm_pair(const GemmParams& p0, const GemmParams& p1, int dtype, hipStream_t stream);
struct GemmPair { GemmParams p[2]; int tiles0; int ntx[2]; };
#define MEBT_MAX_GROUP 12
struct GroupedWgrad {
    int n;
    int tile_start[MEBT_MAX_GROUP + 1];
    struct Item { const void* A; const void* B; float* C; int M, N, K, lda, ldb, ldc, ntx; float* bias = nullptr; } g[MEBT_MAX_GROUP];
    int fused = 0;
    float* W = nullptr; float* gW = nullptr; float* mW = nullptr; float* vW = nullptr; void* Wlp = nullptr;
    AdamWHyper opt = {0, 0, 0, 0, 0, 1, 1, 1};
    int beta = 0;
    void* Cb = nullptr;
    const GemmScratch* scratch = nullptr;
};
int launch_wgrad_grouped(GroupedWgrad& w, int dtype, hipStream_t stream);
struct GroupedColsum {
    int n;
    int blk_start[MEBT_MAX_GROUP + 1];
    struct Item { const void* X; float* out; int M, N, ldx, gx, rpb; } g[MEBT_MAX_GROUP];
};
int launch_colsum_grouped(GroupedColsum& c, int dtype, hipStream_t stream);
int gemm_init_attributes();
extern "C" int32_t mebt_gemm_autotune_enabled(void);
void mebt_gemm_force_split(int s);

struct EmbedParams {
    const int64_t* x_ids;
    const int64_t* ci;
    const int64_t* ti;
    const float* tok_emb;
    const float* pos_emb;
    const float* mask_emb;
    const float* sos_emb;
    void* sos;
    void* ctx;
    void* tgt;
    int B, N, NC, NT, NS, d, vocab, block_size;
    DropCfg drop;
};
int launch_embed_fwd(const EmbedParams& p, int dtype, hipStream_t stream);
struct EmbedBwdParams {
    const int64_t* x_ids; const int64_t* ci; const int64_t* ti;
    const float* g_ctx;
    const void* g_tgt;
    const void* g_sos;
    float* g_tok_emb; float* g_pos_emb; float* g_mask_emb; float* g_sos_emb;
    int B, N, NC, NT, NS, d;
};
int launch_embed_bwd(const EmbedBwdParams& p, int dtype, hipStream_t stream);

struct LnFwdParams {
    const void* x; void* y; const float* gamma; const float* beta;
    float* mean; float* rstd;
    int rows, d; int seg, seg_stride, seg_off;
};
int launch_ln_fwd(const LnFwdParams& p, int dtype, hipStream_t stream);
constexpr int MEBT_LN_MAXJ = 3;
int launch_ln_fwd_multi(const LnFwdParams* jobs, int n, int dtype, hipStream_t stream);
struct LnBwdParams {
    const void* x;
    const void* dy;
    const void* dy2;
    const void* dx_add;
    const float* gamma; const float* mean; const float* rstd;
    void* dx; int dx_f32; int dx_accumulate;
    float* dgamma; float* dbeta;
    int rows, d; int seg, seg_stride, seg_off;
    void* dx2 = nullptr;
    DropCfg drop2 = {0, 0, 0, 1.0f};
};
int launch_ln_bwd(const LnBwdParams& p, int dtype, hipStream_t stream, hipStream_t param_stream = nullptr);
struct GroupedColsum;
int launch_ln_bwd_multi(const LnBwdParams* jobs, int n, int dtype, hipStream_t stream, hipStream_t param_stream = nullptr, const GroupedColsum* colsums = nullptr);

int launch_apply_dropout(const void* src, void* dst, size_t n, int src_f32, int dst_f32, const DropCfg& d, hipStream_t stream);

int launch_copy_rows(const void* src, void* dst, long rows, int d, int src_f32, int dst_f32, int s_seg, int s_stride, int s_off,
                     int d_seg, int d_stride, int d_off, hipStream_t stream);

int launch_cast_i64_i32(const int64_t* src, int32_t* dst, size_t n, hipStream_t stream);
int launch_index_rows(const void* src, void* dst, const int64_t* idx, int B, int n, int npos, int row_bytes, int scatter, hipStream_t stream);

int launch_colsum(const void* X, int M, int N, int ldx, float* out, int dtype, hipStream_t stream);

struct CeParams {
    const float* logits;
    const int64_t* x_ids;
    const int64_t* ti;
    int rows, V, B, N, NT;
    float label_smoothing;
    float* row_lse;
    float* row_loss;
    int* row_rank;
    double* out;
    void* dlogits = nullptr;
    float grad_scale = 0.f;
    int dl_bf16 = 0;
};
int launch_ce_fwd(const CeParams& p, hipStream_t stream);
inline bool ce_fwd_can_fuse_grad(int V) { return V == 16384; }
struct CeBwdParams {
    const float* logits; const int64_t* x_ids; const int64_t* ti; const float* row_lse;
    void* dlogits;
    const float* upstream;
    float scale;
    float label_smoothing;
    int rows, V, B, N, NT;
};
int launch_ce_bwd(const CeBwdParams& p, int dtype, hipStream_t stream);

struct AdamWParams {
    float* p; const float* g; float* m; float* v; void* p_bf16;
    size_t n; float lr, beta1, beta2, eps, weight_decay, bc1, bc2, grad_scale;
    int g_bf16 = 0;
    int g_pieces = 1;
    size_t g_stride = 0;
};
int launch_adamw(const AdamWParams& p, hipStream_t stream);
int launch_cast_f32_to_bf16(const float* src, void* dst, size_t n, hipStream_t stream);

struct AttnParams {
    const void* q; const void* k; const void* v; void* o; float* lse;
    int B, H, NQ, NK, HD; int ldq, ldk, ldv, ldo;
    const void* d_o; void* dq; void* dk; void* dv; float* delta; int lddo, lddq, lddk, lddv;
    DropCfg drop;
    uint16_t* dmask = nullptr;
    const int32_t* kidx = nullptr;
    int kidx_rows = 0;
    int xcd_order = 0;
};
__host__ __device__ static inline int mebt_attn_dmask_tiles(int NK) { return 4 * ((NK + 255) / 256); }
static inline size_t mebt_attn_dmask_bytes(int B, int H, int NQ, int NK) { return (size_t)B * H * NQ * mebt_attn_dmask_tiles(NK) * 8; }
int launch_attn_fwd(const AttnParams& p, int dtype, hipStream_t stream);
int launch_attn_bwd(const AttnParams& p, int dtype, hipStream_t stream);
void mebt_attn_force_generic(int on);
void mebt_attn_set_legacy(int bits);
int mebt_attn_legacy();
int launch_attn_block_order_probe(int T, int X, int H, int xcd, int32_t* pos_to_id, hipStream_t stream);
bool attn_fwd_can_gather(int dtype, int HD);

struct SampleParams {
    const float* logits;
    int logits_bf16 = 0;
    int icdf = 0;
    const float* noise;
    uint64_t noise_seed = 0;
    float temperature; int top_k; float top_p;
    int64_t* ids;
    float* score;
    float* probs;
    int rows, V;
    float* kth = nullptr;
    const int64_t* probs_ti = nullptr;
    int probs_N = 0, probs_NT = 0;
};
int launch_sample(const SampleParams& p, hipStream_t stream);
int launch_scatter_ids(int64_t* x, const int64_t* ti, const int64_t* ids, int B, int N, int NT, hipStream_t stream);
struct NextMaskParams {
    const int64_t* ci; const int64_t* ti; const float* score; const float* noise;
    float ctemp; int n_new; int B, NC, NT;
    int64_t* new_ci;
    int64_t* new_ti;
};
int launch_next_mask(const NextMaskParams& p, hipStream_t stream);
```

mebt_amd/engine.py:

```python
import ctypes as C
import math
import os

import torch

from . import _lib
from ._lib import check, ptr, cur_stream


def layer_param_names(i):
    p = f"transformer.blocks.{i}."
    w = [p + "attn.query.weight", p + "attn.key.weight", p + "attn.value.weight", p + "attn.proj.weight",
         p + "mlp.0.weight", p + "mlp.2.weight"]
    s = [p + "ln1.weight", p + "ln1.bias", p + "ln2.weight", p + "ln2.bias", p + "attn.query.bias",
         p + "attn.key.bias", p + "attn.value.bias", p + "attn.proj.bias", p + "mlp.0.bias", p + "mlp.2.bias"]
    return w, s


def flat_layout(n_layer, has_sos=True):
    W, P = [], []
    for i in range(n_layer):
        w, s = layer_param_names(i)
        W += w
        P += s
# ... 93 lines not shown
            raise _lib.MebtError("bad workspace query")
        if self.ws is None or self.ws.numel() < need or self.ws.device != self.device:
            self.ws = torch.empty(int(need * 1.05) + 4096, dtype=torch.uint8, device=self.device)
        return self.ws

    def forward(self, x_ids, ci, ti, training=False, logits=None, dropout_seed=0, dropout=True, logits_bf16=False):
        assert x_ids.dtype == torch.long and ti.dtype == torch.long
        x_ids, ti = x_ids.contiguous(), ti.contiguous()
        ci = ci.contiguous() if ci is not None else None
        B, N = x_ids.shape
        NC = 0 if ci is None else ci.shape[1]
        NT = ti.shape[1]
        self.sync_lowp()
        ws = self.workspace(B, NC, NT, training)
        logits_bf16 = bool(logits_bf16) and not training and self.dtype == "bf16"
        if logits is None:
            logits = torch.empty(B, NT, self.vocab, device=self.device, dtype=torch.bfloat16 if logits_bf16 else torch.float32)
        check(self.lib.mebt_forward(self.h, ptr(ws), ws.numel(), B, N, NC, NT, ptr(x_ids),
                                    ptr(ci) if NC > 0 else None, ptr(ti), ptr(logits),
                                    (1 | (2 if dropout else 0)) if training else (4 if logits_bf16 else 0),
                                    int(dropout_seed), cur_stream()))
        self._keep = (x_ids, ci, ti, logits)
        if training:
            self.generation += 1
        return logits

    def new_kv_cache(self, B, N):
        nbytes = self.lib.mebt_kvcache_bytes(self.h, int(B), int(N))
        if nbytes <= 0:
            return None
        return torch.empty(int(nbytes), dtype=torch.uint8, device=self.device)

    def forward_cached(self, x_ids, ci, ti, cache, dirty, logits_bf16=False):
        assert self.dtype == "bf16" and x_ids.dtype == torch.long
        x_ids, ti, ci = x_ids.contiguous(), ti.contiguous(), ci.contiguous()
        dirty = ci if dirty is None else dirty.contiguous()
        B, N = x_ids.shape
        NC, NT, ND = ci.shape[1], ti.shape[1], dirty.shape[1]
        self.sync_lowp()
        ws = self.workspace(B, NC, NT, False)
        logits = torch.empty(B, NT, self.vocab, device=self.device, dtype=torch.bfloat16 if logits_bf16 else torch.float32)
        check(self.lib.mebt_forward_kvcache(self.h, ptr(ws), ws.numel(), B, N, NC, NT, ptr(x_ids), ptr(ci) if NC > 0 else None, ptr(ti),
                                            ptr(logits), 4 if logits_bf16 else 0, ptr(cache), ptr(dirty) if ND > 0 else None, ND, cur_stream()))
        self._keep = (x_ids, ci, ti, logits, dirty)
        return logits

    def gpt_forward(self, sos, contexts, targets):
        sos, contexts, targets = (t.to(self.device, torch.float32).contiguous() for t in (sos, contexts, targets))
        B, NC, NT = sos.shape[0], contexts.shape[1], targets.shape[1]
        self.sync_lowp()
        ws = self.workspace(B, NC, NT, False)
        logits = torch.empty(B, NT, self.vocab, device=self.device, dtype=torch.float32)
        check(self.lib.mebt_gpt_forward(self.h, ptr(ws), ws.numel(), B, NC, NT, ptr(sos), ptr(contexts) if NC > 0 else None,
                                        ptr(targets), ptr(logits), cur_stream()))
        return logits

    def gpt_forward_train(self, sos, contexts, targets, dropout_seed=0, dropout=True):
        sos, contexts, targets = (t.to(self.device, torch.float32).contiguous() for t in (sos, contexts, targets))
        B, NC, NT = sos.shape[0], contexts.shape[1], targets.shape[1]
        self.sync_lowp()
        ws = self.workspace(B, NC, NT, True)
        logits = torch.empty(B, NT, self.vocab, device=self.device, dtype=torch.float32)
        check(self.lib.mebt_gpt_forward_train(self.h, ptr(ws), ws.numel(), B, NC, NT, ptr(sos), ptr(contexts) if NC > 0 else None,
                                              ptr(targets), ptr(logits), 1 if dropout else 0, int(dropout_seed), cur_stream()))
        self._keep = (sos, contexts, targets, logits)
        self.generation += 1
        return logits

    def gpt_backward(self, dlogits, shapes):
        self.ensure_grads()
        dlogits = dlogits.to(torch.float32).contiguous()
        outs = [torch.empty(s, device=self.device, dtype=torch.float32) for s in shapes]
        check(self.lib.mebt_gpt_backward(self.h, ptr(self.ws), ptr(dlogits), *[ptr(o) if o.numel() else None for o in outs], cur_stream()))
        return outs

    def loss_stats(self, logits, grad_scale=None):
        out = torch.empty(4, device=self.device, dtype=torch.float64)
        if grad_scale is None:
            check(self.lib.mebt_loss(self.h, ptr(self.ws), ptr(logits), ptr(out), cur_stream()))
        else:
            check(self.lib.mebt_loss_with_grad(self.h, ptr(self.ws), ptr(logits), ptr(out), float(grad_scale), cur_stream()))
        return out

    def backward_head(self, logits, loss_scale, upstream=None):
        self.ensure_grads()
        check(self.lib.mebt_backward_head(self.h, ptr(self.ws), ptr(logits), ptr(upstream), float(loss_scale), cur_stream()))

    def backward_layers(self, hi, lo):
        check(self.lib.mebt_backward_layers(self.h, ptr(self.ws), hi, lo, cur_stream()))

    def backward_embed(self):
        check(self.lib.mebt_backward_embed(self.h, ptr(self.ws), cur_stream()))

    def backward(self, logits, loss_scale, upstream=None, between=None, dlogits=None, bucket_layers=4):
        if dlogits is not None:
            self.ensure_grads()
            dlogits = dlogits.contiguous()
            check(self.lib.mebt_backward_head_dlogits(self.h, ptr(self.ws), ptr(dlogits), cur_stream()))
        else:
            self.backward_head(logits, loss_scale, upstream)
        if between:
            between("head", None, None)
        sizes = list(bucket_layers) if isinstance(bucket_layers, (list, tuple)) else None
        hi, nb = self.n_layer - 1, 0
        while hi >= 0:
            step = max(1, int(sizes[min(nb, len(sizes) - 1)] if sizes else bucket_layers))
            nb += 1
            lo = max(0, hi - step + 1)
            self.backward_layers(hi, lo)
            if between:
                between("layers", hi, lo)
            hi = lo - 1
        self.backward_embed()
        if between:
            between("embed", None, None)

    def _adam_state(self):
        if self.adam is None:
            self.adam = [torch.zeros_like(self.W), torch.zeros_like(self.W), torch.zeros_like(self.P), torch.zeros_like(self.P)]
        return self.adam

    def adamw_range(self, kind, hi, lo, lr, weight_decay, step, betas=(0.9, 0.95), eps=1e-8, grad_scale=1.0, stream=None):
        mW, vW, mP, vP = self._adam_state()
        k = {"head": 0, "layers": 1, "embed": 2, "all": 3, "rest": 4}[kind]
        check(self.lib.mebt_adamw_range(self.h, ptr(mW), ptr(vW), ptr(mP), ptr(vP), float(lr), float(betas[0]), float(betas[1]),
                                        float(eps), float(weight_decay), int(step), float(grad_scale), k, int(hi or 0), int(lo or 0),
                                        stream if stream is not None else cur_stream()))

    def adamw_slice(self, which, off, n, grad, lr, weight_decay, step, betas=(0.9, 0.95), eps=1e-8, grad_scale=1.0, stream=None, pieces=1):
        mW, vW, mP, vP = self._adam_state()
        if pieces > 1:
            assert grad.dtype == torch.bfloat16 and grad.numel() == pieces * n
            check(self.lib.mebt_adamw_slice_pieces(self.h, int(which), int(off), int(n), ptr(grad), int(pieces),
                                                   ptr(mW), ptr(vW), ptr(mP), ptr(vP), float(lr), float(betas[0]), float(betas[1]), float(eps),
                                                   float(weight_decay), int(step), float(grad_scale), stream if stream is not None else cur_stream()))
            return
        check(self.lib.mebt_adamw_slice(self.h, int(which), int(off), int(n), ptr(grad), 1 if grad.dtype == torch.bfloat16 else 0,
                                        ptr(mW), ptr(vW), ptr(mP), ptr(vP), float(lr), float(betas[0]), float(betas[1]), float(eps),
                                        float(weight_decay), int(step), float(grad_scale), stream if stream is not None else cur_stream()))

    def cast_bf16(self, src, dst):
        check(self.lib.mebt_op_cast_bf16(ptr(src), ptr(dst), src.numel(), cur_stream()))

    def set_fused_adamw(self, lr=0.0, weight_decay=0.0, step=0, betas=(0.9, 0.95), eps=1e-8, grad_scale=1.0):
        mW, vW, _, _ = self._adam_state()
        check(self.lib.mebt_model_set_fused_adamw(self.h, ptr(mW), ptr(vW), float(lr), float(betas[0]), float(betas[1]), float(eps),
                                                  float(weight_decay), int(step), float(grad_scale)))

    def enable_wire_grads(self, on=True):
        if on and self.dtype == "bf16":
            if self.gWb is None:
                self.gWb = torch.zeros(self.n_w, device=self.device, dtype=torch.bfloat16)
            check(self.lib.mebt_model_bind_wire_grads(self.h, ptr(self.gWb)))
        else:
            self.gWb = None
            check(self.lib.mebt_model_bind_wire_grads(self.h, None))

    def set_forward_waits(self, waits):
        import ctypes as C
        waits = list(waits)
        n = len(waits)
        layers = (C.c_int32 * max(1, n))(*[int(l) for l, _ in waits])
        evs = (C.c_void_p * max(1, n))(*[int(e.cuda_event) for _, e in waits])
        check(self.lib.mebt_model_set_forward_waits(self.h, n, layers, evs))
        self._fw_events = [e for _, e in waits]

# ... 36 lines not shown
```

mebt_amd/trainer.py:

```python
import os
import random

import numpy as np
import torch

from .frames import RawVideoBatch
from .parallel import GradReducer, pick_concurrent_stream


class TrainLoop:
    def __init__(self, model, reducer=None, max_steps=0, overlap_optimizer=None, fused_optimizer=None,
                 accumulate_grad_batches=1):
        if overlap_optimizer is None:
            multi = reducer is not None and getattr(reducer, "active", reducer.world_size > 1)
            overlap_optimizer = os.environ.get("MEBT_OVERLAP_OPT", "1" if multi else "0") != "0"
        """model: mebt_amd.transformer.Net2NetTransformer on its GPU, with learning_rate /
        warmup_steps / weight_decay / cosine_lr set (train_transformer.py:54-66)."""
        self.model = model
        self.accum = max(1, int(accumulate_grad_batches))
        self._micro = 0
        self.native = model._ensure_native()
        self.native.ensure_grads()
        self.reducer = reducer or GradReducer(world_size=1)
        model._reducer = self.reducer
        self.step_count = 0
        model.trainer.max_steps = max_steps
        self.reducer.broadcast_parameters(self.native)
        self.opt_stream = pick_concurrent_stream(torch.cuda.current_stream(), device=self.native.device) if overlap_optimizer else None
        self.sync_tune = bool(self.reducer.active and os.environ.get("MEBT_DP_SYNC_TUNE", "1") != "0")
        if self.sync_tune:
            self.reducer.lead_tuning()
        self.hold_tune_sync = False
        self.sharded = bool(self.reducer.active and self.reducer.mode == "sharded")
        wire = (self.sharded and self.reducer.wire == "bf16" and self.accum == 1 and model.compute_dtype == "bf16"
                and os.environ.get("MEBT_DP_WIRE_GRADS", "1") != "0")
        if self.sharded:
            self.native._adam_state()
        self.wire_grads = bool(wire)
        self.native.enable_wire_grads(wire)
        if fused_optimizer is None:
            fused_optimizer = os.environ.get("MEBT_FUSED_ADAMW", "1") != "0" and model.compute_dtype == "bf16"
        self.fused_optimizer = bool(fused_optimizer) and not self.reducer.active
        if self.accum > 1:
            self.fused_optimizer = False

    def step(self, x, indices, t=None, flush=False):
        m, nm, red = self.model, self.native, self.reducer
        if isinstance(x, RawVideoBatch):
            x = x.to_video()
        if x.dtype != torch.long:
            x = m.encode_to_z(x)[1]
        B = x.shape[0]
        x_ids = x.reshape(B, -1)
        if t is None:
            t = m._draw_t(False)
        prior_t = m.t_prior(m.t_lengths, m.global_step)
        ci, ti, seq_len = m.mask_sampler.divide_indices(indices, torch.tensor(float(t)), m.t_lengths, prior_t)
        ci, ti = ci.contiguous(), ti.contiguous()
        ratio = float(seq_len - ci.shape[1]) / float(seq_len)
        scale = 1.0 / (B * seq_len * ratio ** m.config.avg_loss)
        lr = m.learning_rate * m.lr_scale()
        logits = nm.forward(x_ids, ci, ti, training=True, dropout_seed=m._next_seed())
        fused_ce = os.environ.get("MEBT_FUSED_CE", "1") != "0"
        stats = nm.loss_stats(logits, grad_scale=(scale / self.accum if self.accum > 1 else scale) if fused_ce else None)
        if self.accum > 1:
            self._micro += 1
            nm.set_grad_accumulate(self._micro > 1)
            if self._micro < self.accum and not flush:
                nm.backward(logits, scale / self.accum)
                nm.set_grad_accumulate(False)
                return torch.cat([stats, (stats[0] * scale).reshape(1)])
            self._micro = 0
            bwd_scale = scale / self.accum
        else:
            bwd_scale = scale
        self.step_count += 1
        if self.fused_optimizer:
            nm.set_fused_adamw(lr, m.weight_decay, self.step_count)
            nm.backward(logits, scale)
            nm.set_fused_adamw(step=0)
            nm.adamw_range("rest", None, None, lr, m.weight_decay, self.step_count)
        elif self.opt_stream is None and not self.sharded:
            nm.backward(logits, bwd_scale, between=lambda s, hi, lo: red.bucket_ready(nm, s, hi, lo))
            red.wait()
            nm.adamw_step(lr, m.weight_decay, self.step_count, grad_scale=red.grad_scale)
        elif self.sharded:
            opt = self.opt_stream
            update = lambda s, hi, lo: red.reduce_update(nm, s, hi, lo, lr, m.weight_decay, self.step_count, opt_stream=opt)
            if self.step_count == 1:
                done = []
                nm.backward(logits, bwd_scale, bucket_layers=red.bucket_plan(nm.n_layer), between=lambda s, hi, lo: done.append((s, hi, lo)))
                for stage in done:
                    update(*stage)
            else:
                nm.backward(logits, bwd_scale, bucket_layers=red.bucket_plan(nm.n_layer), between=update)
            if red.defer:
                red.gather_deferred(nm, opt)
            else:
                red.finish(opt)
        else:
            main, opt = torch.cuda.current_stream(), self.opt_stream

            def bucket(stage, hi, lo):
                works = red.bucket_ready(nm, stage, hi, lo)
                opt.wait_stream(main)
                with torch.cuda.stream(opt):
                    for w in works:
                        w.wait()
                    nm.adamw_range(stage, hi, lo, lr, m.weight_decay, self.step_count, grad_scale=red.grad_scale)

            nm.backward(logits, bwd_scale, between=bucket)
            red.pending = []
            main.wait_stream(opt)
        if self.accum > 1:
            nm.set_grad_accumulate(False)
        if self.sync_tune and not self.hold_tune_sync and red.tune_sync_due(self.step_count):
            red.sync_tune_table()
        m.trainer.global_step += 1
        m.global_step += 1
        return torch.cat([stats, (stats[0] * scale).reshape(1)])

    def consolidate(self, optimizer_state=True):
        self.reducer.consolidate(self.native, optimizer_state=optimizer_state)

    def state_dict(self):
        m = self.model
        return {"adam": [t.detach().cpu().clone() for t in self.native._adam_state()], "step_count": self.step_count,
                "global_step": m.global_step, "trainer_global_step": m.trainer.global_step, "seed_ctr": m._seed_ctr,
                "rng": {"python": random.getstate(), "numpy": np.random.get_state(), "torch": torch.get_rng_state()}}

    def load_state_dict(self, sd, restore_rng=True):
        m = self.model
        for dst, src in zip(self.native._adam_state(), sd["adam"]):
            dst.copy_(src)
        self.step_count = int(sd["step_count"])
        m.global_step = int(sd["global_step"])
        m.trainer.global_step = int(sd["trainer_global_step"])
        m._seed_ctr = int(sd["seed_ctr"])
        if restore_rng and "rng" in sd:
            random.setstate(sd["rng"]["python"])
            np.random.set_state(sd["rng"]["numpy"])
            torch.set_rng_state(sd["rng"]["torch"])
```

Measured before the change: 309,700 masked tokens/s (whole job).

## Fuse embed backward, gather AdamW tail segments, fold loss stats scaling

Replaces the atomic scatter embed backward with an inverse-map gather kernel that also folds embedding dropout and the mask/sos column sums into one launch. The rest-of-model AdamW updates are batched into a single multi-segment kernel. The scaled-loss stat is computed inside the CE reduce kernel, which removes a torch.cat per step. A head-weight wgrad path with AdamW fused in is added behind an env flag. Together these are meant to cut launch count and atomic traffic in the step tail, at the cost of added complexity and new kernels whose correctness has to be checked against the legacy paths.

Measured after the change: 311,300 masked tokens/s (whole job), median of 6. Within noise of the previous version (+0.5%).

```diff
diff --git a/include/mebt_hip.h b/include/mebt_hip.h
--- a/include/mebt_hip.h
+++ b/include/mebt_hip.h
@@ -53,6 +53,8 @@
                       mebt_stream_t stream);
 int mebt_loss(mebt_model* m, void* ws, const float* logits, double* out4, mebt_stream_t stream);
 int mebt_loss_with_grad(mebt_model* m, void* ws, const float* logits, double* out4, float loss_scale, mebt_stream_t stream);
+int mebt_loss_stats(mebt_model* m, void* ws, const float* logits, double* out5, double stat_scale, int32_t with_grad, float loss_scale,
+                    mebt_stream_t stream);
 int mebt_backward_head(mebt_model* m, void* ws, const float* logits, const float* upstream, float loss_scale, mebt_stream_t stream);
 int mebt_backward_head_dlogits(mebt_model* m, void* ws, const float* dlogits, mebt_stream_t stream);
 int mebt_backward_layers(mebt_model* m, void* ws, int32_t layer_hi, int32_t layer_lo, mebt_stream_t stream);
@@ -100,6 +102,10 @@
                       const float* pos_emb, const float* mask_emb, const float* sos_emb, void* sos, void* ctx, void* tgt,
                       int32_t B, int32_t N, int32_t NC, int32_t NT, int32_t NS, int32_t d, int32_t vocab,
                       int32_t block_size, mebt_stream_t stream);
+int mebt_op_embed_bwd(int32_t dtype, const int64_t* x_ids, const int64_t* ci, const int64_t* ti, float* g_ctx, void* g_tgt, void* g_sos,
+                      float* g_tok_emb, float* g_pos_emb, float* g_mask_emb, float* g_sos_emb, int32_t* inv_scratch, int32_t B, int32_t N,
+                      int32_t NC, int32_t NT, int32_t NS, int32_t d, int32_t vocab, int32_t block_size, uint64_t seed, float p_drop,
+                      int32_t legacy, mebt_stream_t stream);
 int mebt_op_sample(const float* logits, const float* noise, float temperature, int32_t top_k, float top_p, int64_t* ids,
                    float* score, float* probs, int32_t rows, int32_t V, mebt_stream_t stream);
 int mebt_op_sample_seeded(const float* logits, uint64_t seed, float temperature, int32_t top_k, float top_p, int64_t* ids,
@@ -194,6 +200,7 @@
 int mebt_debug_dropout_mask(uint64_t seed, uint32_t site, float p, int64_t n, float* out, mebt_stream_t stream);
 int mebt_debug_clock_probe(unsigned long long* out4, uint64_t ref_ticks_100mhz, mebt_stream_t stream);
 void mebt_debug_side_stream(mebt_model* m, int32_t on);
+void mebt_debug_step_edges(int32_t fused_head, int32_t rest_split);
 void mebt_debug_set_side_stream(mebt_model* m, mebt_stream_t stream);
 void mebt_debug_gemm_tile(int32_t bm, int32_t bn);
 void mebt_debug_gemm_variant(int32_t dma);
diff --git a/mebt_amd/_lib.py b/mebt_amd/_lib.py
--- a/mebt_amd/_lib.py
+++ b/mebt_amd/_lib.py
@@ -38,6 +38,7 @@
     "mebt_gpt_backward": (c_i32, [c_vp, c_vp, c_vp, c_vp, c_vp, c_vp, c_vp]),
     "mebt_loss": (c_i32, [c_vp, c_vp, c_vp, c_vp, c_vp]),
     "mebt_loss_with_grad": (c_i32, [c_vp, c_vp, c_vp, c_vp, C.c_float, c_vp]),
+    "mebt_loss_stats": (c_i32, [c_vp, c_vp, c_vp, c_vp, C.c_double, c_i32, C.c_float, c_vp]),
     "mebt_backward_head": (c_i32, [c_vp, c_vp, c_vp, c_vp, c_f32, c_vp]),
     "mebt_backward_head_dlogits": (c_i32, [c_vp, c_vp, c_vp, c_vp]),
     "mebt_backward_layers": (c_i32, [c_vp, c_vp, c_i32, c_i32, c_vp]),
@@ -56,6 +57,7 @@
     "mebt_op_attention_fwd": (c_i32, [c_i32, c_vp, c_vp, c_vp, c_vp, c_vp] + [c_i32] * 10 + [c_vp]),
     "mebt_op_attention_bwd": (c_i32, [c_i32] + [c_vp] * 10 + [c_i32] * 10 + [c_vp]),
     "mebt_op_embed_fwd": (c_i32, [c_i32] + [c_vp] * 10 + [c_i32] * 8 + [c_vp]),
+    "mebt_op_embed_bwd": (c_i32, [c_i32] + [c_vp] * 11 + [c_i32] * 8 + [C.c_uint64, c_f32, c_i32, c_vp]),
     "mebt_op_sample": (c_i32, [c_vp, c_vp, c_f32, c_i32, c_f32, c_vp, c_vp, c_vp, c_i32, c_i32, c_vp]),
     "mebt_op_sample_seeded": (c_i32, [c_vp, C.c_uint64, c_f32, c_i32, c_f32, c_vp, c_vp, c_vp, c_i32, c_i32, c_vp]),
     "mebt_op_sample_scatter": (c_i32, [c_vp, c_vp, C.c_uint64, c_f32, c_i32, c_vp, c_vp, c_vp, c_vp, c_i32, c_i32, c_i32, c_i32, c_vp]),
@@ -85,6 +87,7 @@
     "mebt_debug_dropout_mask": (c_i32, [C.c_uint64, C.c_uint32, c_f32, c_i64, c_vp, c_vp]),
     "mebt_debug_clock_probe": (c_i32, [c_vp, C.c_uint64, c_vp]),
     "mebt_debug_side_stream": (None, [c_vp, c_i32]),
+    "mebt_debug_step_edges": (None, [c_i32, c_i32]),
     "mebt_debug_set_side_stream": (None, [c_vp, c_vp]),
     "mebt_debug_gemm_tile": (None, [c_i32, c_i32]),
     "mebt_debug_gemm_variant": (None, [c_i32]),
diff --git a/mebt_amd/csrc/capi.cpp b/mebt_amd/csrc/capi.cpp
--- a/mebt_amd/csrc/capi.cpp
+++ b/mebt_amd/csrc/capi.cpp
@@ -158,6 +158,32 @@
     return launch_embed_fwd(p, dtype, S(stream));
 }
 
+extern "C" int mebt_op_embed_bwd(int32_t dtype, const int64_t* x_ids, const int64_t* ci, const int64_t* ti, float* g_ctx, void* g_tgt, void* g_sos,
+                                 float* g_tok_emb, float* g_pos_emb, float* g_mask_emb, float* g_sos_emb, int32_t* inv_scratch, int32_t B,
+                                 int32_t N, int32_t NC, int32_t NT, int32_t NS, int32_t d, int32_t vocab, int32_t block_size, uint64_t seed,
+                                 float p_drop, int32_t legacy, mebt_stream_t stream) {
+    if (int rc = check_dtype(dtype)) return rc;
+    if (!x_ids || !g_tok_emb || !g_pos_emb || !g_mask_emb || (NC > 0 && (!ci || !g_ctx)) || (NT > 0 && (!ti || !g_tgt)) || (NS > 0 && (!g_sos || !g_sos_emb)) ||
+        (!legacy && !inv_scratch)) { mebt_set_error("embed_bwd: null pointer"); return MEBT_EINVAL; }
+    if (B < 0 || N <= 0 || NC < 0 || NT < 0 || NS < 0 || d <= 0 || (d % 4) || vocab <= 0 || N > block_size) { mebt_set_error("embed_bwd: bad shape"); return MEBT_ESHAPE; }
+    const int f32 = dtype == MEBT_F32;
+    EmbedBwdParams p;
+    p.x_ids = x_ids; p.ci = ci; p.ti = ti; p.g_ctx = g_ctx; p.g_tgt = g_tgt; p.g_sos = g_sos;
+    p.g_tok_emb = g_tok_emb; p.g_pos_emb = g_pos_emb; p.g_mask_emb = g_mask_emb; p.g_sos_emb = g_sos_emb;
+    p.B = B; p.N = N; p.NC = NC; p.NT = NT; p.NS = NS; p.d = d; p.vocab = vocab; p.pos_rows = block_size; p.inv = inv_scratch;
+    p.legacy = legacy ? 1 : 0;
+    if (p_drop > 0.f) {
+        p.drop_sos = make_drop(seed, SITE_EMB_SOS, p_drop); p.drop_tgt = make_drop(seed, SITE_EMB_TGT, p_drop); p.drop_ctx = make_drop(seed, SITE_EMB_CTX, p_drop);
+        if (legacy) {
+            hipStream_t st = S(stream);
+            if (int rc = launch_apply_dropout(g_sos, g_sos, (size_t)B * NS * d, f32, f32, p.drop_sos, st)) return rc;
+            if (int rc = launch_apply_dropout(g_tgt, g_tgt, (size_t)B * NT * d, f32, f32, p.drop_tgt, st)) return rc;
+            if (int rc = launch_apply_dropout(g_ctx, g_ctx, (size_t)B * NC * d, 1, 1, p.drop_ctx, st)) return rc;
+        }
+    }
+    return launch_embed_bwd(p, dtype, S(stream));
+}
+
 extern "C" int mebt_op_sample(const float* logits, const float* noise, float temperature, int32_t top_k, float top_p, int64_t* ids,
                               float* score, float* probs, int32_t rows, int32_t V, mebt_stream_t stream) {
     if (!logits || !noise || !ids) { mebt_set_error("sample: null pointer"); return MEBT_EINVAL; }
diff --git a/mebt_amd/csrc/common.h b/mebt_amd/csrc/common.h
--- a/mebt_amd/csrc/common.h
+++ b/mebt_amd/csrc/common.h
@@ -115,6 +115,21 @@
     }
 }
 
+__device__ __forceinline__ void adamw_update4_pinned(f32x4& p, const f32x4& g, f32x4& m, f32x4& v, const AdamWHyper& a) {
+    const float step_size = a.lr / a.bc1;
+    const float inv_sqrt_bc2 = rsqrtf(a.bc2);
+    const float decay = __fmaf_rn(-a.lr, a.weight_decay, 1.0f);
+    const float c1 = __fsub_rn(1.0f, a.beta1), c2 = __fsub_rn(1.0f, a.beta2);
+#pragma unroll
+    for (int j = 0; j < 4; ++j) {
+        const float gj = __fmul_rn(g[j], a.grad_scale);
+        m[j] = __fmaf_rn(c1, gj, __fmul_rn(a.beta1, m[j]));
+        v[j] = __fmaf_rn(a.beta2, v[j], __fmul_rn(gj, __fmul_rn(c2, gj)));
+        const float denom = __fmaf_rn(sqrtf(v[j]), inv_sqrt_bc2, a.eps);
+        p[j] = __fmaf_rn(decay, p[j], -__fmul_rn(step_size, __fdiv_rn(m[j], denom)));
+    }
+}
+
 __device__ __forceinline__ uint32_t pair_hash(uint64_t seed, uint32_t site, uint64_t pair) {
     uint32_t h = ((uint32_t)pair ^ (uint32_t)seed) + ((uint32_t)(pair >> 32) + site) * 0x632BE5ABu + (uint32_t)(seed >> 32);
     h *= 0x9E3779B1u;
diff --git a/mebt_amd/csrc/elementwise.hip b/mebt_amd/csrc/elementwise.hip
--- a/mebt_amd/csrc/elementwise.hip
+++ b/mebt_amd/csrc/elementwise.hip
@@ -51,7 +51,7 @@
 }
 
 template <typename T>
-__global__ __launch_bounds__(256) void embed_bwd_kernel(const EmbedBwdParams p) {
+__global__ __launch_bounds__(256) void embed_bwd_scatter_kernel(const EmbedBwdParams p) {
     const int lane = threadIdx.x & 63;
     const long row = (long)blockIdx.x * 4 + (threadIdx.x >> 6);
     const long per_b = (long)p.NC + p.NT;
@@ -75,6 +75,113 @@
         const T* g = reinterpret_cast<const T*>(p.g_tgt) + ((size_t)b * p.NT + j0) * p.d;
         float* gp = p.g_pos_emb + (size_t)pos * p.d;
         for (int e = lane; e < p.d; e += 64) atomicAdd(gp + e, to_f32<T>(g[e]));
+    }
+}
+
+__global__ __launch_bounds__(256) void embed_inverse_map_kernel(const int64_t* ci, const int64_t* ti, int32_t* inv, int N, int NC, int NT) {
+    const int b = blockIdx.x;
+    int32_t* row = inv + (size_t)b * N;
+    for (int n = threadIdx.x; n < N; n += 256) row[n] = -1;
+    __syncthreads();
+    for (int j = threadIdx.x; j < NC; j += 256) {
+        const long pos = ci[(size_t)b * NC + j];
+        if (pos >= 0 && pos < N) row[pos] = j;
+    }
+    for (int j = threadIdx.x; j < NT; j += 256) {
+        const long pos = ti[(size_t)b * NT + j];
+        if (pos >= 0 && pos < N) row[pos] = NC + j;
+    }
+}
+
+template <typename T>
+__device__ __forceinline__ void embed_colsum_body(const T* X, int M, int N, float* out, int rpb, int gx, int bid, const DropCfg& dc) {
+    __shared__ float red[16][64 + 4];
+    const int bx = bid % gx, by = bid / gx;
+    const int cg = threadIdx.x & 15, rl = threadIdx.x >> 4;
+    const int n = bx * 64 + cg * 4;
+    const int m0 = by * rpb, m1 = min(M, m0 + rpb);
+    f32x4 acc = {0, 0, 0, 0};
+    if (n < N)
+#pragma unroll 4
+        for (int m = m0 + rl; m < m1; m += 16) {
+            const size_t i = (size_t)m * N + n;
+            f32x4 v = load4<T>(X + i);
+            if (dc.thresh) {
+                const f32x4 k = drop_keep4(dc, i);
+#pragma unroll
+                for (int j = 0; j < 4; ++j) v[j] = to_f32<T>(from_f32<T>(__fmul_rn(v[j], k[j])));
+            }
+            acc += v;
+        }
+#pragma unroll
+    for (int j = 0; j < 4; ++j) red[rl][cg * 4 + j] = acc[j];
+    __syncthreads();
+    if (threadIdx.x < 64) {
+        float t = 0.f;
+#pragma unroll
+        for (int r = 0; r < 16; ++r) t += red[r][threadIdx.x];
+        const int col = bx * 64 + threadIdx.x;
+        if (col < N) atomicAdd(out + col, t);
+    }
+}
+
+template <typename T>
+__global__ __launch_bounds__(256) void embed_bwd_kernel(const EmbedBwdParams p, int pos_blocks, int sos_start, int mask_rpb, int mask_gx, int sos_rpb, int sos_gx) {
+    const int bid = blockIdx.x;
+    if (bid >= pos_blocks) {
+        if (bid < sos_start) embed_colsum_body<T>(reinterpret_cast<const T*>(p.g_tgt), p.B * p.NT, p.d, p.g_mask_emb, mask_rpb, mask_gx, bid - pos_blocks, p.drop_tgt);
+        else embed_colsum_body<T>(reinterpret_cast<const T*>(p.g_sos), p.B, p.NS * p.d, p.g_sos_emb, sos_rpb, sos_gx, bid - sos_start, p.drop_sos);
+        return;
+    }
+    const int lane = threadIdx.x & 63;
+    const int nch = (p.d + 255) / 256;
+    const long w = (long)bid * 4 + (threadIdx.x >> 6);
+    const int n = (int)(w / nch);
+    if (n >= p.pos_rows) return;
+    const int e0 = (int)(w % nch) * 256 + lane;
+    float acc[4] = {0.f, 0.f, 0.f, 0.f};
+    if (n < p.N) {
+        for (int b = 0; b < p.B; ++b) {
+            const int slot = p.inv[(size_t)b * p.N + n];
+            if (slot < 0) continue;
+            if (slot < p.NC) {
+                const size_t base = ((size_t)b * p.NC + slot) * p.d;
+                long tok = p.x_ids[(size_t)b * p.N + n];
+                tok = tok < 0 ? 0 : (tok >= p.vocab ? p.vocab - 1 : tok);
+                float* gt = p.g_tok_emb + (size_t)tok * p.d;
+                float v[4];
+#pragma unroll
+                for (int k = 0; k < 4; ++k) {
+                    const int e = e0 + 64 * k;
+                    v[k] = e < p.d ? p.g_ctx[base + e] : 0.f;
+                    if (p.drop_ctx.thresh && e < p.d) v[k] = __fmul_rn(v[k], drop_keep(p.drop_ctx, base + e));
+                }
+#pragma unroll
+                for (int k = 0; k < 4; ++k) {
+                    const int e = e0 + 64 * k;
+                    if (e < p.d) atomicAdd(gt + e, v[k]);
+                    acc[k] += v[k];
+                }
+            } else {
+                const size_t base = ((size_t)b * p.NT + (slot - p.NC)) * p.d;
+                const T* g = reinterpret_cast<const T*>(p.g_tgt);
+#pragma unroll
+                for (int k = 0; k < 4; ++k) {
+                    const int e = e0 + 64 * k;
+                    if (e < p.d) {
+                        float v = to_f32<T>(g[base + e]);
+                        if (p.drop_tgt.thresh) v = to_f32<T>(from_f32<T>(__fmul_rn(v, drop_keep(p.drop_tgt, base + e))));
+                        acc[k] += v;
+                    }
+                }
+            }
+        }
+    }
+    float* gp = p.g_pos_emb + (size_t)n * p.d;
+#pragma unroll
+    for (int k = 0; k < 4; ++k) {
+        const int e = e0 + 64 * k;
+        if (e < p.d) gp[e] = p.accumulate ? gp[e] + acc[k] : acc[k];
     }
 }
 
@@ -579,7 +686,7 @@
     }
 }
 
-__global__ __launch_bounds__(256) void ce_reduce_kernel(const float* row_loss, const int* row_rank, int rows, double* out) {
+__global__ __launch_bounds__(256) void ce_reduce_kernel(const float* row_loss, const int* row_rank, int rows, double* out, int n_out, double scale) {
     __shared__ double sd[3][256];
     double s = 0, t1 = 0, t5 = 0;
     for (int r = threadIdx.x; r < rows; r += 256) {
@@ -597,7 +704,10 @@
         }
         __syncthreads();
     }
-    if (threadIdx.x == 0) { out[0] = sd[0][0]; out[1] = sd[1][0]; out[2] = sd[2][0]; out[3] = rows; }
+    if (threadIdx.x == 0) {
+        out[0] = sd[0][0]; out[1] = sd[1][0]; out[2] = sd[2][0]; out[3] = rows;
+        if (n_out > 4) out[4] = sd[0][0] * scale;
+    }
 }
 
 template <typename T>
@@ -638,6 +748,27 @@
     }
 }
 
+__global__ __launch_bounds__(256) void adamw_segments_kernel(const AdamWSegments a) {
+    int sg = 0;
+#pragma unroll
+    for (int i = 1; i < MEBT_ADAMW_MAX_SEG; ++i)
+        if (i < a.n_seg && blockIdx.x >= a.blk_start[i]) sg = i;
+    const AdamWParams& q = a.s[sg];
+    const AdamWHyper h = {q.lr, q.beta1, q.beta2, q.eps, q.weight_decay, q.bc1, q.bc2, q.grad_scale};
+    const size_t nblk = a.blk_start[sg + 1] - a.blk_start[sg];
+    for (size_t i = ((size_t)(blockIdx.x - a.blk_start[sg]) * 256 + threadIdx.x) * 4; i < q.n; i += nblk * 1024) {
+        f32x4 p = *reinterpret_cast<const f32x4*>(q.p + i);
+        f32x4 g = *reinterpret_cast<const f32x4*>(q.g + i);
+        f32x4 m = *reinterpret_cast<const f32x4*>(q.m + i);
+        f32x4 v = *reinterpret_cast<const f32x4*>(q.v + i);
+        adamw_update4_pinned(p, g, m, v, h);
+        *reinterpret_cast<f32x4*>(q.p + i) = p;
+        *reinterpret_cast<f32x4*>(q.m + i) = m;
+        *reinterpret_cast<f32x4*>(q.v + i) = v;
+        if (q.p_bf16) store4<bf16_t>(reinterpret_cast<bf16_t*>(q.p_bf16) + i, p);
+    }
+}
+
 template <typename TS, typename TD>
 __global__ __launch_bounds__(256) void apply_dropout_kernel(const TS* src, TD* dst, size_t n, DropCfg d) {
     for (size_t i = ((size_t)blockIdx.x * 256 + threadIdx.x) * 4; i < n; i += (size_t)gridDim.x * 1024) {
@@ -679,18 +810,45 @@
     return MEBT_OK;
 }
 
+static int colsum_rpb(int M, int gx) {
+    int rpb = 256;
+    while ((M + rpb - 1) / rpb > 32) rpb *= 2;
+    while (rpb > 64 && (long)gx * ((M + rpb - 1) / rpb) < 256) rpb /= 2;
+    return rpb;
+}
+
 int launch_embed_bwd(const EmbedBwdParams& p, int dtype, hipStream_t stream) {
-    const long rows = (long)p.B * (p.NC + p.NT);
-    if (rows > 0) {
-        const dim3 grid((unsigned)((rows + 3) / 4));
-        if (dtype == MEBT_BF16) hipLaunchKernelGGL(embed_bwd_kernel<bf16_t>, grid, dim3(256), 0, stream, p);
-        else hipLaunchKernelGGL(embed_bwd_kernel<float>, grid, dim3(256), 0, stream, p);
-        CHECK_LAUNCH();
-    }
-    int rc = launch_colsum(p.g_tgt, p.B * p.NT, p.d, p.d, p.g_mask_emb, dtype, stream);
-    if (rc) return rc;
-    if (p.NS > 0) rc = launch_colsum(p.g_sos, p.B, p.NS * p.d, p.NS * p.d, p.g_sos_emb, dtype, stream);
-    return rc;
+    if (p.legacy) {
+        const long rows = (long)p.B * (p.NC + p.NT);
+        if (rows > 0) {
+            const dim3 grid((unsigned)((rows + 3) / 4));
+            if (dtype == MEBT_BF16) hipLaunchKernelGGL(embed_bwd_scatter_kernel<bf16_t>, grid, dim3(256), 0, stream, p);
+            else hipLaunchKernelGGL(embed_bwd_scatter_kernel<float>, grid, dim3(256), 0, stream, p);
+            CHECK_LAUNCH();
+        }
+        int rc = launch_colsum(p.g_tgt, p.B * p.NT, p.d, p.d, p.g_mask_emb, dtype, stream);
+        if (rc) return rc;
+        if (p.NS > 0) rc = launch_colsum(p.g_sos, p.B, p.NS * p.d, p.NS * p.d, p.g_sos_emb, dtype, stream);
+        return rc;
+    }
+    if (p.d % 4) { mebt_set_error("embed_bwd: d must be a multiple of 4"); return MEBT_ESHAPE; }
+    if (!p.inv || p.pos_rows < p.N || p.vocab <= 0) { mebt_set_error("embed_bwd: inverse-map scratch / table sizes not set"); return MEBT_EINVAL; }
+    if (p.B <= 0 || p.N <= 0) return MEBT_OK;
+    hipLaunchKernelGGL(embed_inverse_map_kernel, dim3(p.B), dim3(256), 0, stream, p.ci, p.ti, p.inv, p.N, p.NC, p.NT);
+    CHECK_LAUNCH();
+    const int nch = (p.d + 255) / 256;
+    const int pos_blocks = (int)(((long)p.pos_rows * nch + 3) / 4);
+    const int mask_M = p.B * p.NT, sos_M = p.NS > 0 ? p.B : 0;
+    const int mask_gx = (p.d + 63) / 64, sos_gx = (p.NS * p.d + 63) / 64;
+    const int mask_rpb = colsum_rpb(mask_M, mask_gx), sos_rpb = colsum_rpb(sos_M, sos_gx);
+    const int mask_blocks = mask_M > 0 ? mask_gx * ((mask_M + mask_rpb - 1) / mask_rpb) : 0;
+    const int sos_blocks = sos_M > 0 ? sos_gx * ((sos_M + sos_rpb - 1) / sos_rpb) : 0;
+    const int sos_start = pos_blocks + mask_blocks;
+    const dim3 grid((unsigned)(sos_start + sos_blocks));
+    if (dtype == MEBT_BF16) hipLaunchKernelGGL(embed_bwd_kernel<bf16_t>, grid, dim3(256), 0, stream, p, pos_blocks, sos_start, mask_rpb, mask_gx, sos_rpb, sos_gx);
+    else hipLaunchKernelGGL(embed_bwd_kernel<float>, grid, dim3(256), 0, stream, p, pos_blocks, sos_start, mask_rpb, mask_gx, sos_rpb, sos_gx);
+    CHECK_LAUNCH();
+    return MEBT_OK;
 }
 
 int launch_ln_fwd_multi(const LnFwdParams* jobs, int n, int dtype, hipStream_t stream) {
@@ -850,7 +1008,7 @@
         }
         CHECK_LAUNCH();
     }
-    hipLaunchKernelGGL(ce_reduce_kernel, dim3(1), dim3(256), 0, stream, p.row_loss, p.row_rank, p.rows, p.out);
+    hipLaunchKernelGGL(ce_reduce_kernel, dim3(1), dim3(256), 0, stream, p.row_loss, p.row_rank, p.rows, p.out, p.n_out, p.stat_scale);
     CHECK_LAUNCH();
     return MEBT_OK;
 }
@@ -869,6 +1027,26 @@
     const size_t blocks = (p.n / 4 + 255) / 256;
     if (p.g_bf16) hipLaunchKernelGGL(adamw_kernel<bf16_t>, dim3((unsigned)(blocks < 4096 ? blocks : 4096)), dim3(256), 0, stream, p);
     else hipLaunchKernelGGL(adamw_kernel<float>, dim3((unsigned)(blocks < 4096 ? blocks : 4096)), dim3(256), 0, stream, p);
+    CHECK_LAUNCH();
+    return MEBT_OK;
+}
+
+int launch_adamw_segments(AdamWSegments& a, hipStream_t stream) {
+    unsigned blocks = 0;
+    int k = 0;
+    for (int i = 0; i < a.n_seg; ++i) {
+        if (a.s[i].n == 0) continue;
+        if (a.s[i].n % 4 || a.s[i].g_bf16) { mebt_set_error("adamw: segments are fp32 gradients, lengths multiples of 4"); return MEBT_ESHAPE; }
+        a.s[k] = a.s[i];
+        a.blk_start[k] = blocks;
+        const size_t b = (a.s[k].n / 4 + 255) / 256;
+        blocks += (unsigned)(b < 4096 ? b : 4096);
+        ++k;
+    }
+    a.n_seg = k;
+    if (!k) return MEBT_OK;
+    for (int i = k; i <= MEBT_ADAMW_MAX_SEG; ++i) a.blk_start[i] = blocks;
+    hipLaunchKernelGGL(adamw_segments_kernel, dim3(blocks), dim3(256), 0, stream, a);
     CHECK_LAUNCH();
     return MEBT_OK;
 }
diff --git a/mebt_amd/csrc/engine.cpp b/mebt_amd/csrc/engine.cpp
--- a/mebt_amd/csrc/engine.cpp
+++ b/mebt_amd/csrc/engine.cpp
@@ -50,6 +50,7 @@
     bool dlogits_ready = false;
     float dlogits_scale = 0.f;
     void *g_S = nullptr, *g_T = nullptr; float* g_C = nullptr;
+    int32_t* inv_pos = nullptr;
     void* g_cat = nullptr;
     void *dlogits = nullptr, *dhf = nullptr, *datt = nullptr;
     struct Scratch { void *d4, *dh, *dx, *dqkv_q, *dqkv_k, *dqn, *dkn, *dout_m, *dx_m; } sc[2];
@@ -83,6 +84,7 @@
     bool use_side = true;
     hipStream_t side_own = nullptr;
     bool fused_on = false;
+    bool head_fused = false;
     bool grad_acc = false;
     GroupedWgrad pend_w;
     bool pend = false;
@@ -95,6 +97,9 @@
         return d.dtype == MEBT_BF16 ? (const void*)((const char*)Wlp + off * 2) : (const void*)(W + off);
     }
 };
+
+static int g_fused_head = -1, g_rest_split = -1;
+extern "C" void mebt_debug_step_edges(int32_t fused_head, int32_t rest_split) { g_fused_head = fused_head; g_rest_split = rest_split; }
 
 static hipStream_t S(mebt_stream_t s) { return reinterpret_cast<hipStream_t>(s); }
 static int fork_side(mebt_model* m, hipStream_t st);
@@ -405,7 +410,8 @@
     x.logits_ws = nullptr;
     if (training) {
         x.row_lse = (float*)c.take(R * 4); x.row_loss = (float*)c.take(R * 4); x.row_rank = (int*)c.take(R * 4);
-        x.loss_out = (double*)c.take(32);
+        x.loss_out = (double*)c.take(40);
+        x.inv_pos = (int32_t*)c.take((int64_t)B * m->d.block_size * 4);
         int64_t Mmax = (int64_t)B * (NS + NT);
         if ((int64_t)B * NC > Mmax) Mmax = (int64_t)B * NC;
         if (m->has_maskgit && (int64_t)B * (NC + NT) > Mmax) Mmax = (int64_t)B * (NC + NT);
@@ -721,15 +727,16 @@
     return forward_impl(m, ws, ws_bytes, B, 1, NC, NT, nullptr, nullptr, nullptr, e, logits, 1 | (dropout ? 2 : 0), dropout_seed, stream);
 }
 
-static int loss_impl(mebt_model* m, void* ws, const float* logits, double* out4, bool with_grad, float loss_scale, mebt_stream_t stream) {
+static int loss_impl(mebt_model* m, void* ws, const float* logits, double* out, bool with_grad, float loss_scale, int n_out, double stat_scale, mebt_stream_t stream) {
     if (!m || !m->ctx.valid || m->ctx.ws != ws) { mebt_set_error("loss: no training-mode forward on this workspace"); return MEBT_EINVAL; }
     FwdCtx& x = m->ctx;
     if (!x.x_ids) { mebt_set_error("loss: the last forward ran on caller-embedded inputs (no token ids to score against)"); return MEBT_EINVAL; }
-    if (!out4) out4 = x.loss_out;
+    if (!out) out = x.loss_out;
     x.loss_done = true;
     CeParams p;
     p.logits = logits; p.x_ids = x.x_ids; p.ti = x.ti; p.rows = x.B * x.NT; p.V = m->d.vocab; p.B = x.B; p.N = x.N; p.NT = x.NT;
-    p.label_smoothing = m->d.label_smoothing; p.row_lse = x.row_lse; p.row_loss = x.row_loss; p.row_rank = x.row_rank; p.out = out4;
+    p.label_smoothing = m->d.label_smoothing; p.row_lse = x.row_lse; p.row_loss = x.row_loss; p.row_rank = x.row_rank; p.out = out;
+    p.n_out = n_out; p.stat_scale = stat_scale;
     x.dlogits_ready = false;
     if (with_grad && x.dlogits && ce_fwd_can_fuse_grad(p.V)) {
         p.dlogits = x.dlogits; p.grad_scale = loss_scale; p.dl_bf16 = m->d.dtype == MEBT_BF16;
@@ -738,10 +745,15 @@
     return launch_ce_fwd(p, S(stream));
 }
 extern "C" int mebt_loss(mebt_model* m, void* ws, const float* logits, double* out4, mebt_stream_t stream) {
-    return loss_impl(m, ws, logits, out4, false, 0.f, stream);
+    return loss_impl(m, ws, logits, out4, false, 0.f, 4, 0.0, stream);
 }
 extern "C" int mebt_loss_with_grad(mebt_model* m, void* ws, const float* logits, double* out4, float loss_scale, mebt_stream_t stream) {
-    return loss_impl(m, ws, logits, out4, true, loss_scale, stream);
+    return loss_impl(m, ws, logits, out4, true, loss_scale, 4, 0.0, stream);
+}
+extern "C" int mebt_loss_stats(mebt_model* m, void* ws, const float* logits, double* out5, double stat_scale, int32_t with_grad, float loss_scale,
+                               mebt_stream_t stream) {
+    if (!out5) { mebt_set_error("loss_stats: null output"); return MEBT_EINVAL; }
+    return loss_impl(m, ws, logits, out5, with_grad != 0, loss_scale, 5, stat_scale, stream);
 }
 
 static int ln_bwd(const mebt_model* m, const void* x, const void* dy, const void* dy2, int64_t gw, int64_t gb, const float* mean,
@@ -769,6 +781,7 @@
     return gemm(m, p, st);
 }
 
+static int head_wgrad_fused(mebt_model* m, hipStream_t sd);
 static int head_backward_common(mebt_model* m, hipStream_t st) {
     FwdCtx& x = m->ctx;
     const int d = m->d.n_embd, V = m->d.vocab, R = x.B * x.NT;
@@ -779,7 +792,15 @@
         MEBT_HIP_CHECK(hipEventRecord(m->ev_layer[0], sd));
         MEBT_HIP_CHECK(hipEventRecord(m->ev_layer[1], sd));
     }
-    RC(wgrad(m, x.dlogits, V, x.hf, d, m->head_w, V, d, R, sd));
+    static const bool fused_head_env = [] { const char* e = getenv("MEBT_FUSED_HEAD"); return e && e[0] == '1'; }();
+    const bool fused_head = g_fused_head < 0 ? fused_head_env : g_fused_head != 0;
+    m->head_fused = false;
+    if (fused_head && m->fused_on && m->d.dtype == MEBT_BF16 && !m->grad_acc && !m->wire() && R > 0) {
+        RC(head_wgrad_fused(m, sd));
+        m->head_fused = true;
+    } else {
+        RC(wgrad(m, x.dlogits, V, x.hf, d, m->head_w, V, d, R, sd));
+    }
     RC(dgrad(m, x.dlogits, V, m->head_w, x.dhf, R, V, d, EPI_NONE, nullptr, 0, st, m->lo[m->d.n_layer - 1].w2, (int64_t)4 * d * d,
              &x.L[m->d.n_layer - 1], 1));
     RC(ln_bwd(m, x.T_final, x.dhf, nullptr, m->lnf_w, m->lnf_b, x.meanf, x.rstdf, x.g_T, 0, 0, R, 0, 0, 0, st));
@@ -922,6 +943,13 @@
         if (m->fused_on && it.M > 0 && it.N > 0) RC(fused_adamw_slice(m, it.C, (int64_t)it.M * it.N, sd));
     }
     return MEBT_OK;
+}
+
+static int head_wgrad_fused(mebt_model* m, hipStream_t sd) {
+    FwdCtx& x = m->ctx;
+    Leaves lv;
+    lv.wgrad(x.dlogits, m->d.vocab, x.hf, m->d.n_embd, m->gW + m->head_w, m->d.vocab, m->d.n_embd, x.B * x.NT);
+    return flush_leaves(m, lv, sd);
 }
 
 static int flush_or_park(mebt_model* m, Leaves& lv, hipStream_t sd, bool side) {
@@ -1131,12 +1159,20 @@
     if (!m || !m->ctx.valid || m->ctx.ws != ws) { mebt_set_error("backward: no training-mode forward on this workspace"); return MEBT_EINVAL; }
     FwdCtx& x = m->ctx;
     if (!x.x_ids) { mebt_set_error("backward_embed: the last forward ran on caller-embedded inputs: use mebt_gpt_backward"); return MEBT_EINVAL; }
-    RC(input_grad_dropout(m, S(stream)));
+    static const bool legacy = [] { const char* e = getenv("MEBT_EMBED_BWD_LEGACY"); return e && e[0] == '1'; }();
+    if (legacy) RC(input_grad_dropout(m, S(stream)));
     EmbedBwdParams p;
     p.x_ids = x.x_ids; p.ci = x.ci; p.ti = x.ti;
     p.g_ctx = x.g_C; p.g_tgt = x.g_T; p.g_sos = x.g_S;
     p.g_tok_emb = m->gP + m->tok_emb; p.g_pos_emb = m->gP + m->pos_emb; p.g_mask_emb = m->gP + m->mask_emb; p.g_sos_emb = m->gP + m->sos_emb;
     p.B = x.B; p.N = x.N; p.NC = x.gC_defined ? x.NC : 0; p.NT = x.gT_defined ? x.NT : 0; p.NS = x.gS_defined ? m->d.n_latent : 0; p.d = m->d.n_embd;
+    p.legacy = legacy ? 1 : 0;
+    p.vocab = m->d.vocab; p.pos_rows = m->d.block_size; p.inv = x.inv_pos; p.accumulate = m->grad_acc ? 1 : 0;
+    if (x.drop_on && m->d.embd_pdrop > 0.f) {
+        p.drop_sos = make_drop(x.drop_seed, SITE_EMB_SOS, m->d.embd_pdrop);
+        p.drop_tgt = make_drop(x.drop_seed, SITE_EMB_TGT, m->d.embd_pdrop);
+        p.drop_ctx = make_drop(x.drop_seed, SITE_EMB_CTX, m->d.embd_pdrop);
+    }
     if (p.NC != x.NC && x.NC > 0) {
         mebt_set_error("backward_embed: contexts without a live latent_enc block are not supported");
         return MEBT_EINVAL;
@@ -1145,7 +1181,7 @@
     if (g_prof_on) {
         r.a = get_event(); r.b = get_event(); r.kind = 3; r.flops = 0;
         const double dd = p.d;
-        r.bytes = (double)p.B * ((double)p.NC * dd * 4 + ((double)p.NT + p.NS) * dd * m->esz() + ((double)2 * p.NC + p.NT) * dd * 4);
+        r.bytes = (double)p.B * ((double)p.NC * dd * 4 + ((double)p.NT + p.NS) * dd * m->esz() + (double)p.NC * dd * 4) + (double)p.pos_rows * dd * 4;
         (void)hipEventRecord(r.a, S(stream));
     }
     const int rc = launch_embed_bwd(p, m->d.dtype, S(stream));
@@ -1164,9 +1200,18 @@
     a.lr = lr; a.beta1 = beta1; a.beta2 = beta2; a.eps = eps; a.grad_scale = grad_scale;
     a.bc1 = (float)(1.0 - pow((double)beta1, step)); a.bc2 = (float)(1.0 - pow((double)beta2, step));
     const int d = m->d.n_embd;
+    static const bool rest_split_env = [] { const char* e = getenv("MEBT_ADAMW_REST_SPLIT"); return e && e[0] == '1'; }();
+    const bool rest_split = g_rest_split < 0 ? rest_split_env : g_rest_split != 0;
+    AdamWSegments sg;
+    const bool gather = kind == 4 && !rest_split;
     auto run = [&](float* p, const float* g, float* mm, float* vv, void* lp, int64_t off, int64_t n, float wd) -> int {
         a.p = p + off; a.g = g + off; a.m = mm + off; a.v = vv + off; a.n = (size_t)n; a.weight_decay = wd;
         a.p_bf16 = lp ? (void*)((char*)lp + off * 2) : nullptr;
+        if (gather) {
+            if (sg.n_seg == MEBT_ADAMW_MAX_SEG) { RC(launch_adamw_segments(sg, st)); sg.n_seg = 0; }
+            sg.s[sg.n_seg++] = a;
+            return MEBT_OK;
+        }
         return launch_adamw(a, st);
     };
     if (kind == 1 || kind == 3 || kind == 4) {
@@ -1181,11 +1226,14 @@
             i = j + 1;
         }
     }
-    if (kind == 0 || kind == 3 || kind == 4) RC(run(m->W, m->gW, mW, vW, m->Wlp, m->head_w, (int64_t)m->d.vocab * d, weight_decay));
+    const bool head_done = kind == 4 && m->head_fused;
+    if (kind == 4) m->head_fused = false;
+    if ((kind == 0 || kind == 3 || kind == 4) && !head_done) RC(run(m->W, m->gW, mW, vW, m->Wlp, m->head_w, (int64_t)m->d.vocab * d, weight_decay));
     if (kind == 2 || kind == 3 || kind == 4) {
         const int64_t tail_n = (m->tok_live ? m->n_p : m->tok_emb) - m->lnf_w;
         RC(run(m->P, m->gP, mP, vP, nullptr, m->lnf_w, tail_n, 0.f));
     }
+    if (gather) RC(launch_adamw_segments(sg, st));
     return MEBT_OK;
 }
 
diff --git a/mebt_amd/csrc/kernels.h b/mebt_amd/csrc/kernels.h
--- a/mebt_amd/csrc/kernels.h
+++ b/mebt_amd/csrc/kernels.h
@@ -102,6 +102,11 @@
     const void* g_sos;
     float* g_tok_emb; float* g_pos_emb; float* g_mask_emb; float* g_sos_emb;
     int B, N, NC, NT, NS, d;
+    int vocab = 0, pos_rows = 0;
+    int32_t* inv = nullptr;
+    int accumulate = 0;
+    DropCfg drop_ctx = {0, 0, 0, 1.0f, 0, 0}, drop_tgt = {0, 0, 0, 1.0f, 0, 0}, drop_sos = {0, 0, 0, 1.0f, 0, 0};
+    int legacy = 0;
 };
 int launch_embed_bwd(const EmbedBwdParams& p, int dtype, hipStream_t stream);
 
@@ -149,6 +154,8 @@
     float* row_loss;
     int* row_rank;
     double* out;
+    int n_out = 4;
+    double stat_scale = 0.0;
     void* dlogits = nullptr;
     float grad_scale = 0.f;
     int dl_bf16 = 0;
@@ -173,6 +180,13 @@
     size_t g_stride = 0;
 };
 int launch_adamw(const AdamWParams& p, hipStream_t stream);
+#define MEBT_ADAMW_MAX_SEG 8
+struct AdamWSegments {
+    AdamWParams s[MEBT_ADAMW_MAX_SEG];
+    unsigned blk_start[MEBT_ADAMW_MAX_SEG + 1];
+    int n_seg = 0;
+};
+int launch_adamw_segments(AdamWSegments& a, hipStream_t stream);
 int launch_cast_f32_to_bf16(const float* src, void* dst, size_t n, hipStream_t stream);
 
 struct AttnParams {
diff --git a/mebt_amd/engine.py b/mebt_amd/engine.py
--- a/mebt_amd/engine.py
+++ b/mebt_amd/engine.py
@@ -199,6 +199,12 @@
             check(self.lib.mebt_loss_with_grad(self.h, ptr(self.ws), ptr(logits), ptr(out), float(grad_scale), cur_stream()))
         return out
 
+    def step_stats(self, logits, stat_scale, grad_scale=None):
+        out = torch.empty(5, device=self.device, dtype=torch.float64)
+        check(self.lib.mebt_loss_stats(self.h, ptr(self.ws), ptr(logits), ptr(out), float(stat_scale), 0 if grad_scale is None else 1,
+                                       float(grad_scale or 0.0), cur_stream()))
+        return out
+
     def backward_head(self, logits, loss_scale, upstream=None):
         self.ensure_grads()
         check(self.lib.mebt_backward_head(self.h, ptr(self.ws), ptr(logits), ptr(upstream), float(loss_scale), cur_stream()))
diff --git a/mebt_amd/trainer.py b/mebt_amd/trainer.py
--- a/mebt_amd/trainer.py
+++ b/mebt_amd/trainer.py
@@ -62,14 +62,14 @@
         lr = m.learning_rate * m.lr_scale()
         logits = nm.forward(x_ids, ci, ti, training=True, dropout_seed=m._next_seed())
         fused_ce = os.environ.get("MEBT_FUSED_CE", "1") != "0"
-        stats = nm.loss_stats(logits, grad_scale=(scale / self.accum if self.accum > 1 else scale) if fused_ce else None)
+        stats = nm.step_stats(logits, scale, grad_scale=(scale / self.accum if self.accum > 1 else scale) if fused_ce else None)
         if self.accum > 1:
             self._micro += 1
             nm.set_grad_accumulate(self._micro > 1)
             if self._micro < self.accum and not flush:
                 nm.backward(logits, scale / self.accum)
                 nm.set_grad_accumulate(False)
-                return torch.cat([stats, (stats[0] * scale).reshape(1)])
+                return stats
             self._micro = 0
             bwd_scale = scale / self.accum
         else:
@@ -118,7 +118,7 @@
             red.sync_tune_table()
         m.trainer.global_step += 1
         m.global_step += 1
-        return torch.cat([stats, (stats[0] * scale).reshape(1)])
+        return stats
 
     def consolidate(self, optimizer_state=True):
         self.reducer.consolidate(self.native, optimizer_state=optimizer_state)
```
